# JVBSouza/descriptools

Hardware: AMD Instinct MI355X
Metric: Mcells/s full descriptor chain (higher is better)
Workload: dtype f32; 1 GPU; 16384x16384 synthetic tilted-integer-fBm DEM per GPU, full chain (d8, flowacc, river mask, flowhand/HAND with fused GFI + ln(hl/H), fused slope+TI+MTI, downslope), device-resident; global_dem=16384x16384, river_threshold_cells=524288

## Files before the change

descriptools_amd/_lib.py:

```python
import ctypes as C
import os

import numpy as np

_HERE = os.path.dirname(os.path.abspath(__file__))
_SO = os.path.join(_HERE, "libdescriptools_hip.so")
_lib = None

c_f32p = C.POINTER(C.c_float)
c_f64p = C.POINTER(C.c_double)
c_u8p = C.POINTER(C.c_uint8)
c_i8p = C.POINTER(C.c_int8)
c_i32p = C.POINTER(C.c_int32)
c_i64p = C.POINTER(C.c_int64)
i64, f64, u32, ci = C.c_int64, C.c_double, C.c_uint32, C.c_int
vp = C.c_void_p

_SIGS = {
    "dt_last_error": (C.c_char_p, []),
    "dt_version": (C.c_char_p, []),
    "dt_device_count": (ci, []),
    "dt_set_flow_impl": (ci, [ci]),
    "dt_debug_set": (ci, [ci, ci]),
    "dt_host_trim": (ci, []),
# ... 33 lines not shown
    "dt_dev_condition_d8_f64_async": (ci, [vp, vp, i64, i64, f64, vp, vp, ci]),
    "dt_dev_condition_stage_w": (ci, [vp, vp, ci, ci, vp, vp, vp, vp, vp]),
    "dt_dev_condition_stage_m_w": (ci, [vp, vp, ci, ci, vp, vp, vp, vp, vp, vp]),
    "dt_flowhand": (ci, [c_f32p, c_u8p, c_i8p, i64, i64, f64, c_f32p, c_i64p, c_f32p]),
    "dt_hand_f32": (ci, [c_f32p, c_i64p, i64, c_f32p]),
    "dt_twi": (ci, [c_i64p, c_f32p, i64, f64, f64, c_f32p, c_f32p]),
    "dt_river_accumulation": (ci, [c_i64p, c_i64p, i64, c_i64p]),
    "dt_gfi_area": (ci, [c_f32p, c_i64p, i64, f64, f64, f64, ci, c_f32p]),
    "dt_gfi": (ci, [c_f32p, c_i64p, c_i64p, i64, f64, f64, f64, c_f32p]),
    "dt_lnhlh": (ci, [c_f32p, c_i64p, i64, f64, f64, f64, c_f32p]),
    "dt_downslope": (ci, [c_f32p, c_u8p, i64, i64, f64, f64, ci, c_f32p]),
    "dt_slope_f64": (ci, [c_f64p, i64, i64, f64, c_f32p]),
    "dt_hand_f64": (ci, [c_f64p, c_i64p, i64, c_f64p]),
    "dt_downslope_f64": (ci, [c_f64p, c_u8p, i64, i64, f64, f64, ci, c_f32p]),
    "dt_gfi_f64h": (ci, [c_f64p, c_i64p, c_i64p, i64, f64, f64, f64, ci, c_f32p]),
    "dt_d8_f64": (ci, [c_f64p, i64, i64, f64, c_u8p, c_f32p]),
    "dt_confusion_multi": (ci, [c_f64p, c_i8p, i64, f64, c_f64p, ci, ci, c_i64p]),
    "dt_synth_dem": (ci, [u32, i64, i64, i64, i64, i64, i64, ci, c_f32p]),
    "dt_dev_malloc": (ci, [vp, i64, C.POINTER(vp)]),
    "dt_dev_free": (ci, [vp, vp]),
    "dt_dev_h2d": (ci, [vp, vp, vp, i64]),
    "dt_dev_d2h": (ci, [vp, vp, vp, i64]),
    "dt_dev_d2h_async": (ci, [vp, vp, vp, i64]),
    "dt_dev_synth_dem": (ci, [vp, u32, i64, i64, i64, i64, i64, i64, ci, vp]),
    "dt_dev_slope_d8": (ci, [vp, vp, i64, i64, f64, vp, vp, vp]),
    "dt_dev_slope_twi": (ci, [vp, vp, vp, i64, i64, f64, f64, vp, vp, vp, vp]),
    "dt_dev_flowacc": (ci, [vp, vp, vp, i64, i64, vp]),
    "dt_dev_flowacc_weighted": (ci, [vp, vp, vp, vp, i64, i64, ci, vp]),
    "dt_dev_stream_order": (ci, [vp, vp, vp, i64, i64, vp, vp, vp]),
    "dt_dev_drainage": (ci, [vp, vp, vp, vp, i64, i64, f64, vp, vp, vp]),
    "dt_dev_upslope_length": (ci, [vp, vp, vp, i64, i64, f64, vp]),
    "dt_dev_dinf_direction": (ci, [vp, vp, vp, i64, i64, f64, vp, vp]),
    "dt_dev_dinf_accumulate": (ci, [vp, vp, vp, i64, i64, ci, ci, vp]),
    "dt_dev_dinf_accumulate_info": (ci, [vp, c_i64p]),
    "dt_dev_reach_catchments": (ci, [vp, vp, vp, ci, i64, i64, vp, vp, vp, i64, vp]),
    "dt_dev_reach_channels": (ci, [vp, vp, vp, i64, i64, i64, vp, vp, vp, vp, vp]),
    "dt_dev_reach_tables": (ci, [vp, vp, vp, ci, vp, i64, i64, c_f64p, ci, i64, ci, vp, vp, vp]),
    "dt_dev_inundate": (ci, [vp, vp, vp, ci, vp, i64, i64, i64, vp]),
    "dt_dev_river_mask": (ci, [vp, vp, i64, i64, vp]),
    "dt_dev_flowacc_river": (ci, [vp, vp, vp, i64, i64, i64, vp, vp]),
    "dt_dev_gfi_lnhlh": (ci, [vp, vp, vp, vp, i64, f64, f64, f64, vp, vp]),
    "dt_dev_flowhand": (ci, [vp, vp, vp, vp, vp, i64, i64, f64, vp, vp, vp, vp]),
    "dt_dev_twi": (ci, [vp, vp, vp, i64, f64, f64, vp, vp]),
    "dt_dev_gfi": (ci, [vp, vp, vp, i64, f64, f64, f64, vp]),
    "dt_dev_lnhlh": (ci, [vp, vp, vp, i64, f64, f64, f64, vp]),
    "dt_dev_downslope": (ci, [vp, vp, vp, i64, i64, f64, f64, ci, vp]),
    "dt_downslope_lift_workspace": (i64, [i64, i64]),
    "dt_dev_downslope_lift": (ci, [vp, vp, vp, i64, i64, f64, f64, ci, vp, vp, i64]),
    "dt_downslope_queue_workspace": (i64, [i64, i64]),
    "dt_downslope_tables_workspace": (i64, [i64, i64]),
    "dt_downslope_tables_threshold": (i64, [i64, i64]),
    "dt_dev_downslope_queue": (ci, [vp, vp, vp, i64, i64, f64, f64, ci, vp, vp, i64]),
    "dt_dev_downslope_queued": (ci, [vp, vp, C.POINTER(i64)]),
    "dt_dev_downslope_finish": (ci, [vp, vp, vp, i64, i64, f64, f64, ci, vp, vp, i64, vp, i64]),
    "dt_dev_confusion_multi": (ci, [vp, vp, vp, i64, f64, c_f64p, ci, ci, vp]),
    "dt_perim_cells": (i64, [i64, i64]),
    "dt_dev_slope_d8_w": (ci, [vp, vp, vp, f64, vp, vp, vp]),
    "dt_dev_slope_twi_w": (ci, [vp, vp, vp, vp, f64, f64, vp, vp, vp, vp]),
    "dt_dev_downslope_w": (ci, [vp, vp, vp, vp, f64, f64, ci, vp, vp]),
    "dt_downslope_lift_workspace_w": (i64, [vp]),
    "dt_dev_downslope_lift_w": (ci, [vp, vp, vp, vp, f64, f64, ci, vp, vp, vp, i64]),
    "dt_dev_downslope_emit_w": (ci, [vp, vp, vp, vp, f64, f64, ci, vp, vp, vp, i64, vp, i64]),
    "dt_dev_downslope_walk_w": (ci, [vp, vp, vp, vp, f64, f64, i64, vp, vp, i64]),
    "dt_dev_downslope_walk_route_w": (ci, [vp, vp, vp, vp, f64, f64, i64, vp, vp, i64, vp, vp, C.c_int32, vp, C.c_int32, vp, vp, vp]),
    "dt_dev_downslope_walk_seed_w": (ci, [vp, vp, vp, i64, vp, vp, vp]),
    "dt_dev_flowacc_local_w": (ci, [vp, vp, vp, vp, vp, vp, vp]),
    "dt_dev_flowacc_finish_w": (ci, [vp, vp, vp, vp, vp, i64, vp, vp]),
    "dt_dev_flowhand_local_w": (ci, [vp, vp, vp, vp, vp, vp, vp, vp, vp, vp, vp, vp]),
    "dt_dev_flowhand_finish_w": (ci, [vp, vp, vp, vp, vp, vp, f64, vp, vp, vp, vp, vp, vp, vp, vp, vp, vp, vp]),
    "dt_dev_unique_extremes_f32": (ci, [vp, vp, i64, vp]),
    "dt_dev_minmax_scale_f32": (ci, [vp, vp, i64, C.c_float, C.c_float, C.c_float, vp]),
    "dt_dev_membench_copy": (ci, [vp, vp, vp, i64, ci]),
    "dt_dev_membench_mix": (ci, [vp, vp, vp, vp, vp, vp, i64, ci, ci, ci]),
    "dt_dev_membench_mix_timed": (ci, [vp, vp, vp, vp, vp, vp, i64, ci, ci, ci, ci, c_f64p]),
    "dt_dev_mem_info": (ci, [vp, c_i64p, c_i64p]),
    "dt_dev_minmax_scale_f32_f64": (ci, [vp, vp, i64, f64, f64, f64, vp]),
    "dt_dev_classify": (ci, [vp, vp, vp, i64, f64, f64, ci, ci, vp, vp, vp]),
    "dt_minmax_scale": (ci, [vp, ci, i64, f64, f64, f64, vp]),
    "dt_binary_map": (ci, [vp, ci, i64, f64, f64, ci, c_u8p]),
    "dt_avaliacao": (ci, [c_i32p, c_i8p, i64, c_i32p, c_i64p]),
    "dt_dev_flowhand_gfi": (ci, [vp, vp, vp, vp, vp, i64, i64, f64, f64, f64, vp, vp, vp, vp, vp, vp]),
    "dt_dev_flowhand_gfi_finish_w": (ci, [vp, vp, vp, vp, vp, vp, f64, f64, f64, vp, vp, vp, vp, vp,
                                          vp, vp, vp, vp, vp, vp, vp, vp]),
    "dt_ctx_set_priority": (ci, [vp, ci]),
    "dt_ctx_fork": (ci, [vp, vp]),
    "dt_ctx_join": (ci, [vp, vp]),
    "dt_dev_rank_solve_flowacc": (ci, [vp, ci, ci, c_i64p, c_i64p, i64, vp, i64, c_i64p, ci, i64, vp]),
    "dt_dev_rank_solve_flowhand": (ci, [vp, ci, ci, c_i64p, c_i64p, i64, vp, i64, c_i64p, ci, i64, vp, vp, vp, vp,
                                        vp, vp]),
    "dt_dev_flowacc_finish_w_a64": (ci, [vp, vp, vp, vp, vp, i64, vp, vp]),
    "dt_dev_slope_twi_w_a64": (ci, [vp, vp, vp, vp, f64, f64, vp, vp, vp, vp]),
    "dt_dev_flowhand_local_w_a64": (ci, [vp, vp, vp, vp, vp, vp, vp, vp, vp, vp, vp, vp]),
    "dt_dev_flowhand_finish_w_a64": (ci, [vp, vp, vp, vp, vp, vp, f64, vp, vp, vp, vp, vp, vp, vp, vp, vp, vp, vp]),
    "dt_dev_flowhand_gfi_finish_w_a64": (ci, [vp, vp, vp, vp, vp, vp, f64, f64, f64, vp, vp, vp, vp, vp,
                                              vp, vp, vp, vp, vp, vp, vp, vp]),
    "dt_dev_gfi_lnhlh_a64": (ci, [vp, vp, vp, vp, i64, f64, f64, f64, vp, vp]),
    "dt_dev_flowacc_river_flowhand_local": (ci, [vp, vp, vp, i64, i64, i64, vp, vp]),
    "dt_dev_flowacc_river_flowhand_local_m": (ci, [vp, vp, vp, vp, i64, i64, i64, vp, vp]),
    "dt_dev_slope_d8_m": (ci, [vp, vp, i64, i64, f64, vp, vp]),
    "dt_nodata_mask_bytes": (i64, [i64, i64]),
    "dt_slope_from_d8_ok": (ci, [i64, i64]),
    "dt_slope_marks_bytes": (i64, [i64, i64]),
    "dt_dev_slope_d8_ms": (ci, [vp, vp, i64, i64, f64, vp, vp, vp, vp]),
    "dt_dev_flowacc_river_flowhand_local_ms": (ci, [vp, vp, vp, vp, i64, i64, i64, vp, vp, f64, f64, vp, vp, vp, vp]),
    "dt_dev_slope_twi_fix": (ci, [vp, vp, vp, i64, i64, f64, f64, vp, vp, vp, vp]),
    "dt_dev_flowacc_finish_flowhand_local_w": (ci, [vp, vp, vp, vp, vp, i64, vp, vp, vp, vp, vp, vp, vp, vp]),
    "dt_dev_flowacc_finish_flowhand_local_w_a64": (ci, [vp, vp, vp, vp, vp, i64, vp, vp, vp, vp, vp, vp, vp, vp]),
    "dt_dev_i32_to_i64": (ci, [vp, vp, i64, vp]),
    "dt_dev_i64_to_i32": (ci, [vp, vp, i64, vp]),
    "dt_dev_slope_d8_f64": (ci, [vp, vp, i64, i64, f64, vp, vp]),
    "dt_dev_slope_twi_f64": (ci, [vp, vp, vp, i64, i64, f64, f64, vp, vp, vp, vp]),
    "dt_dev_downslope_f64": (ci, [vp, vp, vp, i64, i64, f64, f64, ci, vp]),
    "dt_dev_hand_gfi_f64": (ci, [vp, vp, vp, vp, i64, i64, f64, f64, f64, vp, vp, vp]),
    "dt_dev_slope_d8_f64_w": (ci, [vp, vp, vp, f64, vp, vp]),
    "dt_dev_slope_twi_f64_w": (ci, [vp, vp, vp, vp, f64, f64, vp, vp, vp, vp]),
    "dt_dev_slope_twi_f64_w_a64": (ci, [vp, vp, vp, vp, f64, f64, vp, vp, vp, vp]),
    "dt_dev_downslope_f64_w": (ci, [vp, vp, vp, vp, f64, f64, ci, vp, vp]),
    "dt_dev_downslope_walk_seed_f64_w": (ci, [vp, vp, vp, i64, vp, vp, vp]),
    "dt_dev_downslope_walk_route_f64_w": (ci, [vp, vp, vp, vp, f64, f64, i64, vp, vp, vp, C.c_int32, vp, C.c_int32,
                                               vp, vp, vp]),
    "dt_dev_flowhand_zr64_w": (ci, [vp, vp, vp, i64, vp, vp, vp]),
    "dt_dev_rank_solve_flowhand_f64": (ci, [vp, ci, ci, c_i64p, c_i64p, i64, vp, i64, c_i64p, ci, i64, vp, vp, vp, vp,
                                            vp, vp, vp]),
    "dt_hand_f64_table_bytes": (i64, [i64]),
    "dt_dev_hand_gfi_f64_w": (ci, [vp, vp, vp, vp, vp, vp, vp, i64, vp, vp, vp, vp, i64, f64, f64, f64, vp, vp, vp]),
    "dt_dev_hand_gfi_f64_w_a64": (ci, [vp, vp, vp, vp, vp, vp, vp, i64, vp, vp, vp, vp, i64, f64, f64, f64, vp, vp,
                                       vp]),
}


class Window(C.Structure):
    _fields_ = [(n, C.c_int64) for n in ("H", "W", "ld", "gy0", "gx0", "Hg", "Wg", "halo")]


def exported_symbols():
    return sorted(_SIGS)


def _preload_torch_hip_runtime():
    import sys
    if "torch" in sys.modules:
        return
    try:
        import importlib.util
        spec = importlib.util.find_spec("torch")
        if spec is None or not spec.submodule_search_locations:
            return
        cand = os.path.join(list(spec.submodule_search_locations)[0], "lib", "libamdhip64.so")
        if os.path.exists(cand):
            C.CDLL(cand, mode=C.RTLD_GLOBAL)
    except Exception:
        pass


def lib():
    global _lib
    if _lib is not None:
        return _lib
    _preload_torch_hip_runtime()
    if not os.path.exists(_SO):
        from . import build as _build
        _build.build()
    try:
        L = C.CDLL(_SO)
    except OSError as e:
        raise RuntimeError("descriptools_amd: cannot load %s (%s); the HIP library is required, "
# ... 108 lines not shown
```

descriptools_amd/build.py:

```python
import os
import subprocess
import sys

HERE = os.path.dirname(os.path.abspath(__file__))
CSRC = os.path.join(HERE, "csrc")
SO = os.path.join(HERE, "libdescriptools_hip.so")
SOURCES = ["dt_kernels.hip", "dt_stencil.hip", "dt_tiles.hip", "dt_hydro.hip", "dt_wide.hip", "dt_streams.hip",
           "dt_watershed.hip", "dt_reaches.hip", "dt_dinf.hip", "dt_proximity.hip", "dt_capi.hip"]
HEADERS = ["dt_common.h", "dt_kernels.h", "dt_math.h", "dt_math_coeffs.h", "dt_d8_kernel.inc", "dt_fa3fh1_kernel.inc",
           os.path.join("..", "..", "include", "descriptools_hip.h")]
FLAGS = ["-O3", "--offload-arch=gfx950", "-fPIC", "-std=c++17", "-ffp-contract=off", "-fno-fast-math",
         "-Wall", "-Wno-unused-function"]


def _stale():
    if not os.path.exists(SO):
        return True
    t = os.path.getmtime(SO)
    deps = [os.path.join(CSRC, f) for f in SOURCES + HEADERS] + [os.path.abspath(__file__)]
    return any(os.path.getmtime(d) > t for d in deps)


def build(force=False, verbose=False):
    if not force and not _stale():
        return SO
    hipcc = os.environ.get("HIPCC", "/opt/rocm/bin/hipcc")
    objs = []
    for src in SOURCES:
        obj = os.path.join(CSRC, src.replace(".hip", ".o"))
        cmd = [hipcc] + FLAGS + ["-c", os.path.join(CSRC, src), "-o", obj]
        if verbose:
            print(" ".join(cmd), flush=True)
        subprocess.check_call(cmd)
        objs.append(obj)
    cmd = [hipcc, "--offload-arch=gfx950", "-shared", "-fPIC", "-o", SO] + objs
    if verbose:
        print(" ".join(cmd), flush=True)
    subprocess.check_call(cmd)
    return SO


if __name__ == "__main__":
    print(build(force="--force" in sys.argv, verbose=True))
```

descriptools_amd/chain.py:

```python
import ctypes as C

import numpy as np

from . import _lib, placement
from ._lib import check
from .device import Context

F32, F64, U8, I8, I32 = np.float32, np.float64, np.uint8, np.int8, np.int32

OUTPUTS = (("slope", F32), ("fdr", U8), ("fac", I32), ("river", I8), ("fdist", F32), ("idx", I32),
           ("hand", F32), ("a_river", I32), ("slope_rad", F32), ("ti", F32), ("mti", F32), ("gfi", F32),
           ("lnhlh", F32), ("down", F32))

ALGO_BYTES_PER_CELL = 90

WRITE_GROUPS = (("slope", "ti", "mti"), ("fdist", "idx", "hand", "gfi", "lnhlh"), ("fac",), ("a_river",),
                ("slope_rad",), ("down",))

OPS = (
    ("d8", 5, ["k_d8<false>", "k_d8_fix"]),
    ("downslope", 9, ["k_downslope_win<24>"]),
    ("flowacc_flowhand_local", 5 + 1 + 2, ["k_fa_tile1", "k_fa_reduce", "k_fa_poison", "k_fa3fh1<2>", "k_fh_tile1",
                                           "k_fh_ghost_init", "k_fh_node_jump"]),
    ("slope_twi", 20, ["k_slope_twi<true, false, 1, int, 1>", "k_slope_twi_fix<int, 1>"]),
    ("flowhand_gfi_finish", 28, ["k_fh_tile3<false, 1, 5, int>"]),
)

OPS_F64 = (
    ("d8", 13, ["k_d8_f64"]),
    ("downslope", 13, ["k_downslope_win_f64"]),
    ("flowacc_flowhand_local", 4 + 1 + 4 + 1 + 2, ["k_fa_tile1", "k_fa_reduce", "k_fa_poison", "k_fa3fh1<2>",
                                                 "k_fh_tile1", "k_fh_ghost_init", "k_fh_node_jump"]),
    ("slope_twi", 24, ["k_slope_twi_f64<false>"]),
    ("flowhand_finish", 10, ["k_fh_tile3<false, 1, 5, int>"]),
    ("hand_gfi", 32, ["k_hand_gfi_f64"]),
)

HEIGHTS = ("float32", "float64")


class Chain:

    def __init__(self, H, W, ctx=None, px=10.0, n_top=0.1, n_gfi=0.4, b=0.1, dz=5.0,
                 river_threshold=None, alloc=None, want_slope_rad=True, side_ctx=None, overlap=True,
                 condition=False, condition_rounds=64, tune_placement=True, release=None, long_walks=False,
                 external_fdr=False, heights="float32"):
        if heights not in HEIGHTS:
            raise ValueError("heights must be one of %s, not %r" % (HEIGHTS, heights))
        self.wide = heights == "float64"
        if self.wide and condition:
            raise ValueError("condition=True is float32-only in Chain: on float64 heights condition the codes with "
                             "dt_dev_condition_d8_f64_async into Chain(heights=\"float64\", external_fdr=True)'s "
                             "p(\"fdr\") (INTEGRATION.md), or use run_host(..., heights=\"float64\", condition=True)")
        if self.wide and long_walks is not False:
            raise ValueError("long_walks is float32-only: the float64 chain walks on its window kernel (long_walks=False)")
        assert long_walks in (False, True, "auto")
        assert not (external_fdr and condition), "conditioning computes the codes itself"
        self.outputs = tuple((k, F64 if (self.wide and k == "hand") else dt) for k, dt in OUTPUTS)
        self.external_fdr = bool(external_fdr)
        self.long_walks = long_walks
        self._lift = self._lift_q = self._lift_dem = self._lift_tables = None
        self.condition, self.condition_rounds = bool(condition), int(condition_rounds)
        self._alloc, self._release = alloc, release
        self.want_slope_rad = want_slope_rad
        self.H, self.W, self.N = int(H), int(W), int(H) * int(W)
        self.ctx = ctx or Context()
        self.side = None
        if overlap:
            self.side = side_ctx if side_ctx is not None else Context(device=self.ctx.device)
        self._own_side = overlap and side_ctx is None
        self.px, self.n_top, self.n_gfi, self.b, self.dz = px, n_top, n_gfi, b, dz
        self.river_threshold = self.N // 512 if river_threshold is None else int(river_threshold)
        self.buf = {}
        self._graphs = []
        for name, dt in self.outputs + ((("filled", F32),) if self.condition else ()):
            self.buf[name] = alloc((H, W), dt) if alloc else self.ctx.empty((H, W), dt)
        self._nodata4 = self._proxy = self._marks = None
        if self.wide:
            self._proxy = self.ctx.empty((H, W), F32)
        elif not (self.external_fdr or self.condition):
            self._nodata4 = self.ctx.empty((int(_lib.lib().dt_nodata_mask_bytes(H, W)),), U8)
            if not want_slope_rad and _lib.lib().dt_slope_from_d8_ok(H, W):
                self._marks = self.ctx.empty((int(_lib.lib().dt_slope_marks_bytes(H, W)),), U8)
        assert tune_placement in (False, True, "search")
        self.placement = {"tuned": False, "why": "tune_placement=False"}
        if tune_placement:
            self._tune_placement(search=tune_placement == "search")

    def _tune_placement(self, search=False):
        four = [name for name, dt in self.outputs if np.dtype(dt).itemsize == 4]
        objs = {}
        for name in four:
            b = self.buf[name]
            objs[int(b.ptr.value if hasattr(b, "ptr") else b)] = b

        def extra_alloc():
            b = self._alloc((self.H, self.W), F32) if self._alloc else self.ctx.empty((self.H, self.W), F32)
            q = int(b.ptr.value if hasattr(b, "ptr") else b)
            objs[q] = b
            return q

        def extra_release(q):
            b = objs.pop(q)
            if hasattr(b, "free"):
                b.free()
            elif self._release is not None:
                self._release(q)
        can_grow = search and (self._alloc is None or self._release is not None)

        def spacer_alloc(nbytes):
            rows = max(int(nbytes) // (self.W * 4), 1)
            if self._alloc:
                return ("user", self._alloc((rows, self.W), F32))
            return ("own", self.ctx.empty((rows, self.W), F32))

        def spacer_release(h):
            kind, b = h
            if kind == "own":
                b.free()
            else:
                self._release(int(b.ptr.value if hasattr(b, "ptr") else b))
        groups = [[k for k in g if k in four] for g in WRITE_GROUPS]
        roles, info = placement.assign(self.ctx, self.N * 4, list(objs), [g for g in groups if g],
                                       extra_alloc if can_grow else None, extra_release if can_grow else None,
                                       spacer_alloc=spacer_alloc if can_grow else None,
                                       spacer_release=spacer_release if can_grow else None, search=search)
        self.placement = info
        if info.get("spacer_GiB"):
            for gib in (2, 16):
                try:
                    self.ctx.empty((gib << 30,), np.uint8).free()
                except MemoryError:
                    break
        if roles is None:
            return
        dts = dict(self.outputs)
        for name, q in roles.items():
            b = objs[q]
            if hasattr(b, "dtype"):
                b.dtype = np.dtype(dts[name])
            self.buf[name] = b

    def _lift_ptr(self):
        if self._lift is None:
            self._lift_bytes = int(_lib.lib().dt_downslope_lift_workspace(self.H, self.W))
            self._lift = self.ctx.empty((self._lift_bytes,), np.uint8)
        return self._lift.ptr

    def _queue_downslope(self, side, dem_ptr):
        L = _lib.lib()
        if self._lift_q is None:
            self._lift_q_bytes = int(L.dt_downslope_queue_workspace(self.H, self.W))
            self._lift_q = self.ctx.empty((self._lift_q_bytes,), np.uint8)
        self._lift_dem = dem_ptr
        return L.dt_dev_downslope_queue(side.h, dem_ptr, self.p("fdr"), self.H, self.W, self.px, self.dz, 0,
                                        self.p("down"), self._lift_q.ptr, self._lift_q_bytes)

    def finish_long_walks(self):
        if self.long_walks != "auto" or self._lift_q is None:
            return 0
        L, c = _lib.lib(), self.ctx
        n = C.c_int64(0)
        check(L.dt_dev_downslope_queued(c.h, self._lift_q.ptr, C.byref(n)))
        if n.value == 0:
            return 0
        tables, tb = None, 0
        if n.value >= int(L.dt_downslope_tables_threshold(self.H, self.W)):
            tb = int(L.dt_downslope_tables_workspace(self.H, self.W))
            if self._lift_tables is None:
                try:
                    self._lift_tables = c.empty((tb,), np.uint8)
                except MemoryError:
                    tb = 0
            tables = self._lift_tables
        check(L.dt_dev_downslope_finish(c.h, self._lift_dem, self.p("fdr"), self.H, self.W, self.px, self.dz, 0,
                                        self.p("down"), self._lift_q.ptr, self._lift_q_bytes,
                                        tables.ptr if tables is not None else None, tb if tables is not None else 0))
        c.sync()
        return int(n.value)

    def p(self, name):
        b = self.buf[name]
        return b.ptr if hasattr(b, "ptr") else b

    def ops(self, dem_ptr, want_a_river=False, serial=False):
        L, c, H, W = _lib.lib(), self.ctx, self.H, self.W
        p = self.p
        side = self.side if (self.side is not None and not serial) else c
        if getattr(self, "_full", None) is None:
            self._full = _lib.Window(H, W, W, 0, 0, H, W, 0)
        full = self._full
        if self.wide:
            return self._ops_f64(dem_ptr, want_a_river, side)
        rad = p("slope_rad") if self.want_slope_rad else None
        m4 = self._nodata4.ptr if self._nodata4 is not None else None
        first = ("d8", c, lambda: L.dt_dev_slope_d8_m(c.h, dem_ptr, H, W, self.px, p("fdr"), m4))
        flow = ((lambda: L.dt_dev_flowacc_river_flowhand_local_m(c.h, p("fdr"), dem_ptr, m4, H, W, self.river_threshold,
                                                                 p("fac"), p("river"))) if m4 is not None else
                (lambda: L.dt_dev_flowacc_river_flowhand_local(c.h, p("fdr"), dem_ptr, H, W, self.river_threshold,
                                                               p("fac"), p("river"))))
        twi = lambda: L.dt_dev_slope_twi(side.h, dem_ptr, p("fac"), H, W, self.px, self.n_top, p("slope"), rad, p("ti"),
                                         p("mti"))
        if self._from_d8(dem_ptr):
            marks = self._marks.ptr
            first = ("d8", c, lambda: L.dt_dev_slope_d8_ms(c.h, dem_ptr, H, W, self.px, p("fdr"), m4, p("slope"), marks))
            flow = lambda: L.dt_dev_flowacc_river_flowhand_local_ms(
                c.h, p("fdr"), dem_ptr, m4, H, W, self.river_threshold, p("fac"), p("river"), self.px, self.n_top,
                p("slope"), p("ti"), p("mti"), marks)
            twi = lambda: L.dt_dev_slope_twi_fix(side.h, dem_ptr, p("fac"), H, W, self.px, self.n_top, p("slope"),
                                                 p("ti"), p("mti"), marks)
        if self.condition:
            first = ("condition_d8", c, lambda: L.dt_dev_condition_d8_async(c.h, dem_ptr, H, W, self.px, p("filled"),
                                                                             p("fdr"), self.condition_rounds))
        return ([] if self.external_fdr else [first]) + [
            ("downslope", side, (lambda: L.dt_dev_downslope_lift(side.h, dem_ptr, p("fdr"), H, W, self.px, self.dz, 0,
                                                                  p("down"), self._lift_ptr(), self._lift_bytes))
             if self.long_walks is True else
             (lambda: self._queue_downslope(side, dem_ptr)) if self.long_walks == "auto" else
             (lambda: L.dt_dev_downslope(side.h, dem_ptr, p("fdr"), H, W, self.px, self.dz, 0, p("down")))),
            ("flowacc_flowhand_local", c, flow),
            ("slope_twi", side, twi),
            ("flowhand_gfi_finish", c, lambda: L.dt_dev_flowhand_gfi_finish_w(
                c.h, C.byref(full), dem_ptr, p("fdr"), p("river"), p("fac"), self.px, self.n_gfi, self.b, None, None,
                None, None, None, None, p("fdist"), p("idx"), None, p("hand"),
                p("a_river") if want_a_river else None, p("gfi"), p("lnhlh"))),
        ]

    def _from_d8(self, dem_ptr=None):
        if self._marks is None:
            return False
        ptrs = [self.p(k) for k in ("slope", "fac", "ti", "mti", "river", "fdr")] + ([dem_ptr] if dem_ptr else [])
        return all((int(q.value if hasattr(q, "value") else q) & 15) == 0 for q in ptrs)

    def _ops_f64(self, dem_ptr, want_a_river, side):
        L, c, H, W, p = _lib.lib(), self.ctx, self.H, self.W, self.p
        prox = self._proxy.ptr
        rad = p("slope_rad") if self.want_slope_rad else None
        first = ("d8", c, lambda: L.dt_dev_slope_d8_f64(c.h, dem_ptr, H, W, self.px, p("fdr"), prox))
        if self.external_fdr:
            first = ("nodata_proxy", c, lambda: L.dt_dev_slope_d8_f64(c.h, dem_ptr, H, W, self.px, None, prox))
        return [
            first,
            ("downslope", side, lambda: L.dt_dev_downslope_f64(side.h, dem_ptr, p("fdr"), H, W, self.px, self.dz, 0,
                                                               p("down"))),
            ("flowacc_flowhand_local", c, lambda: L.dt_dev_flowacc_river_flowhand_local(
                c.h, p("fdr"), prox, H, W, self.river_threshold, p("fac"), p("river"))),
            ("slope_twi", side, lambda: L.dt_dev_slope_twi_f64(side.h, dem_ptr, p("fac"), H, W, self.px, self.n_top,
                                                               p("slope"), rad, p("ti"), p("mti"))),
            ("flowhand_finish", c, lambda: L.dt_dev_flowhand_finish_w(
                c.h, C.byref(self._full), None, p("fdr"), p("river"), p("fac"), self.px, None, None, None, None, None,
                None, p("fdist"), p("idx"), None, None, p("a_river") if want_a_river else None)),
            ("hand_gfi", c, lambda: L.dt_dev_hand_gfi_f64(c.h, dem_ptr, p("idx"), p("fac"), H, W, self.px, self.n_gfi,
                                                          self.b, p("hand"), p("gfi"), p("lnhlh"))),
        ]

    def run(self, dem_ptr, want_a_river=True):
        for name, ctx, call in self.ops(dem_ptr, want_a_river):
            if ctx is not self.ctx:
                self.ctx.fork(ctx)
            check(call())
        if self.side is not None:
            self.ctx.join(self.side)

    def check_status(self):
        self.ctx.raise_on_status()

    def capture(self, dem_ptr, want_a_river=True):
        self.run(dem_ptr, want_a_river)
        self.ctx.sync()
        L = _lib.lib()
        check(L.dt_ctx_capture_begin(self.ctx.h))
        g = C.c_void_p()
        try:
            self.run(dem_ptr, want_a_river)
        except BaseException:
            if L.dt_ctx_capture_end(self.ctx.h, C.byref(g)) == 0 and g:
                L.dt_graph_destroy(g)
            raise
        check(L.dt_ctx_capture_end(self.ctx.h, C.byref(g)))
        gr = Graph(g, self.ctx, self)
        self._graphs.append(gr)
        return gr

    def free(self):
        for gr in self._graphs:
            gr.invalidate("the chain it was captured from has been freed")
        self._graphs = []
        if self._own_side:
            self.side.close()
            self.side, self._own_side = None, False
        for b in list(self.buf.values()):
            if hasattr(b, "free"):
                b.free()
        self.buf = {}
        for name in ("_lift", "_lift_q", "_lift_tables", "_nodata4", "_proxy", "_marks"):
            if getattr(self, name) is not None:
                getattr(self, name).free()
                setattr(self, name, None)


class Graph:

    def __init__(self, handle, ctx, chain=None):
        self.h, self.ctx, self.chain, self._dead = handle, ctx, chain, None

    def invalidate(self, why):
        self._dead = why

    def launch(self):
        if self._dead:
            raise RuntimeError("captured step cannot be replayed: " + self._dead)
        check(_lib.lib().dt_graph_launch(self.h, self.ctx.h))

    def free(self):
        if self.h:
            check(_lib.lib().dt_graph_destroy(self.h))
            self.h = None
        if self.chain is not None and self in self.chain._graphs:
            self.chain._graphs.remove(self)
        self.chain = None


def run_host(dem, px, timings=None, heights="float32", **kw):
    import time
    t0 = time.perf_counter()
    d, wide = _lib.dem_tier(dem, heights)
    H, W = d.shape
    cond64 = None
    if wide:
        if kw.get("long_walks", False) is not False:
            raise ValueError("long_walks is float32-only: the float64 chain walks on its window kernel (long_walks=False)")
        if kw.pop("condition", False):
            if kw.get("external_fdr"):
                raise ValueError("condition=True computes the codes itself: external_fdr must be False")
            cond64 = int(kw.pop("condition_rounds", 64))
            kw["external_fdr"] = True
    ctx = Context()
    kw.setdefault("tune_placement", False)
    kw.setdefault("long_walks", False if wide else "auto")
    ch = Chain(H, W, ctx=ctx, px=px, heights="float64" if wide else "float32", **kw)
    t1 = time.perf_counter()
    d_dem = ctx.to_device(d)
    widened = {k: ctx.empty((H, W), np.int64) for k in ("fac", "idx")}
    filled = ctx.empty((H, W), np.float64) if cond64 is not None else None
# ... 34 lines not shown
```

descriptools_amd/csrc/dt_capi.hip:

```cpp
#include <cmath>
#include <stdarg.h>
#include <stdlib.h>

#include <sys/mman.h>
#include <atomic>
#include <chrono>
#include <mutex>
#include <system_error>
#include <thread>
#include <utility>
#include <vector>

#include "dt_common.h"
#include "dt_kernels.h"

static thread_local char g_err[512] = "";
void dt_set_error(const char *fmt, ...) {
  va_list ap;
  va_start(ap, fmt);
  vsnprintf(g_err, sizeof(g_err), fmt, ap);
  va_end(ap);
}
extern "C" const char *dt_last_error(void) { return g_err; }
extern "C" const char *dt_version(void) { return "descriptools_hip 0.1 (gfx950)"; }
// ... 1191 lines not shown
}

static int dev_flowhand_local_w(dt_ctx *c, const dt_window *win, const float *dem, const uint8_t *fdr,
                                const int8_t *river, const void *acc, int acc64, uint8_t *kind, int32_t *ref,
                                int32_t *nc, int32_t *nd, float *zr, int64_t *ar) {
  DT_DEV(d, c, win);
  DT_REQUIRE(fdr && river && kind && ref && nc && nd && zr && ar, "NULL pointer");
  const size_t need = dt_flowhand_tiled_scratch(d.w.H, d.w.W);
  void *scr = d.scratch(need);
  DT_TRY(d.rc);
  DT_TRY(dt_launch_fh_local(c->stream, d.w, fdr, river, scr, need));
  DT_TRY(d.done(dt_launch_fh_summary(c->stream, d.w, scr, dem, acc, acc64, kind, ref, nc, nd, zr, (long long *)ar)));
  dt_scratch_claim(c, DT_OWNER_HAND, d.w.H, d.w.W, scr);
  return DT_OK;
}
extern "C" int dt_dev_flowhand_local_w(dt_ctx *c, const dt_window *win, const float *dem, const uint8_t *fdr,
                                       const int8_t *river, const int32_t *acc32, uint8_t *kind, int32_t *ref,
                                       int32_t *nc, int32_t *nd, float *zr, int64_t *ar) {
  return dev_flowhand_local_w(c, win, dem, fdr, river, acc32, 0, kind, ref, nc, nd, zr, ar);
}
extern "C" int dt_dev_flowhand_local_w_a64(dt_ctx *c, const dt_window *win, const float *dem, const uint8_t *fdr,
                                           const int8_t *river, const int64_t *acc64, uint8_t *kind, int32_t *ref,
                                           int32_t *nc, int32_t *nd, float *zr, int64_t *ar) {
  return dev_flowhand_local_w(c, win, dem, fdr, river, acc64, 1, kind, ref, nc, nd, zr, ar);
}

static int dev_flowhand_finish_w(dt_ctx *c, const dt_window *win, const float *dem, const uint8_t *fdr,
                                 const int8_t *river, const void *acc, int acc64, double px, double n_gfi, double b,
                                 const uint8_t *res_ok, const int32_t *res_nc, const int32_t *res_nd,
                                 const int64_t *rem_gidx, const float *rem_zr, const int64_t *rem_ar, float *fdist,
                                 int32_t *idx32, int64_t *idx64, float *hand, void *a_river, float *gfi,
                                 float *lnhlh, bool fused) {
  DT_DEV(d, c, win);
  DT_REQUIRE(fdr && river, "NULL raster");
  DT_REQUIRE(!hand || dem, "hand needs dem");
  DT_REQUIRE(!a_river || acc, "a_river needs the accumulation raster");
  DT_REQUIRE(!fused || (dem && acc && gfi && lnhlh), "NULL raster");
  DT_REQUIRE(!res_ok || (res_nc && res_nd && rem_gidx && rem_zr && rem_ar), "incomplete rank-exit results");
  const DtScratchClaim *k;
  DT_TRY(dt_scratch_claimed(c, DT_OWNER_HAND, &d.w, false,
                            "flowhand finish without a matching dt_dev_flowhand_local_w on this context (another call "
                            "has used the context's scratch in between)", &k));
  return d.done(dt_launch_fh_finish(c->stream, d.w, dem, fdr, river, acc, acc64, px, k->ptr, res_ok, res_nc, res_nd,
                                    (const long long *)rem_gidx, rem_zr, (const long long *)rem_ar, fdist, idx32,
                                    (long long *)idx64, hand, a_river, fused ? gfi : nullptr, fused ? lnhlh : nullptr,
                                    n_gfi, b, px));
}
extern "C" int dt_dev_flowhand_finish_w(dt_ctx *c, const dt_window *win, const float *dem, const uint8_t *fdr,
                                        const int8_t *river, const int32_t *acc32, double px,
                                        const uint8_t *res_ok, const int32_t *res_nc, const int32_t *res_nd,
                                        const int64_t *rem_gidx, const float *rem_zr, const int64_t *rem_ar,
                                        float *fdist, int32_t *idx32, int64_t *idx64, float *hand,
                                        int32_t *a_river) {
  return dev_flowhand_finish_w(c, win, dem, fdr, river, acc32, 0, px, 0.0, 1.0, res_ok, res_nc, res_nd, rem_gidx, rem_zr,
                               rem_ar, fdist, idx32, idx64, hand, a_river, nullptr, nullptr, false);
}
extern "C" int dt_dev_flowhand_finish_w_a64(dt_ctx *c, const dt_window *win, const float *dem, const uint8_t *fdr,
                                            const int8_t *river, const int64_t *acc64, double px,
                                            const uint8_t *res_ok, const int32_t *res_nc, const int32_t *res_nd,
                                            const int64_t *rem_gidx, const float *rem_zr, const int64_t *rem_ar,
                                            float *fdist, int32_t *idx32, int64_t *idx64, float *hand,
                                            int64_t *a_river64) {
  return dev_flowhand_finish_w(c, win, dem, fdr, river, acc64, 1, px, 0.0, 1.0, res_ok, res_nc, res_nd, rem_gidx, rem_zr,
                               rem_ar, fdist, idx32, idx64, hand, a_river64, nullptr, nullptr, false);
}
extern "C" int dt_dev_flowhand_gfi_finish_w(dt_ctx *c, const dt_window *win, const float *dem, const uint8_t *fdr,
                                            const int8_t *river, const int32_t *acc32, double px, double n_gfi,
                                            double b, const uint8_t *res_ok, const int32_t *res_nc,
                                            const int32_t *res_nd, const int64_t *rem_gidx, const float *rem_zr,
                                            const int64_t *rem_ar, float *fdist, int32_t *idx32, int64_t *idx64,
                                            float *hand, int32_t *a_river, float *gfi, float *lnhlh) {
  return dev_flowhand_finish_w(c, win, dem, fdr, river, acc32, 0, px, n_gfi, b, res_ok, res_nc, res_nd, rem_gidx, rem_zr,
                               rem_ar, fdist, idx32, idx64, hand, a_river, gfi, lnhlh, true);
}
extern "C" int dt_dev_flowhand_gfi_finish_w_a64(dt_ctx *c, const dt_window *win, const float *dem,
                                                const uint8_t *fdr, const int8_t *river, const int64_t *acc64,
                                                double px, double n_gfi, double b, const uint8_t *res_ok,
                                                const int32_t *res_nc, const int32_t *res_nd,
                                                const int64_t *rem_gidx, const float *rem_zr, const int64_t *rem_ar,
                                                float *fdist, int32_t *idx32, int64_t *idx64, float *hand,
                                                int64_t *a_river64, float *gfi, float *lnhlh) {
  return dev_flowhand_finish_w(c, win, dem, fdr, river, acc64, 1, px, n_gfi, b, res_ok, res_nc, res_nd, rem_gidx, rem_zr,
                               rem_ar, fdist, idx32, idx64, hand, a_river64, gfi, lnhlh, true);
}

static int dt_scratch2_reserve(dt_ctx *c, size_t bytes) {
  return dt_side_reserve(c, &c->scratch2, &c->scratch2_bytes, bytes);
}

extern "C" int dt_dev_rank_solve_flowacc(dt_ctx *c, int ty, int tx, const int64_t *heights, const int64_t *widths,
                                         int64_t Pmax, const void *rows_dev, int64_t rowbytes,
                                         const int64_t *field_offsets3, int rank, int64_t P_rank,
                                         uint64_t *ext_out_dev) {
  DT_DEV(d, c);
  DT_REQUIRE(heights && widths && rows_dev && field_offsets3 && ext_out_dev, "NULL pointer");
  DT_REQUIRE(rank >= 0 && rank < ty * tx && P_rank >= 0 && P_rank <= Pmax, "bad rank / ring size");
  DT_TRY(dt_scratch2_reserve(c, dt_rank_solve_scratch(ty * tx, Pmax)));
  return d.done(dt_launch_rank_solve_flowacc(c->stream, ty, tx, heights, widths, Pmax, rows_dev, rowbytes,
                                             field_offsets3, rank, P_rank, c->scratch2,
                                             (unsigned long long *)ext_out_dev));
}

extern "C" int dt_dev_rank_solve_flowhand(dt_ctx *c, int ty, int tx, const int64_t *heights, const int64_t *widths,
                                          int64_t Pmax, const void *rows_dev, int64_t rowbytes,
                                          const int64_t *field_offsets7, int rank, int64_t P_rank,
                                          uint8_t *res_ok, int32_t *res_nc, int32_t *res_nd, int64_t *rem_gidx,
                                          float *rem_zr, int64_t *rem_ar) {
  DT_DEV(d, c);
  DT_REQUIRE(heights && widths && rows_dev && field_offsets7 && res_ok && res_nc && res_nd && rem_gidx && rem_zr &&
                 rem_ar, "NULL pointer");
  DT_REQUIRE(rank >= 0 && rank < ty * tx && P_rank >= 0 && P_rank <= Pmax, "bad rank / ring size");
  DT_TRY(dt_scratch2_reserve(c, dt_rank_solve_scratch(ty * tx, Pmax)));
  return d.done(dt_launch_rank_solve_flowhand(c->stream, ty, tx, heights, widths, Pmax, rows_dev, rowbytes,
                                              field_offsets7, rank, P_rank, c->scratch2, res_ok, res_nc, res_nd,
                                              (long long *)rem_gidx, rem_zr, (long long *)rem_ar));
}

extern "C" int dt_dev_slope_d8_f64_w(dt_ctx *c, const dt_window *win, const double *dem, double px, uint8_t *fdr,
                                     float *proxy) {
  DT_DEV(d, c, win);
  DT_REQUIRE(dem && (fdr || proxy), "NULL raster");
  return d.done(dt_launch_d8_f64_w(c->stream, d.w, dem, px, fdr, proxy));
}
static int dev_slope_twi_f64_w(dt_ctx *c, const dt_window *win, const double *dem, const void *acc, int acc64,
                               double px, double n_top, float *slope, float *slope_rad, float *ti, float *mti) {
  DT_DEV(d, c, win);
  DT_REQUIRE(dem && acc && ti && mti, "NULL raster");
  return d.done(dt_launch_slope_twi_f64_w(c->stream, d.w, dem, acc, acc64, px, n_top, slope, slope_rad, ti, mti));
}
extern "C" int dt_dev_slope_twi_f64_w(dt_ctx *c, const dt_window *win, const double *dem, const int32_t *acc32,
                                      double px, double n_top, float *slope, float *slope_rad, float *ti, float *mti) {
  return dev_slope_twi_f64_w(c, win, dem, acc32, 0, px, n_top, slope, slope_rad, ti, mti);
}
extern "C" int dt_dev_slope_twi_f64_w_a64(dt_ctx *c, const dt_window *win, const double *dem, const int64_t *acc64,
                                          double px, double n_top, float *slope, float *slope_rad, float *ti,
                                          float *mti) {
  return dev_slope_twi_f64_w(c, win, dem, acc64, 1, px, n_top, slope, slope_rad, ti, mti);
}
extern "C" int dt_dev_downslope_f64_w(dt_ctx *c, const dt_window *win, const double *dem, const uint8_t *fdr,
                                      double px, double dz, int raw, float *out, int32_t *n_unresolved_dev) {
  DT_DEV(d, c, win);
  DT_REQUIRE(dem && fdr && out, "NULL raster");
  if (n_unresolved_dev) DT_HIP(hipMemsetAsync(n_unresolved_dev, 0, sizeof(int32_t), c->stream));
  return d.done(dt_launch_downslope_win_f64_w(c->stream, d.w, dem, fdr, px, dz, raw, out, (int *)n_unresolved_dev));
}
extern "C" int dt_dev_downslope_walk_seed_f64_w(dt_ctx *c, const dt_window *win, const double *dem, int64_t n,
                                                const int32_t *ys, const int32_t *xs, void *rec) {
  return dev_downslope_walk_seed_w(c, win, dem, n, ys, xs, rec, dt_launch_ds_walk_seed_f64);
}
extern "C" int dt_dev_downslope_walk_route_f64_w(dt_ctx *c, const dt_window *win, const double *dem,
                                                 const uint8_t *fdr, double px, double dz, int64_t n, void *rec,
                                                 float *out, const int32_t *row_starts, int32_t ty,
                                                 const int32_t *col_starts, int32_t tx, void *send, int32_t *counts,
                                                 int32_t *scratch) {
  DT_DEV(d, c, win);
  DT_REQUIRE(n >= 0, "negative count");
  DT_REQUIRE(ty >= 1 && tx >= 1 && row_starts && col_starts && counts, "layout / counts missing");
  DT_REQUIRE(n == 0 || (dem && fdr && rec && out && send && scratch), "NULL pointer");
  DT_TRY(dt_launch_ds_walk_f64(c->stream, d.w, dem, fdr, px, dz, n, rec, out));
  return d.done(dt_launch_ds_route(c->stream, n, rec, row_starts, ty, col_starts, tx, send, counts, scratch));
}
extern "C" int dt_dev_flowhand_zr64_w(dt_ctx *c, const dt_window *win, const double *dem, int64_t n,
                                      const uint8_t *kind, const int32_t *ref, double *zr64) {
  DT_DEV(d, c, win);
  DT_REQUIRE(n >= 0 && n <= dt_perim_count(d.w.H, d.w.W), "bad ring size");
  DT_REQUIRE(n == 0 || (dem && kind && ref && zr64), "NULL pointer");
// ... 877 lines not shown
```

descriptools_amd/csrc/dt_kernels.h:

```cpp
#pragma once
#include "dt_common.h"

int dt_launch_synth_dem(hipStream_t s, uint32_t seed, int O, int64_t Hg, int64_t y0, int64_t x0,
                        int64_t h, int64_t w, int nodata_pct, float *out);
int dt_launch_stencil(hipStream_t s, const DtWin &w, const float *dem, double px, float *slope,
                      uint8_t *fdr, float *slope_rad, const void *acc, int acc64, double n_top, float *ti,
                      float *mti, void *aux = nullptr, uint8_t *nod4 = nullptr, int ldm = 0);
static inline int dt_nodata4_ld(int64_t W) { return (int)((((W + 3) / 4) + 7) & ~(int64_t)7); }
static inline size_t dt_nodata4_bytes(int64_t H, int64_t W) { return (size_t)((H + 3) / 4) * (size_t)dt_nodata4_ld(W) * 2; }
struct DtStencilAux {
  uint8_t *mark;
  uint16_t *lmask;
  size_t bytes;
};
static inline DtStencilAux dt_stencil_aux_layout(int64_t ntiles, void *aux) {
  DtStencilAux a;
  DtCarver c(aux);
  a.mark = c.take<uint8_t>((size_t)ntiles);
  a.lmask = c.take<uint16_t>((size_t)ntiles * 256);
  a.bytes = c.bytes();
  return a;
}
size_t dt_stencil_aux_bytes(int64_t H, int64_t W);
int dt_launch_d8_slope(hipStream_t s, const DtWin &w, const float *dem, double px, uint8_t *fdr, float *slope,
                       void *aux, uint8_t *nod4, int ldm, void *smarks);
int dt_launch_slope_twi_fix(hipStream_t s, const DtWin &w, const float *dem, double px, float *slope,
                            const int32_t *acc, double n_top, float *ti, float *mti, void *smarks);
int dt_launch_flowacc(hipStream_t s, const uint8_t *fdr, const float *dem, int64_t H, int64_t W,
                      unsigned long long *state, int32_t *acc32);
int dt_launch_river_mask(hipStream_t s, const int32_t *acc32, int64_t n, int64_t thr, int8_t *river);
int dt_launch_flowhand(hipStream_t s, const float *dem, const uint8_t *fdr, const int8_t *river,
                       const int32_t *acc32, int64_t H, int64_t W, double px,
                       unsigned long long *state, float *fdist, int32_t *idx32, float *hand,
                       int32_t *a_river);
int dt_launch_twi(hipStream_t s, const int32_t *acc32, const float *srad, int64_t n, double px,
                  double n_top, float *ti, float *mti);
int dt_launch_twi_i64(hipStream_t s, const int64_t *fac, const float *srad, int64_t n, double px,
                      double n_top, float *ti, float *mti);
int dt_launch_gfi(hipStream_t s, const float *hand, const int32_t *area, int64_t n, double expo,
                  double b, double size, float *out, int own_cell);
int dt_launch_gfi_i64(hipStream_t s, const float *hand, const int64_t *area, int64_t n, double expo,
                      double b, double size, float *out, int own_cell);
int dt_launch_river_acc_i64(hipStream_t s, const int64_t *fac, const int64_t *idx, int64_t n,
                            int64_t *out);
struct DtDsLift {
  uint32_t *qcount;
  uint4 *qentries;
  uint32_t qcapacity;
  uint2 *tab[3];
  uint8_t *dom;
  size_t queue_bytes, tables_bytes, bytes;
};
DtDsLift dt_downslope_lift_layout(const DtWin &w, void *work);
size_t dt_downslope_lift_bytes(int64_t H, int64_t W);
size_t dt_downslope_queue_bytes(int64_t H, int64_t W);
size_t dt_downslope_tables_bytes(int64_t H, int64_t W);
uint32_t dt_downslope_lift_min(int64_t H, int64_t W);
size_t dt_downslope_tables_bytes_w(const DtWin &w);
size_t dt_downslope_lift_bytes_w(const DtWin &w);
int dt_launch_downslope(hipStream_t s, const DtWin &w, const float *dem, const uint8_t *fdr, double px,
                        double dz, int raw, float *out, int *n_unresolved, void *qwork = nullptr,
                        void *twork = nullptr, int phase = 0, void *walkers = nullptr, size_t walkers_bytes = 0);
int dt_launch_ds_walk(hipStream_t s, const DtWin &w, const float *dem, const uint8_t *fdr, double px, double dz,
                      int64_t n, void *rec, void *work, float *out = nullptr);
int dt_launch_ds_route(hipStream_t s, int64_t n, const void *rec, const int32_t *row_starts, int ty,
                       const int32_t *col_starts, int tx, void *send, int32_t *counts, int32_t *scratch);
int dt_launch_ds_walk_seed(hipStream_t s, const DtWin &w, const float *dem, int64_t n, const int32_t *ys,
                           const int32_t *xs, void *rec);
int dt_launch_downslope_v1(hipStream_t s, const float *dem, const uint8_t *fdr, int64_t H, int64_t W,
                           double px, double dz, int raw, float *out);
int dt_launch_hand_i64(hipStream_t s, const float *dem, const int64_t *idx, int64_t n, float *hand);
int dt_launch_slope_f64(hipStream_t s, const double *dem, int64_t H, int64_t W, double px, float *slope);
int dt_launch_hand_f64(hipStream_t s, const double *dem, const int64_t *idx, int64_t n, double *hand);
int dt_launch_downslope_f64(hipStream_t s, const double *dem, const uint8_t *fdr, int64_t H, int64_t W, double px,
                            double dz, int raw, float *out);
int dt_launch_gfi_f64h(hipStream_t s, const double *hand, const int64_t *fac, const int64_t *idx, int64_t n,
                       double expo, double b, double size, int own_area, float *out);
int dt_launch_d8_f64(hipStream_t s, const double *dem, int64_t H, int64_t W, double px, uint8_t *fdr, float *slope,
                     float *proxy);
int dt_launch_slope_twi_f64(hipStream_t s, const double *dem, const int32_t *acc32, int64_t H, int64_t W, double px,
                            double n_top, float *slope, float *slope_rad, float *ti, float *mti);
int dt_launch_downslope_win_f64(hipStream_t s, const double *dem, const uint8_t *fdr, int64_t H, int64_t W, double px,
                                double dz, int raw, float *out);
int dt_launch_hand_gfi_f64(hipStream_t s, const double *dem, const int32_t *idx32, const int32_t *acc32, int64_t n,
                           double expo, double b, double size, double *hand, float *gfi, float *lnhlh);
int dt_launch_d8_f64_w(hipStream_t s, const DtWin &w, const double *dem, double px, uint8_t *fdr, float *proxy);
int dt_launch_slope_twi_f64_w(hipStream_t s, const DtWin &w, const double *dem, const void *acc, int acc64, double px,
                              double n_top, float *slope, float *slope_rad, float *ti, float *mti);
int dt_launch_downslope_win_f64_w(hipStream_t s, const DtWin &w, const double *dem, const uint8_t *fdr, double px,
                                  double dz, int raw, float *out, int *n_unresolved);
int dt_launch_fh_zr64_w(hipStream_t s, const DtWin &w, const double *dem, int64_t n, const uint8_t *kind,
                        const int32_t *ref, double *zr64);
int64_t dt_hand_f64_table_slots(int64_t n_remote);
int dt_launch_hand_gfi_f64_w(hipStream_t s, const DtWin &w, const double *dem, const int32_t *idx32,
                             const int64_t *idx64, const void *fac, const void *a_river, int acc64, int64_t n_remote,
                             const uint8_t *res_ok, const int64_t *rem_gidx, const double *rem_zr64, void *table,
                             double expo, double b, double size, double *hand, float *gfi, float *lnhlh);
int dt_launch_ds_walk_f64(hipStream_t s, const DtWin &w, const double *dem, const uint8_t *fdr, double px, double dz,
                          int64_t n, void *rec, float *out);
int dt_launch_ds_walk_seed_f64(hipStream_t s, const DtWin &w, const double *dem, int64_t n, const int32_t *ys,
                               const int32_t *xs, void *rec);
int dt_launch_confusion(hipStream_t s, const double *desc, const int8_t *flood, int64_t n,
                        double nodata, const double *th_host, int nth, int under,
                        unsigned long long *counts4);
int dt_launch_i32_to_i64(hipStream_t s, const int32_t *a, int64_t n, int64_t *b);
int dt_launch_i64_to_i32(hipStream_t s, const int64_t *a, int64_t n, int32_t *b);

size_t dt_flowacc_tiled_scratch(int64_t H, int64_t W);
int dt_launch_fa_local(hipStream_t s, const DtWin &w, const uint8_t *fdr, void *scratch, size_t scratch_bytes,
                       int32_t *acc32, int rank_level);
int dt_launch_fa_summary(hipStream_t s, const DtWin &w, void *scratch, int64_t *A, int32_t *xr, uint8_t *code);
int dt_launch_fa_finish(hipStream_t s, const DtWin &w, const uint8_t *fdr, const float *dem, void *scratch,
                        const unsigned long long *ext_perim, int64_t river_thr, void *acc, int acc64,
                        int8_t *river, int *status = nullptr);
size_t dt_flowacc_weighted_scratch(int64_t H, int64_t W);
int dt_launch_flowacc_weighted(hipStream_t s, const DtWin &w, const uint8_t *fdr, const float *dem, const double *wt,
                               int frac_bits, void *scratch, size_t scratch_bytes, double *acc, int *status);
size_t dt_flowhand_tiled_scratch(int64_t H, int64_t W);
struct DtTwiEpilogue {
  const float *slope;
  float *ti, *mti;
  double px, n_top;
  void *marks;
};
int dt_launch_fa_finish_fh_local(hipStream_t s, const DtWin &w, const uint8_t *fdr, const float *dem, void *fa_scratch,
                                 void *fh_scratch, size_t fh_bytes, const unsigned long long *ext_perim,
                                 int64_t river_thr, void *acc, int acc64, int8_t *river, int *status,
                                 const uint8_t *nod4 = nullptr, int ldm = 0, const DtTwiEpilogue *twi = nullptr);
bool dt_twi_epilogue_ok(const DtWin &w, const void *acc, const int8_t *river, const DtTwiEpilogue *twi);
int dt_launch_fh_local(hipStream_t s, const DtWin &w, const uint8_t *fdr, const int8_t *river, void *scratch,
                       size_t scratch_bytes);
int dt_launch_fh_summary(hipStream_t s, const DtWin &w, void *scratch, const float *dem, const void *acc, int acc64,
                         uint8_t *kind, int32_t *ref, int32_t *nc, int32_t *nd, float *zr, long long *ar);
int dt_launch_fh_finish(hipStream_t s, const DtWin &w, const float *dem, const uint8_t *fdr,
                        const int8_t *river, const void *acc, int acc64, double px, void *scratch,
                        const uint8_t *res_ok, const int32_t *res_nc, const int32_t *res_nd,
                        const long long *rem_gidx, const float *rem_zr, const long long *rem_ar, float *fdist,
                        int32_t *idx32, long long *idx64, float *hand, void *a_river, float *gfi = nullptr,
                        float *lnhlh = nullptr, double n_gfi = 0.0, double b_gfi = 1.0, double size = 1.0);
int dt_launch_gfi_both(hipStream_t s, const float *hand, const void *a_river, const void *fac, int acc64,
                       int64_t n, double expo, double b, double size, float *gfi, float *lnhlh);
int dt_launch_unique_extremes(hipStream_t s, const float *x, int64_t n, uint32_t *work4, float *out3);
int dt_launch_minmax_scale(hipStream_t s, const float *x, int64_t n, float mn, float mx, float nodata,
                           double *out);
int dt_launch_minmax_scale_f32f32(hipStream_t s, const float *x, int64_t n, float mn, float mx, float nodata,
                                  float *out);
int dt_launch_minmax_scale_f64(hipStream_t s, const double *x, int64_t n, double mn, double mx, double nodata,
                               double *out);
int dt_launch_minmax_scale_f32f64(hipStream_t s, const float *x, int64_t n, double mn, double mx, double nodata,
                                  double *out);
int dt_launch_classify_f64(hipStream_t s, const double *desc, const int32_t *bin_in, int8_t *flood, int64_t n,
// ... 84 lines not shown
```

descriptools_amd/csrc/dt_kernels.hip:

```cpp
#include <math.h>

#include "dt_common.h"
#include "dt_kernels.h"
#include "dt_math.h"

void dt_math_host_table(DtLogEntry *tab) {
  for (int i = 0; i < DT_LOGTAB_N; i++) {
    double c = 1.0 + (i + 0.5) / DT_LOGTAB_N;
    double rc = 1.0 / c;
    tab[i].rc = rc;
    tab[i].lnc = (double)(-logl((long double)rc));
  }
}
__device__ DtLogEntry g_logtab[DT_LOGTAB_N];
const DtLogEntry *dt_math_device_table(hipStream_t s) {
  static thread_local int uploaded_dev = -1;
  int dev = 0;
  (void)hipGetDevice(&dev);
  DtLogEntry *p = nullptr;
  (void)hipGetSymbolAddress((void **)&p, HIP_SYMBOL(g_logtab));
  if (uploaded_dev != dev) {
    static DtLogEntry host[DT_LOGTAB_N];
    dt_math_host_table(host);
    (void)hipMemcpyAsync(p, host, sizeof(host), hipMemcpyHostToDevice, s);
    (void)hipStreamSynchronize(s);
    uploaded_dev = dev;
  }
  return p;
}

#define DT_SYNTH_TILT 64
#define DT_SYNTH_KMIN 5
#define DT_SYNTH_SX 4
__constant__ int32_t c_synth_amp[15] = {0,    0,    0,    0,    0,     256,   445,  776,
                                        1351, 2352, 4096, 7131, 12416, 21618, 37640};

__device__ __forceinline__ uint32_t dt_hash32(uint32_t seed, uint32_t o, uint32_t ix, uint32_t iy) {
  uint32_t h = seed * 0x9E3779B1u ^ (o + 1u) * 0x85EBCA77u;
  h ^= ix * 0xC2B2AE3Du;
  h = ((h << 13) | (h >> 19)) * 0x27D4EB2Fu;
  h ^= iy * 0x165667B1u;
  h = ((h << 13) | (h >> 19)) * 0x9E3779B1u;
  h ^= h >> 15;
  h *= 0x85EBCA6Bu;
  h ^= h >> 13;
  h *= 0xC2B2AE35u;
  h ^= h >> 16;
  return h;
}

__global__ __launch_bounds__(256) void k_synth_dem(uint32_t seed, int O, int64_t Hg, int64_t y0,
                                                  int64_t x0, int64_t h, int64_t w, int nodata_pct,
                                                  float *__restrict__ out) {
  int64_t i = (int64_t)blockIdx.x * 256 + threadIdx.x;
  if (i >= h * w) return;
  int64_t r = i / w, c = i - r * w;
  int64_t y = y0 + r, x = x0 + c;
  int64_t z = (int64_t)DT_SYNTH_TILT * (Hg - 1 - y);
  for (int o = 0; o < O; o++) {
    int sh = O - o;
    if (sh < DT_SYNTH_KMIN) break;
    int shx = sh - DT_SYNTH_SX;
    uint32_t lx = (uint32_t)(x >> shx), ly = (uint32_t)(y >> sh);
    uint64_t fx = (uint64_t)(x & ((1 << shx) - 1)) << (16 - shx);
    uint64_t fy = (uint64_t)(y & ((1 << sh) - 1)) << (16 - sh);
    uint64_t v00 = dt_hash32(seed, (uint32_t)o, lx, ly) >> 16;
    uint64_t v10 = dt_hash32(seed, (uint32_t)o, lx + 1, ly) >> 16;
    uint64_t v01 = dt_hash32(seed, (uint32_t)o, lx, ly + 1) >> 16;
    uint64_t v11 = dt_hash32(seed, (uint32_t)o, lx + 1, ly + 1) >> 16;
    uint64_t top = v00 * (65536 - fx) + v10 * fx;
    uint64_t bot = v01 * (65536 - fx) + v11 * fx;
    uint64_t val = (top * (65536 - fy) + bot * fy) >> 32;
    z += (int64_t)((val * (uint64_t)c_synth_amp[sh]) >> 16);
  }
  float zf = (float)z * (1.0f / 256.0f);
  if (nodata_pct > 0) {
    uint32_t hb = dt_hash32(seed ^ 0xA5A5A5A5u, 77u, (uint32_t)(x >> 5), (uint32_t)(y >> 5));
    if ((hb % 100u) < (uint32_t)nodata_pct) zf = DT_NODATA;
  }
  out[i] = zf;
}

int dt_launch_synth_dem(hipStream_t s, uint32_t seed, int O, int64_t Hg, int64_t y0, int64_t x0,
                        int64_t h, int64_t w, int nodata_pct, float *out) {
  int64_t n = h * w;
  if (n == 0) return DT_OK;
  hipLaunchKernelGGL(k_synth_dem, dim3((unsigned)((n + 255) / 256)), dim3(256), 0, s, seed, O, Hg,
// ... 454 lines not shown
      dt_d8_delta(code, dy, dx);
      int ny = y + dy, nx = x + dx;
      if (!dt_in_global(w, ny, nx)) { failed = true; break; }
      if (!dt_readable(w, ny, nx)) { unresolved = true; break; }
      const long long on = (long long)ny * w.ld + nx;
      float zt = dem[on];
      code = fdr[on];
      if (zt == DT_NODATA) { failed = true; break; }
      y = ny;
      x = nx;
      nd += (dy != 0 && dx != 0) ? 1u : 0u;
      drop = z0 - zt;
      if (++loop == 5000u) { failed = true; break; }
    }
  }
  float res = 0.0f;
  if (!slow && !unresolved && loop != 0u) {
    bool safe;
    res = ds_quotient(drop, loop, nd, dcard, ddiag, safe);
    if (!safe) slow = true;
  }
  if (slow) {
    y = y0;
    x = x0;
    double dist = 0.0;
    drop = 0.0f;
    failed = false;
    unresolved = false;
    uint32_t moves = 0;
    nd = 0u;
    while ((double)drop < dz) {
      if (!(RANKED ? dt_has_code(w, y, x) : dt_readable(w, y, x))) { unresolved = true; break; }
      uint32_t code = fdr[(long long)y * w.ld + x];
      if (!dt_d8_valid(code)) { failed = true; break; }
      int dy, dx;
      dt_d8_delta(code, dy, dx);
      int ny = y + dy, nx = x + dx;
      if (!dt_in_global(w, ny, nx)) { failed = true; break; }
      if (!dt_readable(w, ny, nx)) { unresolved = true; break; }
      float zt = dem[(long long)ny * w.ld + nx];
      if (zt == DT_NODATA) { failed = true; break; }
      y = ny;
      x = nx;
      dist += (dy != 0 && dx != 0) ? ddiag : dcard;
      drop = z0 - zt;
      if (++moves == 5000u) { failed = true; break; }
    }
    res = dist == 0.0 ? 0.0f : (float)((double)drop / dist);
    loop = moves;
    wflags = DSW_SEQ;
    wdist = dist;
  }
  if (unresolved) {
    *outp = -50.0f;
    n_unres++;
    if (RANKED && wo.rec) ds_emit_walker(wo, w, y0, x0, y, x, loop, nd, z0, wflags, wdist);
  } else if (raw && failed) *outp = -50.0f;
  else *outp = res;
}

template <bool RANKED>
__device__ __attribute__((noinline)) void ds_finish_overflow(const DtWin &w, const float *__restrict__ dem,
                                                             const uint8_t *__restrict__ fdr, int y0, int x0, float z0,
                                                             uint32_t loop, uint32_t nd, uint32_t pos, double px,
                                                             double dz, float dzf, int raw, float *__restrict__ out,
                                                             int *__restrict__ n_unresolved, DsWalkOut wo) {
  int y, x;
  ds_mem_cell(w, pos, y, x);
  uint32_t unres = 0u;
  ds_finish_cell<RANKED>(w, dem, fdr, y0, x0, z0, z0 - dem[(long long)y * w.ld + x], loop, nd, false, y, x, px,
                        px * sqrt(2.0), dz, dzf, raw, out + (long long)y0 * w.ld + x0, unres, wo);
  if (unres && n_unresolved) atomicAdd(n_unresolved, (int)unres);
}

#define DW_CORE 64
#define MW_OFF 0x3FFu
#define MW_BIAS 512
#define MW_DIAG 0x400u
#define MW_BADCODE 0x800u
#define MW_EDGE 0x1000u
#define MW_RING 0x2000u
#define MW_STOP 0x8000u

template <int DW_M, bool QUEUE, bool RANKED>
__device__ __forceinline__ void ds_win_body(const float *__restrict__ dem,
                                                       const uint8_t *__restrict__ fdr, DtWin w,
                                                       double px, double dz, float dzf, int raw,
                                                       float *__restrict__ out, int tiles_x, int ntiles,
                                                       int *__restrict__ n_unresolved, DsQueue queue, DsWalkOut wo) {
  constexpr int DW_WIN = DW_CORE + 2 * DW_M, DW_LD = DW_WIN + 4;
  __shared__ __attribute__((aligned(16))) unsigned char smem[DW_LD * DW_WIN * 6];
  __shared__ uint16_t s_lut[256];
  __shared__ uint32_t s_queued[3];
  float *s_z = reinterpret_cast<float *>(smem);
  uint16_t *s_w = reinterpret_cast<uint16_t *>(smem + DW_LD * DW_WIN * 4);
  const uint32_t lds0 = (uint32_t)(uintptr_t)(__attribute__((address_space(3))) unsigned char *)smem;
  int b = blockIdx.x, tile;
  {
    int xcd = b & 7, j = b >> 3;
    int q = ntiles >> 3, rem = ntiles & 7;
    if (rem == 0 && q % tiles_x == 0 && (tiles_x & 7) == 0) {
      const int rows = q / tiles_x, per_strip = rows * 8;
      const int strip = j / per_strip, r = (j - strip * per_strip) >> 3, c = (j & 7) + strip * 8;
      tile = xcd * q + r * tiles_x + c;
    } else {
      tile = (xcd < rem ? xcd * (q + 1) : rem * (q + 1) + (xcd - rem) * q) + j;
    }
  }
  const int tyi = tile / tiles_x, txi = tile - tyi * tiles_x;
  const int wy0 = tyi * DW_CORE - DW_M, wx0 = txi * DW_CORE - DW_M;
  const bool vec = (w.ld % 4 == 0) && (((uintptr_t)dem & 15) == 0) && (((uintptr_t)fdr & 3) == 0);
  const int ya = max(-w.halo, -w.gy0), yb = min(w.H + w.halo, w.Hg - w.gy0);
  const int xa = max(-w.halo, -w.gx0), xb = min(w.W + w.halo, w.Wg - w.gx0);
  const int yca = (RANKED && -w.halo > -w.gy0) ? ya + 1 : ya, ycb = (RANKED && w.H + w.halo < w.Hg - w.gy0) ? yb - 1 : yb;
  const int xca = (RANKED && -w.halo > -w.gx0) ? xa + 1 : xa, xcb = (RANKED && w.W + w.halo < w.Wg - w.gx0) ? xb - 1 : xb;
  const bool interior = vec && wy0 >= yca && wy0 + DW_WIN <= ycb && wx0 >= xca && wx0 + DW_WIN <= xcb &&
                        w.gy0 + wy0 >= 1 && w.gy0 + wy0 + DW_WIN <= w.Hg - 1 && w.gx0 + wx0 >= 1 &&
                        w.gx0 + wx0 + DW_WIN <= w.Wg - 1;
  const float ninf = -__builtin_inff();
  constexpr int NG = DW_WIN * (DW_WIN / 4);
  float4 vv[4];
  uint32_t cc[4];
  int nod_here = 0;
  if (interior) {
#pragma unroll
    for (int u = 0; u < 4; u++) {
      int i = threadIdx.x + 1024 * u;
      if (i < NG) {
        int r = i / (DW_WIN / 4), c4 = (i - r * (DW_WIN / 4)) * 4;
        long long g = (long long)(wy0 + r) * w.ld + wx0 + c4;
        vv[u] = *reinterpret_cast<const float4 *>(dem + g);
        cc[u] = *reinterpret_cast<const uint32_t *>(fdr + g);
      }
    }
  }
  if (threadIdx.x < 256) {
    uint32_t code = threadIdx.x, mw = MW_BADCODE | MW_STOP | MW_BIAS;
    if (dt_d8_valid(code)) {
      int dy, dx;
      dt_d8_delta(code, dy, dx);
      mw = (uint32_t)(2 * (dy * DW_LD + dx) + MW_BIAS);
      if (dy != 0 && dx != 0) mw |= MW_DIAG;
    }
    s_lut[code] = (uint16_t)mw;
  }
  if ((QUEUE || RANKED) && threadIdx.x == 0) s_queued[0] = s_queued[2] = 0u;
  __syncthreads();
  if (interior) {
#pragma unroll
    for (int u = 0; u < 4; u++) {
      int i = threadIdx.x + 1024 * u;
      if (i < NG) {
        int r = i / (DW_WIN / 4), c4 = (i - r * (DW_WIN / 4)) * 4;
        const uint32_t rowring = (r == 0 || r == DW_WIN - 1) ? (MW_RING | MW_STOP) : 0u;
        uint32_t m0 = (uint32_t)s_lut[cc[u] & 0xFFu] | rowring | (c4 == 0 ? (MW_RING | MW_STOP) : 0u);
        uint32_t m1 = (uint32_t)s_lut[(cc[u] >> 8) & 0xFFu] | rowring;
        uint32_t m2 = (uint32_t)s_lut[(cc[u] >> 16) & 0xFFu] | rowring;
        uint32_t m3 = (uint32_t)s_lut[cc[u] >> 24] | rowring | (c4 == DW_WIN - 4 ? (MW_RING | MW_STOP) : 0u);
        float4 v = vv[u];
        nod_here |= (v.x == DT_NODATA || v.y == DT_NODATA || v.z == DT_NODATA || v.w == DT_NODATA) ? 1 : 0;
        v.x = v.x == DT_NODATA ? ninf : v.x;
        v.y = v.y == DT_NODATA ? ninf : v.y;
        v.z = v.z == DT_NODATA ? ninf : v.z;
        v.w = v.w == DT_NODATA ? ninf : v.w;
        *reinterpret_cast<float4 *>(&s_z[r * DW_LD + c4]) = v;
        *reinterpret_cast<uint2 *>(&s_w[r * DW_LD + c4]) = make_uint2(m0 | (m1 << 16), m2 | (m3 << 16));
      }
    }
  } else {
    for (int i = threadIdx.x; i < NG; i += 1024) {
      int r = i / (DW_WIN / 4), c4 = (i - r * (DW_WIN / 4)) * 4;
      int gy = wy0 + r, gx = wx0 + c4;
      float4 v = make_float4(0.f, 0.f, 0.f, 0.f);
      uint32_t mwv[4];
      uint32_t codes = 0;
      const bool row_ok = gy >= ya && gy < yb;
      bool rd[4];
#pragma unroll
      for (int k = 0; k < 4; k++) rd[k] = row_ok && gx + k >= xa && gx + k < xb;
      if (vec && rd[0] && rd[3]) {
        v = *reinterpret_cast<const float4 *>(dem + (long long)gy * w.ld + gx);
        codes = *reinterpret_cast<const uint32_t *>(fdr + (long long)gy * w.ld + gx);
      } else {
        const float *p = dem + (long long)gy * w.ld;
        const uint8_t *f = fdr + (long long)gy * w.ld;
        if (rd[0]) { v.x = p[gx]; codes |= (uint32_t)f[gx]; }
        if (rd[1]) { v.y = p[gx + 1]; codes |= (uint32_t)f[gx + 1] << 8; }
        if (rd[2]) { v.z = p[gx + 2]; codes |= (uint32_t)f[gx + 2] << 16; }
        if (rd[3]) { v.w = p[gx + 3]; codes |= (uint32_t)f[gx + 3] << 24; }
      }
#pragma unroll
      for (int k = 0; k < 4; k++) {
// ... 56 lines not shown
    uint32_t q2 = q2_0, mw = s_w[pos0], acc = 0;
    {
      uint32_t t, cnt;
      float zt;
      uint64_t sv;
      asm volatile(
          "s_mov_b64 %[sv], exec\n\t"
          "s_movk_i32 %[cnt], %[cap]\n\t"
          "v_cmpx_gt_f32 vcc, %[dzf], %[drop]\n\t"
          "v_cmpx_gt_u32 vcc, 0x8000, %[mw]\n\t"
          "s_cbranch_execz 2f\n"
          "1:\n\t"
          "v_and_b32 %[t], 0x3ff, %[mw]\n\t"
          "v_add3_u32 %[acc], %[acc], %[mw], %[k19]\n\t"
          "v_add3_u32 %[q2], %[q2], %[t], %[nbias]\n\t"
          "v_lshl_add_u32 %[t], %[q2], 1, %[n2l]\n\t"
          "ds_read_b32 %[zt], %[t]\n\t"
          "ds_read_u16 %[mw], %[q2] offset:%[woff]\n\t"
          "s_sub_u32 %[cnt], %[cnt], 1\n\t"
          "s_waitcnt lgkmcnt(0)\n\t"
          "v_sub_f32 %[drop], %[z0], %[zt]\n\t"
          "s_cbranch_scc1 2f\n\t"
          "v_cmpx_gt_f32 vcc, %[dzf], %[drop]\n\t"
          "v_cmpx_gt_u32 vcc, 0x8000, %[mw]\n\t"
          "s_cbranch_execnz 1b\n"
          "2:\n\t"
          "s_mov_b64 exec, %[sv]"
          : [q2] "+v"(q2), [mw] "+v"(mw), [acc] "+v"(acc), [drop] "+v"(drop), [t] "=&v"(t), [zt] "=&v"(zt),
            [sv] "=&s"(sv), [cnt] "=&s"(cnt)
          : [z0] "v"(z0), [dzf] "s"(dzf), [nbias] "s"(0u - (uint32_t)MW_BIAS), [n2l] "s"(neg2lds0),
            [k19] "s"(1u << 19), [woff] "n"(DW_LD * DW_WIN * 4),
            [cap] "n"(QUEUE ? DS_Q_CAP : 255)
          : "vcc", "scc", "memory");
    }
    uint32_t loop = acc >> 19;
    uint32_t nd = ((acc & 0x7FFFFu) - (q2 - q2_0) - (uint32_t)MW_BIAS * loop) / MW_DIAG;
    const uint32_t pos = (q2 - lds0) >> 1;
    const int ys = wy0 + (int)(pos / DW_LD), xs = wx0 + (int)(pos % DW_LD);
    const bool stop_fail = (mw & (MW_BADCODE | MW_EDGE)) != 0u;
    if (QUEUE && drop < dzf && !stop_fail && (RANKED ? dt_has_code(w, ys, xs) : dt_readable(w, ys, xs))) {
      const uint32_t pq = ds_mem_index(w, ys, xs), pl = loop | (nd << 16);
      if (j == 0) { pq0 = pq; pl0 = pl; }
      else if (j == 1) { pq1 = pq; pl1 = pl; }
      else if (j == 2) { pq2 = pq; pl2 = pl; }
      else { pq3 = pq; pl3 = pl; }
      pend |= 1u << j;
      continue;
    }
    ds_finish_cell<RANKED>(w, dem, fdr, y0, x0, z0, drop, loop, nd, stop_fail, ys, xs, dcard, ddiag, dz, dzf, raw,
                           out + o, unres, wo);
  }
  if (RANKED) {
    if (unres) atomicAdd(&s_queued[2], unres);
    __syncthreads();
    if (threadIdx.x == 0 && s_queued[2] && n_unresolved) atomicAdd(n_unresolved, (int)s_queued[2]);
  } else if (unres && n_unresolved) {
    atomicAdd(n_unresolved, (int)unres);
  }
  if (QUEUE) {
    const uint32_t mine = (uint32_t)__popc(pend);
    uint32_t slot = 0u;
    if (mine) slot = atomicAdd(&s_queued[0], mine);
    __syncthreads();
    if (threadIdx.x == 0 && s_queued[0]) s_queued[1] = atomicAdd(queue.count, s_queued[0]);
    __syncthreads();
    slot += s_queued[1];
    for (int j = 0; pend >> j; j++) {
      if (!((pend >> j) & 1u)) continue;
      const uint32_t pq = j == 0 ? pq0 : j == 1 ? pq1 : j == 2 ? pq2 : pq3;
      const uint32_t pl = j == 0 ? pl0 : j == 1 ? pl1 : j == 2 ? pl2 : pl3;
      const int c = threadIdx.x + 1024 * j;
      const int cy = c / DW_CORE, cx = c - cy * DW_CORE;
      const int y0 = tyi * DW_CORE + cy, x0 = txi * DW_CORE + cx;
      if (slot < queue.capacity) {
        queue.entries[slot] = make_uint4(ds_mem_index(w, y0, x0), pq, pl & 0xFFFFu, pl >> 16);
      } else {
        const float z0 = s_z[(cy + DW_M) * DW_LD + cx + DW_M];
        ds_finish_overflow<RANKED>(w, dem, fdr, y0, x0, z0, pl & 0xFFFFu, pl >> 16, pq, px, dz, dzf, raw, out,
                                   n_unresolved, wo);
      }
      slot++;
    }
  }
}

template <int DW_M>
__global__ __launch_bounds__(1024, 8) void k_downslope_win(const float *__restrict__ dem,
                                                       const uint8_t *__restrict__ fdr, DtWin w, double px, double dz,
                                                       float dzf, int raw, float *__restrict__ out, int tiles_x,
                                                       int ntiles, int *__restrict__ n_unresolved) {
  ds_win_body<DW_M, false, false>(dem, fdr, w, px, dz, dzf, raw, out, tiles_x, ntiles, n_unresolved, DsQueue(),
                                  DsWalkOut());
}
__global__ __launch_bounds__(1024, 8) void k_downslope_win_r(const float *__restrict__ dem,
                                                         const uint8_t *__restrict__ fdr, DtWin w, double px,
                                                         double dz, float dzf, int raw, float *__restrict__ out,
                                                         int tiles_x, int ntiles, int *__restrict__ n_unresolved,
                                                         DsWalkOut wo) {
  ds_win_body<24, false, true>(dem, fdr, w, px, dz, dzf, raw, out, tiles_x, ntiles, n_unresolved, DsQueue(), wo);
}
__global__ __launch_bounds__(1024, 8) void k_downslope_win_q(const float *__restrict__ dem,
                                                         const uint8_t *__restrict__ fdr, DtWin w, double px,
                                                         double dz, float dzf, int raw, float *__restrict__ out,
                                                         int tiles_x, int ntiles, int *__restrict__ n_unresolved,
                                                         DsQueue queue) {
  ds_win_body<24, true, false>(dem, fdr, w, px, dz, dzf, raw, out, tiles_x, ntiles, n_unresolved, queue, DsWalkOut());
}

__global__ __launch_bounds__(1024, 8) void k_downslope_win_rq(const float *__restrict__ dem,
                                                          const uint8_t *__restrict__ fdr, DtWin w, double px,
                                                          double dz, float dzf, int raw, float *__restrict__ out,
                                                          int tiles_x, int ntiles, int *__restrict__ n_unresolved,
                                                          DsQueue queue, DsWalkOut wo) {
  ds_win_body<24, true, true>(dem, fdr, w, px, dz, dzf, raw, out, tiles_x, ntiles, n_unresolved, queue, wo);
}

__device__ __forceinline__ float ds_lift_z(float z) { return z != z ? -__builtin_inff() : z; }
#define LT_M 8
#define LT_WIN (64 + 2 * LT_M)
#define LT_LD (LT_WIN + 1)
template <bool RANKED>
__global__ __launch_bounds__(256) void k_ds_lift_init(const float *__restrict__ dem, const uint8_t *__restrict__ fdr,
                                                     DtWin w, uint2 *__restrict__ T, const uint32_t *__restrict__ qcount,
                                                     uint32_t lift_min, int tiles_x) {
  if (*qcount < lift_min) return;
  __shared__ uint2 s_c[LT_WIN * LT_LD];
  __shared__ uint32_t s_tab[256];
  {
    const uint32_t code = threadIdx.x;
    uint32_t m = 0u;
    if (dt_d8_valid(code)) {
      int dy, dx;
      dt_d8_delta(code, dy, dx);
      m = ((uint32_t)((dy * LT_LD + dx) * 8) & 0xFFFFu) | (1u << 16) | ((dy != 0 && dx != 0) ? (1u << 24) : 0u);
    }
    s_tab[code] = m;
  }
  const int ty = (int)blockIdx.x / tiles_x, tx = (int)blockIdx.x - ty * tiles_x;
  const int y0 = ty * 64 - w.halo, x0 = tx * 64 - w.halo;
  const int wy0 = y0 - LT_M, wx0 = x0 - LT_M;
  static_assert(LT_WIN * LT_WIN % 256 == 0, "the staging loops are unrolled");
  constexpr int LT_CPT = LT_WIN * LT_WIN / 256;
  float zs[LT_CPT];
  uint8_t cs[LT_CPT];
  const int ring = RANKED ? 1 : 0;
  const bool inside = wy0 >= -w.halo + ring && wy0 + LT_WIN <= w.H + w.halo - ring && wx0 >= -w.halo + ring &&
                      wx0 + LT_WIN <= w.W + w.halo - ring && w.gy0 + wy0 >= 0 && w.gy0 + wy0 + LT_WIN <= w.Hg &&
                      w.gx0 + wx0 >= 0 && w.gx0 + wx0 + LT_WIN <= w.Wg;
  if (inside) {
    const float *__restrict__ d0 = dem + ((long long)wy0 * w.ld + wx0);
    const uint8_t *__restrict__ f0 = fdr + ((long long)wy0 * w.ld + wx0);
    const int ld = (int)w.ld;
#pragma unroll
    for (int j = 0; j < LT_CPT; j++) {
      const int i = (int)threadIdx.x + 256 * j;
      const int r = i / LT_WIN, c = i - r * LT_WIN;
      zs[j] = d0[r * ld + c];
      cs[j] = f0[r * ld + c];
    }
  } else {
#pragma unroll
    for (int j = 0; j < LT_CPT; j++) {
      const int i = (int)threadIdx.x + 256 * j;
      const int r = i / LT_WIN, c = i - r * LT_WIN;
      const int y = wy0 + r, x = wx0 + c;
      zs[j] = dt_readable(w, y, x) ? dem[(long long)y * w.ld + x] : DT_NODATA;
      cs[j] = (RANKED ? dt_has_code(w, y, x) : dt_readable(w, y, x)) ? fdr[(long long)y * w.ld + x] : (uint8_t)0;
    }
  }
  int valid = 0;
#pragma unroll
  for (int j = 0; j < LT_CPT; j++) {
    const int i = (int)threadIdx.x + 256 * j;
    const int r = i / LT_WIN, c = i - r * LT_WIN;
    valid |= (r >= LT_M && r < LT_M + 64 && c >= LT_M && c < LT_M + 64 && zs[j] != DT_NODATA) ? 1 : 0;
// ... 453 lines not shown
  L.bytes = c.bytes();
  L.tables_bytes = L.bytes - L.queue_bytes;
  return L;
}
static DtDsLift ds_sizes(int64_t H, int64_t W) { return dt_downslope_lift_layout(dt_full_window(H, W), nullptr); }
size_t dt_downslope_queue_bytes(int64_t H, int64_t W) { return ds_sizes(H, W).queue_bytes; }
size_t dt_downslope_tables_bytes(int64_t H, int64_t W) { return ds_sizes(H, W).tables_bytes; }
size_t dt_downslope_lift_bytes(int64_t H, int64_t W) { return ds_sizes(H, W).bytes; }
uint32_t dt_downslope_lift_min(int64_t H, int64_t W) { return (uint32_t)std::max<int64_t>(DS_LIFT_MIN, H * W / 256); }
size_t dt_downslope_tables_bytes_w(const DtWin &w) { return dt_downslope_lift_layout(w, nullptr).tables_bytes; }
size_t dt_downslope_lift_bytes_w(const DtWin &w) { return dt_downslope_lift_layout(w, nullptr).bytes; }
int dt_launch_downslope(hipStream_t s, const DtWin &w, const float *dem, const uint8_t *fdr, double px,
                        double dz, int raw, float *out, int *n_unresolved, void *qwork, void *twork, int phase,
                        void *walkers, size_t walkers_bytes) {
  const int64_t H = w.H, W = w.W;
  int64_t n = H * W;
  if (n == 0) return DT_OK;
  int tiles_x = (int)((W + DW_CORE - 1) / DW_CORE), tiles_y = (int)((H + DW_CORE - 1) / DW_CORE);
  int64_t ntiles = (int64_t)tiles_x * tiles_y;
  float dzf = (float)dz;
  if ((double)dzf < dz) dzf = nextafterf(dzf, INFINITY);
  DsQueue q;
  DsWalkOut wo;
  if (walkers && walkers_bytes >= 256 + DSW_WORDS * 4) {
    DtCarver cw(walkers);
    wo.count = (uint32_t *)cw.raw(256);
    wo.rec = (uint4 *)((char *)walkers + cw.bytes());
    wo.capacity = (uint32_t)std::min<size_t>((walkers_bytes - cw.bytes()) / (DSW_WORDS * 4), 0x7FFFFFFFu);
    if (phase != 2) DT_HIP(hipMemsetAsync(wo.count, 0, sizeof(uint32_t), s));
  }
  DtDsLift L = {};
  const bool ranked = !(w.halo == 0 && w.gy0 == 0 && w.gx0 == 0 && w.Hg == w.H && w.Wg == w.W);
  if (qwork && ds_mem_cells(w) < 0x7FFFFFFFull) {
    DtCarver cq(qwork), ct(twork);
    ds_carve_queue(cq, w, L);
    ds_carve_tables(ct, w, L);
    q.count = L.qcount;
    q.entries = L.qentries;
    q.capacity = L.qcapacity;
  }
  DT_REQUIRE(phase == 0 || q.entries, "the phases of the long-walk form need the queue workspace (and a window of < 2^31 cells)");
  if (phase != 2) {
    if (q.entries) DT_HIP(hipMemsetAsync(q.count, 0, sizeof(uint32_t), s));
    if (ranked && q.entries)
      hipLaunchKernelGGL(k_downslope_win_rq, dim3((unsigned)ntiles), dim3(1024), 0, s, dem, fdr, w, px, dz, dzf, raw,
                         out, tiles_x, (int)ntiles, n_unresolved, q, wo);
    else if (ranked)
      hipLaunchKernelGGL(k_downslope_win_r, dim3((unsigned)ntiles), dim3(1024), 0, s, dem, fdr, w, px, dz, dzf, raw,
                         out, tiles_x, (int)ntiles, n_unresolved, wo);
    else if (q.entries)
      hipLaunchKernelGGL(k_downslope_win_q, dim3((unsigned)ntiles), dim3(1024), 0, s, dem, fdr, w, px, dz, dzf, raw,
                         out, tiles_x, (int)ntiles, n_unresolved, q);
    else
      hipLaunchKernelGGL(k_downslope_win<24>, dim3((unsigned)ntiles), dim3(1024), 0, s, dem, fdr, w, px, dz, dzf, raw,
                         out, tiles_x, (int)ntiles, n_unresolved);
  }
  if (q.entries && phase != 1) {
    const dim3 b(256);
    const uint32_t lift_min = dt_downslope_lift_min(H, W);
    uint2 *src = nullptr;
    const unsigned fin_blocks = dt_capped_grid(q.capacity, 8192);
    if (L.tab[0]) {
      DT_HIP(hipMemsetAsync(L.dom, 0, ds_mem_cells(w), s));
      const int rows = (int)(H + 2 * w.halo), cols = (int)(W + 2 * w.halo);
      const int ltx = (cols + 63) / 64, lty = (rows + 63) / 64;
      const dim3 gt((unsigned)(ltx * lty));
      const uint32_t *qc = (const uint32_t *)q.count;
      if (ranked) hipLaunchKernelGGL(k_ds_lift_init<true>, gt, b, 0, s, dem, fdr, w, L.tab[2], qc, lift_min, ltx);
      else hipLaunchKernelGGL(k_ds_lift_init<false>, gt, b, 0, s, dem, fdr, w, L.tab[2], qc, lift_min, ltx);
      hipLaunchKernelGGL(k_ds_tab_double<true>, dim3(fin_blocks), b, 0, s, q, (const uint2 *)L.tab[2], L.tab[0], L.dom, (int)w.ld, lift_min);
      hipLaunchKernelGGL(k_ds_tab_double<false>, dim3(fin_blocks), b, 0, s, q, (const uint2 *)L.tab[0], L.tab[1], L.dom, (int)w.ld, lift_min);
      hipLaunchKernelGGL(k_ds_tab_double<false>, dim3(fin_blocks), b, 0, s, q, (const uint2 *)L.tab[1], L.tab[0], L.dom, (int)w.ld, lift_min);
      src = L.tab[0];
    }
    if (ranked)
      hipLaunchKernelGGL(k_ds_finish<true>, dim3(fin_blocks), b, 0, s, dem, fdr, w, px, dz, dzf, raw, out, q,
                         (const uint2 *)src, (const uint2 *)L.tab[2], (const uint8_t *)L.dom, n_unresolved, lift_min, wo);
    else
      hipLaunchKernelGGL(k_ds_finish<false>, dim3(fin_blocks), b, 0, s, dem, fdr, w, px, dz, dzf, raw, out, q,
                         (const uint2 *)src, (const uint2 *)L.tab[2], (const uint8_t *)L.dom, n_unresolved, lift_min, DsWalkOut());
  }
  return DT_OK;
}
int dt_launch_downslope_v1(hipStream_t s, const float *dem, const uint8_t *fdr, int64_t H, int64_t W,
                           double px, double dz, int raw, float *out) {
  int64_t n = H * W;
  if (n == 0) return DT_OK;
  hipLaunchKernelGGL(k_downslope, dim3((unsigned)((n + 255) / 256)), dim3(256), 0, s, dem, fdr, (int)H,
                     (int)W, px, dz, raw, out);
  return DT_OK;
}

__global__ __launch_bounds__(256) void k_hand_i64(const float *__restrict__ dem,
                                                 const int64_t *__restrict__ idx, int64_t n,
                                                 float *__restrict__ hand) {
  int64_t i = (int64_t)blockIdx.x * 256 + threadIdx.x;
  if (i >= n) return;
  float z = dem[i], h = DT_NODATA;
  int64_t k = idx[i];
  if (z != DT_NODATA && k != -100) {
    if (k < 0) k += n;
    if (k >= 0 && k < n) {
      h = z - dem[k];
      if (h < 0.0f && h != DT_NODATA) h = 0.0f;
    }
  }
  hand[i] = h;
}
int dt_launch_hand_i64(hipStream_t s, const float *dem, const int64_t *idx, int64_t n, float *hand) {
  if (n) hipLaunchKernelGGL(k_hand_i64, dim3((unsigned)((n + 255) / 256)), dim3(256), 0, s, dem, idx, n, hand);
  return DT_OK;
}

#define CF_MAXT 24
struct CfThresholds {
  double v[CF_MAXT];
};

__global__ __launch_bounds__(256) void k_confusion(const double *__restrict__ desc,
                                                  const int8_t *__restrict__ flood, int64_t n,
                                                  double nodata, int nth, int under,
                                                  CfThresholds th,
                                                  unsigned long long *__restrict__ counts4) {
  unsigned int b0[CF_MAXT], b2[CF_MAXT];
#pragma unroll
  for (int t = 0; t < CF_MAXT; t++) b0[t] = b2[t] = 0u;
  unsigned int t0 = 0u, t2 = 0u, t3 = 0u;
  int64_t stride = (int64_t)gridDim.x * 256;
  for (int64_t i = (int64_t)blockIdx.x * 256 + threadIdx.x; i < n; i += stride) {
    double v = desc[i];
    int g = flood[i];
    if (g == 1) g = 2;
    else if (g == -100) g = 0;
    bool isn = (v == nodata) || (v != v);
    if (g == 0 || g == 2) {
      if (g == 0) t0++; else t2++;
#pragma unroll
      for (int t = 0; t < CF_MAXT; t++) {
        bool bin = !isn && (t < nth) && (under ? (v <= th.v[t]) : (v >= th.v[t]));
        b0[t] += (bin && g == 0) ? 1u : 0u;
        b2[t] += (bin && g == 2) ? 1u : 0u;
      }
    } else {
      for (int t = 0; t < nth; t++) {
        int bin = (!isn && (under ? (v <= th.v[t]) : (v >= th.v[t]))) ? 1 : 0;
        int r = bin + g;
        if (r >= 0 && r <= 3) atomicAdd(&counts4[t * 4 + r], 1ull);
      }
    }
  }
  (void)t3;
  for (int off = 32; off > 0; off >>= 1) {
    t0 += __shfl_down(t0, off);
    t2 += __shfl_down(t2, off);
#pragma unroll
    for (int t = 0; t < CF_MAXT; t++) {
      b0[t] += __shfl_down(b0[t], off);
      b2[t] += __shfl_down(b2[t], off);
    }
  }
  if ((threadIdx.x & 63) == 0) {
#pragma unroll
    for (int t = 0; t < CF_MAXT; t++) {
      if (t < nth) {
        atomicAdd(&counts4[t * 4 + 0], (unsigned long long)(t0 - b0[t]));
        atomicAdd(&counts4[t * 4 + 1], (unsigned long long)b0[t]);
// ... 274 lines not shown
```

descriptools_amd/csrc/dt_tiles.hip:

```cpp
#include "dt_common.h"
#include "dt_kernels.h"
#include "dt_math.h"

#define TW 64
#define TH 64
#define NT (TW * TH)
#define PS (2 * TW + 2 * (TH - 2))
#define CPT (NT / 256)

#define NX_SINK 0xFFFFu
#define NX_EXIT 0xFFFEu
#define NX_REXIT 0xFFFDu
#define X_NONE 0xFFFFu

__device__ __forceinline__ int dt_slot_of(int ly, int lx) {
  if (ly == 0) return lx;
  if (ly == TH - 1) return TW + lx;
  if (lx == 0) return 2 * TW + (ly - 1);
  if (lx == TW - 1) return 2 * TW + (TH - 2) + (ly - 1);
  return -1;
}
__device__ __forceinline__ void dt_cell_of_slot(int s, int &ly, int &lx) {
  if (s < TW) { ly = 0; lx = s; }
  else if (s < 2 * TW) { ly = TH - 1; lx = s - TW; }
  else if (s < 2 * TW + (TH - 2)) { ly = s - 2 * TW + 1; lx = 0; }
  else { ly = s - 2 * TW - (TH - 2) + 1; lx = TW - 1; }
}
__device__ __forceinline__ uint32_t dt_node_of(int y, int x, int tiles_x) {
  int ty = y / TH, tx = x / TW;
  return (uint32_t)((ty * tiles_x + tx) * PS + dt_slot_of(y - ty * TH, x - tx * TW));
}

__device__ __forceinline__ int dt_tile_of_block(int b, int ntiles) {
  const int full = ntiles & ~15;
  if (b >= full) return b;
  const int xcd = b & 7, j = b >> 3;
  return ((j >> 1) * 8 + xcd) * 2 + (j & 1);
}

__device__ __forceinline__ uint4 dt_tile_fetch16(const uint8_t *__restrict__ fdr, const DtWin &w, int y0, int x0) {
  int t = threadIdx.x;
  int r = t >> 2, c = (t & 3) * 16;
  int gy = y0 + r, gx = x0 + c;
  uint4 v = make_uint4(0, 0, 0, 0);
  if (gy < w.H) {
    const uint8_t *p = fdr + (long long)gy * w.ld + gx;
    if (gx + 15 < w.W && (((uintptr_t)p) & 15) == 0) {
      v = *reinterpret_cast<const uint4 *>(p);
    } else {
      uint32_t w4[4] = {0, 0, 0, 0};
#pragma unroll
      for (int k = 0; k < 16; k++)
        if (gx + k < w.W) w4[k >> 2] |= (uint32_t)p[k] << (8 * (k & 3));
      v = make_uint4(w4[0], w4[1], w4[2], w4[3]);
    }
  }
  return v;
}
__device__ __forceinline__ void dt_tile_put16(uint8_t *s_fdr, uint4 v) {
  int t = threadIdx.x;
  *reinterpret_cast<uint4 *>(&s_fdr[(t >> 2) * TW + (t & 3) * 16]) = v;
}
__device__ __forceinline__ void dt_tile_load_fdr(const uint8_t *__restrict__ fdr, const DtWin &w, int y0,
                                                 int x0, uint8_t *s_fdr) {
  dt_tile_put16(s_fdr, dt_tile_fetch16(fdr, w, y0, x0));
}

__device__ __forceinline__ uint32_t dt_tile_next(uint32_t code, int ly, int lx, int y0, int x0,
                                                const DtWin &w) {
  int y = y0 + ly, x = x0 + lx;
  if (y >= w.H || x >= w.W || !dt_d8_valid(code)) return NX_SINK;
  int dy, dx;
  dt_d8_delta(code, dy, dx);
  int ty = y + dy, tx = x + dx;
  if (!dt_in_core(w, ty, tx)) return dt_in_global(w, ty, tx) ? NX_REXIT : NX_SINK;
  int ny = ly + dy, nx = lx + dx;
  if (ny < 0 || ny >= TH || nx < 0 || nx >= TW) return NX_EXIT;
  return (uint32_t)(ny * TW + nx);
}

__device__ __forceinline__ bool dt_tile_interior(const DtWin &w, int y0, int x0) {
  return y0 >= 1 && x0 >= 1 && y0 + TH + 1 <= w.H && x0 + TW + 1 <= w.W;
}
__device__ __forceinline__ uint32_t dt_tile_next_interior(uint32_t code, int ly, int lx) {
  if (!dt_d8_valid(code)) return NX_SINK;
  int dy, dx;
  dt_d8_delta(code, dy, dx);
  uint32_t ny = (uint32_t)(ly + dy), nx = (uint32_t)(lx + dx);
  return (ny < (uint32_t)TH && nx < (uint32_t)TW) ? ny * TW + nx : NX_EXIT;
}

#define PT_ALIVE 0x8000u
#define PT_EXIT 0x4000u
#define PT_IDX 0x0FFFu

__device__ __forceinline__ void dt_tile_sums_packed(uint32_t *s_word, uint8_t *s_cyc, uint32_t (&va)[CPT / 2],
                                                    uint32_t (&vb)[CPT / 2]) {
  uint32_t P[CPT / 2];
  unsigned long long *s_word2 = reinterpret_cast<unsigned long long *>(s_word);
#pragma unroll
  for (int j = 0; j < CPT / 2; j++) {
    unsigned long long r = s_word2[threadIdx.x + 256 * j];
    P[j] = ((uint32_t)r >> 16) | ((uint32_t)(r >> 32) & 0xFFFF0000u);
    va[j] = vb[j] = 1u;
  }
  for (int round = 0; round < 12; round++) {
    uint32_t jumped = 0;
#pragma unroll
    for (int j = 0; j < CPT / 2; j++) {
      const uint32_t p = P[j];
      if (p & PT_ALIVE) {
        P[j] = (P[j] & 0xFFFF0000u) | (atomicAdd(&s_word[p & PT_IDX], min(va[j], (uint32_t)NT)) >> 16);
        jumped |= 1u << j;
      }
// ... 878 lines not shown
  __syncthreads();
  uint32_t nx[CPT];
#pragma unroll
  for (int j = 0; j < CPT; j++) {
    const int c = threadIdx.x + 256 * j;
    nx[j] = dt_tile_next(s_fdr[c], c / TW, c % TW, y0, x0, w);
  }
  __syncthreads();
#pragma unroll
  for (int j = 0; j < CPT; j++) {
    const int c = threadIdx.x + 256 * j;
    s_nxt[P3(c)] = (uint16_t)(nx[j] < NT ? P3(nx[j]) : nx[j]);
    s_delta[P3(c)] = 0ull;
  }
  __syncthreads();
  if (e != 0ull) {
    int ly, lx;
    dt_cell_of_slot(threadIdx.x, ly, lx);
    uint32_t c = P3(ly * TW + lx);
    if (e & FAW_CYC) {
      for (int it = 0; it < NT && c < NT3; it++) {
        atomicOr(&s_delta[c], FAW_CYC);
        c = s_nxt[c];
      }
    } else {
      for (int it = 0; it < NT && c < NT3; it++) {
        atomicAdd(&s_delta[c], e);
        c = s_nxt[c];
      }
    }
  }
  __syncthreads();
#pragma unroll
  for (int j = 0; j < CPT; j++) {
    const int c = threadIdx.x + 256 * j;
    const int y = y0 + c / TW, x = x0 + c % TW;
    if (y >= w.H || x >= w.W) continue;
    const unsigned long long d = s_delta[P3(c)];
    const bool dead = lv[j] == FAW_LOC_CYC || (d & FAW_CYC) || (HAS_DEM && zv[j] <= DT_NODATA);
    acc[(long long)y * w.ld + x] = dead ? -100.0 : ldexp((double)(lv[j] + d), -sbits);
  }
}
#undef P3
#undef NT3

struct FawScratch {
  unsigned long long *rec, *state, *loc;
  uint32_t *parent;
  int64_t nnodes, ntiles;
  int tiles_x;
  size_t bytes;
};
static FawScratch faw_layout(const DtWin &w, void *scratch) {
  FawScratch f;
  f.tiles_x = (w.W + TW - 1) / TW;
  f.ntiles = (int64_t)f.tiles_x * ((w.H + TH - 1) / TH);
  f.nnodes = f.ntiles * PS;
  DtCarver c(scratch);
  f.rec = c.take<unsigned long long>((size_t)f.nnodes);
  f.state = c.take<unsigned long long>((size_t)f.nnodes);
  f.parent = c.take<uint32_t>((size_t)f.nnodes);
  f.loc = c.take<unsigned long long>((size_t)f.ntiles * NT);
  f.bytes = c.bytes();
  return f;
}
size_t dt_flowacc_weighted_scratch(int64_t H, int64_t W) { return faw_layout(dt_full_window(H, W), nullptr).bytes; }

int dt_launch_flowacc_weighted(hipStream_t s, const DtWin &w, const uint8_t *fdr, const float *dem, const double *wt,
                               int frac_bits, void *scratch, size_t scratch_bytes, double *acc, int *status) {
  if (w.H == 0 || w.W == 0) return DT_OK;
  FawScratch f = faw_layout(w, scratch);
  DT_REQUIRE(scratch_bytes >= f.bytes, "scratch too small");
  DT_REQUIRE(f.nnodes < 0x7FFFFFF0ll, "raster too large for one device tile");
  const unsigned long long qmax = (1ull << 52) / (unsigned long long)((int64_t)w.H * w.W);
  dim3 gt((unsigned)f.ntiles), b(256), gn((unsigned)((f.nnodes + 255) / 256));
  hipLaunchKernelGGL(k_faw_tile1, gt, b, 0, s, fdr, wt, w, f.tiles_x, frac_bits, qmax, f.rec, f.state, f.parent,
                     f.loc, status);
  hipLaunchKernelGGL(k_faw_reduce, gn, b, 0, s, f.rec, f.nnodes, f.parent, f.state);
  if (dem) hipLaunchKernelGGL(k_faw_tile3<true>, gt, b, 0, s, fdr, dem, w, f.tiles_x, f.rec, f.state, f.loc, frac_bits, acc);
  else hipLaunchKernelGGL(k_faw_tile3<false>, gt, b, 0, s, fdr, dem, w, f.tiles_x, f.rec, f.state, f.loc, frac_bits, acc);
  return DT_OK;
}

#define FHT_DEAD 0xFFFFFFFFu
#define FHT_REMOTE 0x80000000u
#define FHT_DONE 0x8000u
#define FHT_CAP 20000u
#define K_RIVER 1u
#define K_DEAD 2u
#define K_EXIT 3u
#define K_REXIT 4u

__device__ __forceinline__ unsigned long long fht_pack(uint32_t ptr, uint32_t nd, uint32_t ncf) {
  return ((unsigned long long)ptr << 32) | ((unsigned long long)nd << 16) | (unsigned long long)ncf;
}

struct FhTile {
  uint8_t *s_fdr;
  uint8_t *s_halo;
  unsigned long long *s_st;
};

__device__ __forceinline__ uint32_t fht_fdr_at(const FhTile &T, int ly, int lx) {
  if (ly >= 0 && ly < TH && lx >= 0 && lx < TW) return T.s_fdr[ly * TW + lx];
  if (ly < 0) return T.s_halo[lx + 1];
  if (ly >= TH) return T.s_halo[(TW + 2) + lx + 1];
  if (lx < 0) return T.s_halo[2 * (TW + 2) + ly];
  return T.s_halo[2 * (TW + 2) + TH + ly];
}

__device__ __forceinline__ void fht_solve_tile(const FhTile &T, const uint8_t *__restrict__ fdr,
                                               const int8_t *__restrict__ river, const DtWin &w, int y0,
                                               int x0) {
  dt_tile_load_fdr(fdr, w, y0, x0, T.s_fdr);
  for (int i = threadIdx.x; i < 2 * (TW + 2) + 2 * TH; i += 256) {
    int y, x;
    if (i < TW + 2) { y = y0 - 1; x = x0 - 1 + i; }
    else if (i < 2 * (TW + 2)) { y = y0 + TH; x = x0 - 1 + (i - (TW + 2)); }
    else if (i < 2 * (TW + 2) + TH) { y = y0 + (i - 2 * (TW + 2)); x = x0 - 1; }
    else { y = y0 + (i - 2 * (TW + 2) - TH); x = x0 + TW; }
    uint8_t v = 0;
    if (dt_readable(w, y, x)) v = fdr[(long long)y * w.ld + x];
    T.s_halo[i] = v;
  }
  uint8_t *s_riv = reinterpret_cast<uint8_t *>(T.s_st);
  dt_tile_load_fdr(reinterpret_cast<const uint8_t *>(river), w, y0, x0, s_riv);
  __syncthreads();
  uint32_t riv = 0;
  for (int j = 0; j < CPT; j++) {
    int c = threadIdx.x + 256 * j;
    if (s_riv[c] == 1) riv |= 1u << j;
  }
  __syncthreads();
  if (dt_tile_interior(w, y0, x0)) {
#pragma unroll
    for (int j = 0; j < CPT; j++) {
      int c = threadIdx.x + 256 * j;
      int ly = c / TW, lx = c % TW;
      uint32_t code = T.s_fdr[c];
      uint32_t ptr = (uint32_t)c | (K_DEAD << 12), lo = FHT_DONE;
      if (code != 0u && ((riv >> j) & 1u)) {
        ptr = (uint32_t)c | (K_RIVER << 12);
      } else if (dt_d8_valid(code)) {
        int dy, dx;
        dt_d8_delta(code, dy, dx);
        uint32_t ny = (uint32_t)(ly + dy), nx = (uint32_t)(lx + dx);
        bool in_tile = ny < (uint32_t)TH && nx < (uint32_t)TW;
        uint32_t tcode = in_tile ? (uint32_t)T.s_fdr[ny * TW + nx] : fht_fdr_at(T, ly + dy, lx + dx);
        if (tcode != 0u) {
          if (in_tile) {
            bool diag = dy != 0 && dx != 0;
            ptr = ny * TW + nx;
            lo = diag ? (1u << 16) : 1u;
          } else {
            ptr = (uint32_t)c | (K_EXIT << 12);
          }
        }
      }
      T.s_st[c] = ((unsigned long long)ptr << 32) | (unsigned long long)lo;
    }
  } else {
    for (int j = 0; j < CPT; j++) {
      int c = threadIdx.x + 256 * j;
      int ly = c / TW, lx = c % TW;
      int y = y0 + ly, x = x0 + lx;
      uint32_t code = T.s_fdr[c];
      unsigned long long s;
      if (y >= w.H || x >= w.W || code == 0u) {
        s = fht_pack((uint32_t)c | (K_DEAD << 12), 0, FHT_DONE);
      } else if ((riv >> j) & 1u) {
        s = fht_pack((uint32_t)c | (K_RIVER << 12), 0, FHT_DONE);
      } else if (!dt_d8_valid(code)) {
        s = fht_pack((uint32_t)c | (K_DEAD << 12), 0, FHT_DONE);
      } else {
        int dy, dx;
        dt_d8_delta(code, dy, dx);
        int ty = y + dy, tx = x + dx;
        if (!dt_in_global(w, ty, tx) || fht_fdr_at(T, ly + dy, lx + dx) == 0u) {
          s = fht_pack((uint32_t)c | (K_DEAD << 12), 0, FHT_DONE);
        } else if (!dt_in_core(w, ty, tx)) {
          s = fht_pack((uint32_t)c | (K_REXIT << 12), 0, FHT_DONE);
        } else if (ly + dy < 0 || ly + dy >= TH || lx + dx < 0 || lx + dx >= TW) {
          s = fht_pack((uint32_t)c | (K_EXIT << 12), 0, FHT_DONE);
        } else {
          bool diag = dy != 0 && dx != 0;
          s = fht_pack((uint32_t)((ly + dy) * TW + lx + dx), diag ? 1u : 0u, diag ? 0u : 1u);
        }
      }
      T.s_st[c] = s;
    }
  }
  __syncthreads();
  ulonglong2 *s_st2 = reinterpret_cast<ulonglong2 *>(T.s_st);
  for (int round = 0; round < 13; round++) {
    int changed = 0;
#pragma unroll
    for (int j = 0; j < CPT / 2; j++) {
      int c2 = threadIdx.x + 256 * j;
      ulonglong2 s = s_st2[c2];
      bool dx = ((uint32_t)s.x & FHT_DONE) != 0u, dy = ((uint32_t)s.y & FHT_DONE) != 0u;
      if (dx && dy) continue;
      if (!dx) {
        unsigned long long t = T.s_st[(uint32_t)(s.x >> 32) & 0xFFFu];
        s.x = (t & 0xFFFFFFFF00000000ull) | (unsigned long long)((uint32_t)s.x + (uint32_t)t);
      }
      if (!dy) {
        unsigned long long t = T.s_st[(uint32_t)(s.y >> 32) & 0xFFFu];
        s.y = (t & 0xFFFFFFFF00000000ull) | (unsigned long long)((uint32_t)s.y + (uint32_t)t);
      }
      s_st2[c2] = s;
      changed |= (((uint32_t)s.x & (uint32_t)s.y & FHT_DONE) == 0u) ? 1 : 0;
    }
    if (!__syncthreads_or(changed)) break;
  }
#pragma unroll
  for (int j = 0; j < CPT; j++) {
    int c = threadIdx.x + 256 * j;
    if (!((uint32_t)T.s_st[c] & FHT_DONE)) T.s_st[c] = fht_pack((uint32_t)c | (K_DEAD << 12), 0, FHT_DONE);
  }
  __syncthreads();
}

__device__ __forceinline__ uint32_t fh_cache_pack(unsigned long long s) {
  uint32_t ptr = (uint32_t)(s >> 32);
  return (ptr & 0x7FFFu) | ((uint32_t)((s >> 16) & 0xFFu) << 15) | ((uint32_t)(s & 0xFFu) << 23);
}
__device__ __forceinline__ unsigned long long fh_cache_unpack(uint32_t v) {
  return fht_pack(v & 0x7FFFu, (v >> 15) & 0xFFu, ((v >> 23) & 0xFFu) | FHT_DONE);
}
__device__ __forceinline__ unsigned long long fh_cache_get(const unsigned long long *__restrict__ cache, bool wide,
                                                            int tile, int c) {
  if (wide) return cache[(size_t)tile * NT + c];
  return fh_cache_unpack(reinterpret_cast<const uint32_t *>(cache + (size_t)tile * NT)[c]);
}

__global__ __launch_bounds__(256) void k_fh_tile1(const uint8_t *__restrict__ fdr,
                                                 const int8_t *__restrict__ river, DtWin w, int tiles_x,
                                                 uint32_t nnodes, unsigned long long *__restrict__ nodes,
                                                 unsigned long long *__restrict__ cache,
                                                 uint8_t *__restrict__ cache_wide, int only_marked, int ntiles) {
  __shared__ __attribute__((aligned(16))) uint8_t s_fdr[NT];
  __shared__ uint8_t s_halo[2 * (TW + 2) + 2 * TH];
  __shared__ __attribute__((aligned(16))) unsigned long long s_st[NT];
  for (int tile = (int)blockIdx.x; tile < ntiles; tile += (int)gridDim.x) {
  if (only_marked && cache_wide[tile] != 2) continue;
  const int ty = tile / tiles_x, tx = tile - ty * tiles_x;
  const int y0 = ty * TH, x0 = tx * TW;
  FhTile T{s_fdr, s_halo, s_st};
  fht_solve_tile(T, fdr, river, w, y0, x0);
  if (threadIdx.x < PS) {
    int ly, lx;
    dt_cell_of_slot(threadIdx.x, ly, lx);
    unsigned long long s = s_st[ly * TW + lx];
    uint32_t ptr = (uint32_t)(s >> 32), nd = (uint32_t)((s >> 16) & 0xFFFFu);
    uint32_t ncf = (uint32_t)(s & 0xFFFFu), nc = ncf & 0x7FFFu;
    uint32_t kind = (ptr >> 12) & 7u, f = ptr & 0xFFFu;
    int fy = (int)f / TW, fx = (int)f % TW;
    unsigned long long o = fht_pack(FHT_DEAD, 0, FHT_DONE);
    if (!(ncf & FHT_DONE)) {
    } else if (kind == K_RIVER) {
      o = fht_pack((uint32_t)((y0 + fy) * w.W + x0 + fx), nd, nc | FHT_DONE);
    } else if (kind == K_EXIT || kind == K_REXIT) {
      int dy, dx;
      dt_d8_delta(s_fdr[f], dy, dx);
      bool diag = dy != 0 && dx != 0;
      uint32_t node = kind == K_EXIT ? dt_node_of(y0 + fy + dy, x0 + fx + dx, tiles_x)
                                     : nnodes + (uint32_t)dt_perim_index(w.H, w.W, y0 + fy, x0 + fx);
      o = fht_pack(node, nd + (diag ? 1u : 0u), nc + (diag ? 0u : 1u));
    }
    nodes[(size_t)tile * PS + threadIdx.x] = o;
  }
  unsigned long long wv[CPT];
  int wide = 0;
#pragma unroll
  for (int j = 0; j < CPT; j++) {
    wv[j] = s_st[threadIdx.x + 256 * j];
    wide |= (((uint32_t)wv[j] & 0x7FFFu) > 255u || ((uint32_t)(wv[j] >> 16) & 0xFFFFu) > 255u) ? 1 : 0;
  }
  wide = __syncthreads_or(wide);
  if (threadIdx.x == 0) cache_wide[tile] = (uint8_t)wide;
  if (wide) {
#pragma unroll
    for (int j = 0; j < CPT; j++) cache[(size_t)tile * NT + threadIdx.x + 256 * j] = wv[j];
  } else {
    uint32_t *c32 = reinterpret_cast<uint32_t *>(cache + (size_t)tile * NT);
#pragma unroll
    for (int j = 0; j < CPT; j++) c32[threadIdx.x + 256 * j] = fh_cache_pack(wv[j]);
  }
  __syncthreads();
  }
}

#define FN_CNT 0x3FFFFu
#define FN_DONE 0x40000u
#define FN_LOW 0x7FFFFu
#define FN_OVF 0x20100u
#define FN_PTR_SH 19
__device__ __forceinline__ uint32_t fh_lut_entry(uint32_t code) {
  if (!dt_d8_valid(code)) return 0u;
  int dy, dx;
  dt_d8_delta(code, dy, dx);
  return ((uint32_t)(dy * TW + dx) << FN_PTR_SH) + ((dy != 0 && dx != 0) ? (1u << 9) : 1u);
}
__device__ __forceinline__ void fh_tile1n_body(uint8_t *s_fdr, uint32_t *s_w, uint8_t *s_kind, int *s_ovf_p,
                                               const uint32_t *s_lut, const uint32_t (&riv4)[NT / 4 / 256],
                                               const DtWin &w, int tile, int tiles_x, int y0, int x0, uint32_t nnodes,
                                               unsigned long long *__restrict__ nodes,
                                               unsigned long long *__restrict__ cache,
                                               uint8_t *__restrict__ cache_wide) {
#define s_ovf (*s_ovf_p)
  const bool interior = dt_tile_interior(w, y0, x0);
  const uint32_t lx0 = (4u * threadIdx.x) & 63u;
#pragma unroll
  for (int u = 0; u < NT / 4 / 256; u++) {
    const int c0 = 4 * (threadIdx.x + 256 * u);
    const uint32_t codes = *reinterpret_cast<const uint32_t *>(&s_fdr[c0]);
// ... 166 lines not shown
  if (i < P) nodes[nnodes + i] = fht_pack(nnodes + (uint32_t)i, 0, 0);
}

__global__ __launch_bounds__(256) void k_fh_node_jump(unsigned long long *__restrict__ state, int64_t n,
                                                      int *__restrict__ flags, int round, int hops) {
  if (flags && round > 0 && flags[round - 1] == 0) {
    if (blockIdx.x == 0 && threadIdx.x == 0) flags[round] = 0;
    return;
  }
  bool pending = false;
  for (int64_t i = (int64_t)blockIdx.x * 256 + threadIdx.x; i < n; i += (int64_t)gridDim.x * 256) {
    unsigned long long s = __hip_atomic_load(&state[i], __ATOMIC_RELAXED, __HIP_MEMORY_SCOPE_AGENT);
    bool open = false, changed = false;
    for (int h = 0; h < hops; h++) {
      const uint32_t ncf = (uint32_t)(s & 0xFFFFu);
      const uint32_t ptr = (uint32_t)(s >> 32), nd = (uint32_t)((s >> 16) & 0xFFFFu);
      if ((ncf & FHT_DONE) || ptr == (uint32_t)i) break;
      const unsigned long long t = __hip_atomic_load(&state[ptr], __ATOMIC_RELAXED, __HIP_MEMORY_SCOPE_AGENT);
      const uint32_t tptr = (uint32_t)(t >> 32), tnd = (uint32_t)((t >> 16) & 0xFFFFu);
      const uint32_t tncf = (uint32_t)(t & 0xFFFFu);
      const uint32_t nnc = ncf + (tncf & 0x7FFFu), nnd = nd + tnd;
      if (((tncf & FHT_DONE) && tptr == FHT_DEAD) || nnc + nnd > FHT_CAP) s = fht_pack(FHT_DEAD, 0, FHT_DONE);
      else s = fht_pack(tptr, nnd, nnc | (tncf & FHT_DONE));
      changed = true;
      open = !(s & (unsigned long long)FHT_DONE) && tptr != ptr;
      if (!open) break;
    }
    if (changed) __hip_atomic_store(&state[i], s, __ATOMIC_RELAXED, __HIP_MEMORY_SCOPE_AGENT);
    pending = pending || open;
  }
  if (flags && __any(pending) && (threadIdx.x & 63) == 0) flags[round] = 1;
}

template <typename AccT>
__global__ __launch_bounds__(256) void k_fh_rank_summary(DtWin w, int tiles_x, uint32_t nnodes,
                                                        const unsigned long long *__restrict__ nodes,
                                                        const float *__restrict__ dem,
                                                        const AccT *__restrict__ acc32, int64_t P,
                                                        uint8_t *__restrict__ kind, int32_t *__restrict__ ref,
                                                        int32_t *__restrict__ nc, int32_t *__restrict__ nd,
                                                        float *__restrict__ zr, long long *__restrict__ ar) {
  int64_t i = (int64_t)blockIdx.x * 256 + threadIdx.x;
  if (i >= P) return;
  int y, x;
  dt_perim_cell(w.H, w.W, i, y, x);
  const bool has_node = dt_slot_of(y % TH, x % TW) >= 0;
  unsigned long long s = has_node ? nodes[dt_node_of(y, x, tiles_x)] : fht_pack(FHT_DEAD, 0, FHT_DONE);
  uint32_t ptr = (uint32_t)(s >> 32), ncf = (uint32_t)(s & 0xFFFFu);
  uint8_t k = (uint8_t)K_DEAD;
  int32_t r = -1;
  float z = DT_NODATA;
  long long a = 0;
  if (ncf & FHT_DONE) {
    if (ptr != FHT_DEAD) {
      k = (uint8_t)K_RIVER;
      r = (int32_t)ptr;
      long long o = (long long)(ptr / (uint32_t)w.W) * w.ld + (ptr % (uint32_t)w.W);
      if (dem) z = dem[o];
      if (acc32) a = (long long)acc32[o];
    }
  } else if (ptr >= nnodes) {
    k = (uint8_t)K_REXIT;
    r = (int32_t)(ptr - nnodes);
  }
  kind[i] = k;
  ref[i] = r;
  nc[i] = (int32_t)(ncf & 0x7FFFu);
  nd[i] = (int32_t)((s >> 16) & 0xFFFFu);
  zr[i] = z;
  ar[i] = a;
}

__global__ __launch_bounds__(256) void k_fh_ghost_set(unsigned long long *__restrict__ nodes, uint32_t nnodes,
                                                     int64_t P, const uint8_t *__restrict__ res_ok,
                                                     const int32_t *__restrict__ res_nc,
                                                     const int32_t *__restrict__ res_nd) {
  int64_t i = (int64_t)blockIdx.x * 256 + threadIdx.x;
  if (i >= P) return;
  unsigned long long o = fht_pack(FHT_DEAD, 0, FHT_DONE);
  if (res_ok[i]) o = fht_pack(FHT_REMOTE | (uint32_t)i, (uint32_t)res_nd[i], (uint32_t)res_nc[i] | FHT_DONE);
  nodes[nnodes + i] = o;
}

struct FhGfi {
  float *gfi, *lnhlh;
  double expo, c0;
  const DtLogEntry *tab;
};
struct FhRemote {
  const long long *gidx;
  const float *zr;
  const long long *ar;
};
template <typename AccT>
struct FhPay;
template <>
struct FhPay<int32_t> {
  unsigned long long v[PS];
  __device__ __forceinline__ void set(int i, float z, int32_t a) {
    v[i] = ((unsigned long long)(uint32_t)a << 32) | (unsigned long long)__float_as_uint(z);
  }
  __device__ __forceinline__ void get(int i, float &z, int32_t &a) const {
    const unsigned long long p = v[i];
    z = __uint_as_float((uint32_t)p);
    a = (int32_t)(uint32_t)(p >> 32);
  }
};
template <>
struct FhPay<long long> {
  long long av[PS];
  float zv[PS];
  __device__ __forceinline__ void set(int i, float z, long long a) {
    av[i] = a;
    zv[i] = z;
  }
  __device__ __forceinline__ void get(int i, float &z, long long &a) const {
    z = zv[i];
    a = av[i];
  }
};

typedef float fh_v4f __attribute__((ext_vector_type(4)));
typedef int fh_v4i __attribute__((ext_vector_type(4)));
__device__ __forceinline__ void fh_store4(float *p, float a, float b, float c, float d) {
  fh_v4f v = {a, b, c, d};
  __builtin_nontemporal_store(v, reinterpret_cast<fh_v4f *>(p));
}
__device__ __forceinline__ void fh_store4(int32_t *p, int32_t a, int32_t b, int32_t c, int32_t d) {
  fh_v4i v = {a, b, c, d};
  __builtin_nontemporal_store(v, reinterpret_cast<fh_v4i *>(p));
}
typedef long long fh_v2l __attribute__((ext_vector_type(2)));
__device__ __forceinline__ void fh_store4(long long *p, long long a, long long b, long long c, long long d) {
  fh_v2l v0 = {a, b}, v1 = {c, d};
  __builtin_nontemporal_store(v0, reinterpret_cast<fh_v2l *>(p));
  __builtin_nontemporal_store(v1, reinterpret_cast<fh_v2l *>(p + 2));
}

template <bool RANKED, int VH, int MINW, typename AccT>
__global__ __launch_bounds__(256, MINW) void k_fh_tile3(const uint8_t *__restrict__ fdr,
                                                 const float *__restrict__ dem,
                                                 const AccT *__restrict__ acc32, DtWin w, int tiles_x,
                                                 uint32_t nnodes, const unsigned long long *__restrict__ nodes,
                                                 const unsigned long long *__restrict__ cache,
                                                 const uint8_t *__restrict__ cache_wide,
                                                 FhRemote rem, double px, float *__restrict__ fdist,
                                                 int32_t *__restrict__ idx32, long long *__restrict__ idx64,
                                                 float *__restrict__ hand, AccT *__restrict__ a_river,
                                                 FhGfi G) {
  __shared__ unsigned long long s_x[PS];
  __shared__ FhPay<AccT> s_pay;
  __shared__ DtLogEntry s_tab[DT_LOGTAB_N];
  if (G.gfi) dt_math_stage(G.tab, s_tab);
  const int tile = dt_tile_of_block((int)blockIdx.x, (int)gridDim.x);
  const int ty = tile / tiles_x, tx = tile - ty * tiles_x;
  const int y0 = ty * TH, x0 = tx * TW;
  const bool wide = cache_wide[tile] != 0;
  if (threadIdx.x < PS) {
    int ly, lx;
    dt_cell_of_slot(threadIdx.x, ly, lx);
    int f = ly * TW + lx;
    unsigned long long s = fh_cache_get(cache, wide, tile, f);
    uint32_t sp = (uint32_t)(s >> 32);
    unsigned long long o = fht_pack(FHT_DEAD, 0, FHT_DONE);
    float zr = DT_NODATA;
    AccT ar = -100;
    bool ex = sp == ((uint32_t)f | (K_EXIT << 12)), rex = sp == ((uint32_t)f | (K_REXIT << 12));
    if (ex || rex) {
      int dy, dx;
      dt_d8_delta(fdr[(long long)(y0 + ly) * w.ld + x0 + lx], dy, dx);
      size_t node = ex ? (size_t)dt_node_of(y0 + ly + dy, x0 + lx + dx, tiles_x)
                       : (size_t)nnodes + (size_t)dt_perim_index(w.H, w.W, y0 + ly, x0 + lx);
      unsigned long long ns = nodes[node];
      uint32_t nptr = (uint32_t)(ns >> 32), nnd = (uint32_t)((ns >> 16) & 0xFFFFu);
      uint32_t nncf = (uint32_t)(ns & 0xFFFFu);
      if (RANKED && !(nncf & FHT_DONE) && nptr >= nnodes && (size_t)nptr != node) {
        unsigned long long gs = nodes[nptr];
        uint32_t gncf = (uint32_t)(gs & 0xFFFFu);
        nnd += (uint32_t)((gs >> 16) & 0xFFFFu);
        const uint32_t cnt = (nncf & 0x7FFFu) + (gncf & 0x7FFFu);
        nptr = (uint32_t)(gs >> 32);
        if ((gncf & FHT_DONE) && nptr != FHT_DEAD && cnt + nnd <= FHT_CAP) nncf = cnt | FHT_DONE;
        else nptr = FHT_DEAD;
      }
      bool diag = dy != 0 && dx != 0;
      if ((nncf & FHT_DONE) && nptr != FHT_DEAD) {
        o = fht_pack(nptr, nnd + (diag ? 1u : 0u), ((nncf & 0x7FFFu) + (diag ? 0u : 1u)) | FHT_DONE);
        if (RANKED && (nptr & FHT_REMOTE)) {
          zr = rem.zr[nptr & ~FHT_REMOTE];
          ar = (AccT)rem.ar[nptr & ~FHT_REMOTE];
        } else {
          long long ro = (long long)(nptr / (uint32_t)w.W) * w.ld + (nptr % (uint32_t)w.W);
          if (dem) zr = dem[ro];
          if (acc32) ar = acc32[ro];
        }
      }
    }
    s_x[threadIdx.x] = o;
    s_pay.set((int)threadIdx.x, zr, ar);
  }
  const bool vec = x0 + TW <= w.W && (w.ld & 3) == 0 && (!dem || ((uintptr_t)dem & 15) == 0) &&
                   (!fdist || ((uintptr_t)fdist & 15) == 0) && (!idx32 || ((uintptr_t)idx32 & 15) == 0) &&
                   (!idx64 || ((uintptr_t)idx64 & 15) == 0) && (!hand || ((uintptr_t)hand & 15) == 0) &&
                   (!a_river || ((uintptr_t)a_river & 15) == 0) &&
                   (!G.gfi || ((((uintptr_t)G.gfi | (uintptr_t)G.lnhlh | (uintptr_t)acc32) & 15) == 0));
  const double dcard = px, ddiag = px * sqrt(2.0);
  struct CellOut {
    float fd, h;
    int32_t i32;
    AccT ar;
    long long i64;
  };
  auto solve = [&](unsigned long long s, float z) -> CellOut {
    uint32_t ptr = (uint32_t)(s >> 32), nd = (uint32_t)((s >> 16) & 0xFFFFu);
    uint32_t ncf = (uint32_t)(s & 0xFFFFu), nc = ncf & 0x7FFFu;
    uint32_t kind = (ptr >> 12) & 7u, f = ptr & 0xFFFu;
    bool ok = false;
    uint32_t ridx = 0;
    float pz = 0.0f;
    AccT pa = 0;
    if (ncf & FHT_DONE) {
      if (kind == K_RIVER) {
        ok = true;
        ridx = (uint32_t)((y0 + (int)f / TW) * w.W + x0 + (int)f % TW);
        long long ro = (long long)(y0 + (int)f / TW) * w.ld + x0 + (int)f % TW;
        pz = dem ? dem[ro] : DT_NODATA;
        pa = acc32 ? acc32[ro] : (AccT)-100;
      } else if (kind == K_EXIT || kind == K_REXIT) {
        int slot = dt_slot_of((int)f / TW, (int)f % TW);
        unsigned long long xs = s_x[slot];
        uint32_t xptr = (uint32_t)(xs >> 32);
        if (xptr != FHT_DEAD) {
          nc += (uint32_t)(xs & 0x7FFFu);
          nd += (uint32_t)((xs >> 16) & 0xFFFFu);
          ok = nc + nd <= FHT_CAP;
          ridx = xptr;
          s_pay.get(slot, pz, pa);
        }
      }
    }
    const bool remote = RANKED && ok && (ridx & FHT_REMOTE) != 0u;
    CellOut o;
    o.fd = ok ? (float)(dcard * (double)nc + ddiag * (double)nd) : DT_NODATA;
    o.i32 = (ok && !remote) ? (int32_t)ridx : -100;
    o.i64 = -100;
    if (RANKED && ok) {
      o.i64 = remote ? rem.gidx[ridx & ~FHT_REMOTE]
                     : (long long)(w.gy0 + (int)(ridx / (uint32_t)w.W)) * w.Wg + w.gx0 + (int)(ridx % (uint32_t)w.W);
      o.i32 = (int32_t)o.i64;
    }
    o.h = DT_NODATA;
    if (z != DT_NODATA && ok) {
      o.h = z - pz;
      if (o.h < 0.0f && o.h != DT_NODATA) o.h = 0.0f;
    }
    o.ar = ok ? pa : (AccT)-100;
    return o;
  };
  if (vec) {
    constexpr int VPT = NT / 4 / 256;
#pragma unroll 1
    for (int h = 0; h < VPT / VH; h++) {
      uint4 wa[VH], wb[VH];
      float4 z4[VH];
#pragma unroll
      for (int u = 0; u < VH; u++) {
        int c = 4 * (threadIdx.x + 256 * (h * VH + u));
        if (wide) {
          const uint4 *cp = reinterpret_cast<const uint4 *>(cache + (size_t)tile * NT + c);
          wa[u] = cp[0];
          wb[u] = cp[1];
        } else {
          uint4 v = *reinterpret_cast<const uint4 *>(reinterpret_cast<const uint32_t *>(cache + (size_t)tile * NT) + c);
          unsigned long long a = fh_cache_unpack(v.x), b2 = fh_cache_unpack(v.y), c2 = fh_cache_unpack(v.z),
                             d2 = fh_cache_unpack(v.w);
          wa[u] = make_uint4((uint32_t)a, (uint32_t)(a >> 32), (uint32_t)b2, (uint32_t)(b2 >> 32));
          wb[u] = make_uint4((uint32_t)c2, (uint32_t)(c2 >> 32), (uint32_t)d2, (uint32_t)(d2 >> 32));
        }
        int y = y0 + c / TW;
        z4[u] = make_float4(DT_NODATA, DT_NODATA, DT_NODATA, DT_NODATA);
        if (dem && y < w.H) z4[u] = *reinterpret_cast<const float4 *>(dem + (long long)y * w.ld + x0 + c % TW);
      }
      if (h == 0) __syncthreads();
#pragma unroll
      for (int u = 0; u < VH; u++) {
        int c = 4 * (threadIdx.x + 256 * (h * VH + u));
        int y = y0 + c / TW;
        if (y >= w.H) continue;
        long long o = (long long)y * w.ld + x0 + c % TW;
        CellOut r0 = solve(((unsigned long long)wa[u].y << 32) | wa[u].x, z4[u].x);
        CellOut r1 = solve(((unsigned long long)wa[u].w << 32) | wa[u].z, z4[u].y);
        CellOut r2 = solve(((unsigned long long)wb[u].y << 32) | wb[u].x, z4[u].z);
        CellOut r3 = solve(((unsigned long long)wb[u].w << 32) | wb[u].z, z4[u].w);
        if (fdist) fh_store4(fdist + o, r0.fd, r1.fd, r2.fd, r3.fd);
        if (idx32) fh_store4(idx32 + o, r0.i32, r1.i32, r2.i32, r3.i32);
        if (RANKED && idx64) {
          *reinterpret_cast<longlong2 *>(idx64 + o) = make_longlong2(r0.i64, r1.i64);
          *reinterpret_cast<longlong2 *>(idx64 + o + 2) = make_longlong2(r2.i64, r3.i64);
        }
        if (hand) fh_store4(hand + o, r0.h, r1.h, r2.h, r3.h);
        if (a_river) fh_store4(a_river + o, r0.ar, r1.ar, r2.ar, r3.ar);
        if (G.gfi) {
          AccT fx, fy, fz, fw;
          if (sizeof(AccT) == 8) {
            const longlong2 fa = *reinterpret_cast<const longlong2 *>(acc32 + o);
            const longlong2 fb = *reinterpret_cast<const longlong2 *>(acc32 + o + 2);
            fx = (AccT)fa.x; fy = (AccT)fa.y; fz = (AccT)fb.x; fw = (AccT)fb.y;
          } else {
            const int4 f = *reinterpret_cast<const int4 *>(acc32 + o);
            fx = (AccT)f.x; fy = (AccT)f.y; fz = (AccT)f.z; fw = (AccT)f.w;
          }
          float4 g, l;
          dt_gfi_both_cell(r0.h, r0.ar, fx, G.expo, G.c0, s_tab, g.x, l.x);
          __builtin_amdgcn_sched_barrier(0);
          dt_gfi_both_cell(r1.h, r1.ar, fy, G.expo, G.c0, s_tab, g.y, l.y);
          __builtin_amdgcn_sched_barrier(0);
          dt_gfi_both_cell(r2.h, r2.ar, fz, G.expo, G.c0, s_tab, g.z, l.z);
          __builtin_amdgcn_sched_barrier(0);
          dt_gfi_both_cell(r3.h, r3.ar, fw, G.expo, G.c0, s_tab, g.w, l.w);
          fh_store4(G.gfi + o, g.x, g.y, g.z, g.w);
          fh_store4(G.lnhlh + o, l.x, l.y, l.z, l.w);
        }
        __builtin_amdgcn_sched_barrier(0);
      }
    }
    return;
  }
  __syncthreads();
#pragma unroll 1
  for (int j = 0; j < CPT; j++) {
    int c = threadIdx.x + 256 * j;
    int y = y0 + c / TW, x = x0 + c % TW;
    if (y >= w.H || x >= w.W) continue;
    long long o = (long long)y * w.ld + x;
    CellOut r = solve(fh_cache_get(cache, wide, tile, c), dem ? dem[o] : DT_NODATA);
    if (fdist) fdist[o] = r.fd;
    if (idx32) idx32[o] = r.i32;
    if (RANKED && idx64) idx64[o] = r.i64;
    if (hand) hand[o] = r.h;
    if (a_river) a_river[o] = r.ar;
    if (G.gfi) {
// ... 82 lines not shown
    const FaIn in = fa_inputs(f, ext_perim);
    int32_t thr = river_thr > 2147483647ll ? 2147483647 : (river_thr < -2147483647ll ? -2147483647 : (int32_t)river_thr);
    const bool use_mask = nod4 != nullptr && w.halo == 0 && w.gx0 == 0 && w.gy0 == 0;
    if (twi) {
      DT_REQUIRE(dt_twi_epilogue_ok(w, acc, river, twi) && use_mask && !ext_perim,
                 "the TI / MTI epilogue takes a single raster with its nodata mask (dt_twi_epilogue_ok)");
      const int64_t stx = (w.W + 255) / 256, sntiles = stx * ((w.H + 15) / 16);
      const DtStencilAux S = dt_stencil_aux_layout(sntiles, twi->marks);
      TwiOut tw{twi->slope, twi->ti, twi->mti, twi->n_top, log(twi->px * twi->px), S.mark, (uint32_t *)S.lmask, (int)stx};
      hipLaunchKernelGGL(k_fa3fh1_twi, gt, b, 0, s, fdr, dem, nod4, ldm, w, f.tiles_x, in.rec, in.state, in.ext, f.loc16,
                         (int32_t *)acc, thr, river, status, (uint32_t)h.nnodes, h.nodes, h.cache, h.cache_wide, tw);
    } else if (use_mask)
      hipLaunchKernelGGL(k_fa3fh1<2>, gt, b, 0, s, fdr, dem, nod4, ldm, w, f.tiles_x, in.rec, in.state, in.ext, f.loc16, (int32_t *)acc, thr,
                         river, status, (uint32_t)h.nnodes, h.nodes, h.cache, h.cache_wide);
    else if (dem)
      hipLaunchKernelGGL(k_fa3fh1<1>, gt, b, 0, s, fdr, dem, nod4, ldm, w, f.tiles_x, in.rec, in.state, in.ext, f.loc16, (int32_t *)acc, thr,
                         river, status, (uint32_t)h.nnodes, h.nodes, h.cache, h.cache_wide);
    else
      hipLaunchKernelGGL(k_fa3fh1<0>, gt, b, 0, s, fdr, dem, nod4, ldm, w, f.tiles_x, in.rec, in.state, in.ext, f.loc16, (int32_t *)acc, thr,
                         river, status, (uint32_t)h.nnodes, h.nodes, h.cache, h.cache_wide);
  } else {
    DT_REQUIRE(!twi, "the TI / MTI epilogue needs the fused form of the tile passes (dt_twi_epilogue_ok)");
    if (acc64) {
      fa_launch_tile3<long long>(s, gt, w, fdr, dem, f, ext_perim, (long long *)acc, (long long)river_thr, river, status);
    } else {
      int32_t thr = river_thr > 2147483647ll ? 2147483647 : (river_thr < -2147483647ll ? -2147483647 : (int32_t)river_thr);
      fa_launch_tile3<int32_t>(s, gt, w, fdr, dem, f, ext_perim, (int32_t *)acc, thr, river, status);
    }
    hipLaunchKernelGGL(k_fh_tile1n, gt, b, 0, s, fdr, river, w, h.tiles_x, (uint32_t)h.nnodes, h.nodes, h.cache,
                       h.cache_wide);
  }
  return fh_local_tail(s, w, fdr, river, h);
}

int dt_launch_fh_summary(hipStream_t s, const DtWin &w, void *scratch, const float *dem, const void *acc, int acc64,
                         uint8_t *kind, int32_t *ref, int32_t *nc, int32_t *nd, float *zr, long long *ar) {
  FhScratch f = fh_layout(w, scratch);
  if (f.P == 0) return DT_OK;
  dim3 g((unsigned)((f.P + 255) / 256)), b(256);
  if (acc64)
    hipLaunchKernelGGL(k_fh_rank_summary<long long>, g, b, 0, s, w, f.tiles_x, (uint32_t)f.nnodes, f.nodes, dem,
                       (const long long *)acc, f.P, kind, ref, nc, nd, zr, ar);
  else
    hipLaunchKernelGGL(k_fh_rank_summary<int32_t>, g, b, 0, s, w, f.tiles_x, (uint32_t)f.nnodes, f.nodes, dem,
                       (const int32_t *)acc, f.P, kind, ref, nc, nd, zr, ar);
  return DT_OK;
}

int dt_launch_fh_finish(hipStream_t s, const DtWin &w, const float *dem, const uint8_t *fdr,
                        const int8_t *river, const void *acc, int acc64, double px, void *scratch,
                        const uint8_t *res_ok, const int32_t *res_nc, const int32_t *res_nd,
                        const long long *rem_gidx, const float *rem_zr, const long long *rem_ar, float *fdist,
                        int32_t *idx32, long long *idx64, float *hand, void *a_river, float *gfi,
                        float *lnhlh, double n_gfi, double b_gfi, double size) {
  if (w.H == 0 || w.W == 0) return DT_OK;
  FhScratch f = fh_layout(w, scratch);
  dim3 gt((unsigned)f.ntiles), b(256), gn((unsigned)((f.nnodes + f.P + 255) / 256));
  if (res_ok) {
    hipLaunchKernelGGL(k_fh_ghost_set, dim3((unsigned)((f.P + 255) / 256)), b, 0, s, f.nodes, (uint32_t)f.nnodes,
                       f.P, res_ok, res_nc, res_nd);
  }
  FhRemote rem{rem_gidx, rem_zr, rem_ar};
  FhGfi G{nullptr, nullptr, 0.0, 0.0, nullptr};
  if (gfi && lnhlh) {
    DT_REQUIRE(dem && acc, "fused GFI needs dem and the accumulation raster");
    G = FhGfi{gfi, lnhlh, n_gfi, log(b_gfi) + n_gfi * log(size * size), dt_math_device_table(s)};
  }
  (void)river;
  const bool ranked = res_ok || idx64;
#define FH_GO(R, MW, T)                                                                                                \
  hipLaunchKernelGGL((k_fh_tile3<R, 1, MW, T>), gt, b, 0, s, fdr, dem, (const T *)acc, w, f.tiles_x, (uint32_t)f.nnodes, \
                     f.nodes, f.cache, f.cache_wide, rem, px, fdist, idx32, idx64, hand, (T *)a_river, G)
  if (acc64) {
    if (ranked) FH_GO(true, 4, long long);
    else FH_GO(false, 4, long long);
  } else {
    if (ranked) FH_GO(true, 5, int32_t);
    else FH_GO(false, 5, int32_t);
  }
#undef FH_GO
  return DT_OK;
}

#define RK_MAX 64
struct RkLayout {
  int ty, tx, nranks;
  long long Pmax;
  int ys[RK_MAX + 1], xs[RK_MAX + 1];
  int Hg, Wg;
};
__device__ __forceinline__ void rk_rank_geom(const RkLayout &L, int r, int &y0, int &x0, int &H, int &W) {
  int ry = r / L.tx, rx = r - ry * L.tx;
  y0 = L.ys[ry];
  x0 = L.xs[rx];
  H = L.ys[ry + 1] - y0;
  W = L.xs[rx + 1] - x0;
}
__device__ __forceinline__ long long rk_step_target(const RkLayout &L, int r, long long i, uint32_t code) {
  if (!dt_d8_valid(code)) return -1;
  int y0, x0, H, W;
  rk_rank_geom(L, r, y0, x0, H, W);
  if (i >= dt_perim_count(H, W)) return -1;
  int y, x, dy, dx;
  dt_perim_cell(H, W, i, y, x);
  dt_d8_delta(code, dy, dx);
  int ty = y + dy, tx = x + dx;
  if (ty >= 0 && ty < H && tx >= 0 && tx < W) return -1;
  int gy = y0 + ty, gx = x0 + tx;
  if (gy < 0 || gy >= L.Hg || gx < 0 || gx >= L.Wg) return -1;
  int ry = 0, rx = 0;
  while (gy >= L.ys[ry + 1]) ry++;
  while (gx >= L.xs[rx + 1]) rx++;
  int r2 = ry * L.tx + rx, y2, x2, H2, W2;
  rk_rank_geom(L, r2, y2, x2, H2, W2);
  return (long long)r2 * L.Pmax + dt_perim_index(H2, W2, gy - y2, gx - x2);
}

struct RkRows {
  const unsigned char *buf;
  long long rowbytes;
  long long off[8];
};
template <typename T>
__device__ __forceinline__ T rk_get(const RkRows &R, int field, int r, long long i) {
  return reinterpret_cast<const T *>(R.buf + (long long)r * R.rowbytes + R.off[field])[i];
}

__global__ __launch_bounds__(256) void k_rk_fa_link(RkLayout L, RkRows R, int32_t *__restrict__ entry_of,
                                                   int32_t *__restrict__ parent, uint32_t *__restrict__ pending) {
  long long n = (long long)blockIdx.x * 256 + threadIdx.x;
  if (n >= (long long)L.nranks * L.Pmax) return;
  int r = (int)(n / L.Pmax);
  long long i = n - (long long)r * L.Pmax;
  long long e = rk_step_target(L, r, i, rk_get<uint8_t>(R, 2, r, i));
  int32_t par = -1;
  if (e >= 0) {
    int r2 = (int)(e / L.Pmax);
    int32_t xr = rk_get<int32_t>(R, 1, r2, e - (long long)r2 * L.Pmax);
    if (xr >= 0) {
      par = (int32_t)((long long)r2 * L.Pmax + xr);
      atomicAdd(&pending[par], 1u);
    }
  }
  entry_of[n] = (int32_t)e;
  parent[n] = par;
}
__global__ __launch_bounds__(256) void k_rk_fa_sources(long long nn, const int32_t *__restrict__ entry_of,
                                                      const uint32_t *__restrict__ pending,
                                                      uint8_t *__restrict__ is_src) {
  long long n = (long long)blockIdx.x * 256 + threadIdx.x;
  if (n >= nn) return;
  is_src[n] = (entry_of[n] >= 0 && pending[n] == 0u) ? 1 : 0;
}
__global__ __launch_bounds__(256) void k_rk_fa_reduce(RkLayout L, RkRows R, const int32_t *__restrict__ entry_of,
                                                     const int32_t *__restrict__ parent,
                                                     const uint8_t *__restrict__ is_src,
                                                     uint32_t *__restrict__ pending,
                                                     unsigned long long *__restrict__ sum,
                                                     unsigned long long *__restrict__ ext) {
  long long n = (long long)blockIdx.x * 256 + threadIdx.x;
  long long nn = (long long)L.nranks * L.Pmax;
  if (n >= nn) return;
  if (!is_src[n]) return;
  long long q = n;
  int rq = (int)(q / L.Pmax);
  unsigned long long A = (unsigned long long)rk_get<long long>(R, 0, rq, q - (long long)rq * L.Pmax);
// ... 194 lines not shown
```

include/descriptools_hip.h:

```cpp
#ifndef DESCRIPTOOLS_HIP_H
#define DESCRIPTOOLS_HIP_H

#include <stdint.h>

#ifdef __cplusplus
extern "C" {
#endif

#define DT_OK 0
#define DT_EINVAL (-1)
#define DT_EHIP (-2)
#define DT_ENOMEM (-3)
#define DT_ENODEV (-4)

typedef struct dt_ctx dt_ctx;

typedef struct dt_window {
  int64_t H, W, ld, gy0, gx0, Hg, Wg, halo;
} dt_window;

const char *dt_last_error(void);
int dt_device_count(void);
const char *dt_version(void);
int dt_set_flow_impl(int impl);
// ... 169 lines not shown
int dt_dev_hand_gfi_f64(dt_ctx *ctx, const double *dem, const int32_t *idx32, const int32_t *acc32, int64_t H,
                        int64_t W, double px, double n_gfi, double scale_factor, double *hand, float *gfi,
                        float *lnhlh);
int dt_dev_river_mask(dt_ctx *ctx, const int32_t *acc32, int64_t N, int64_t threshold,
                      int8_t *river);
int dt_dev_flowhand(dt_ctx *ctx, const float *dem, const uint8_t *fdr, const int8_t *river,
                    const int32_t *acc32, int64_t H, int64_t W, double px, float *fdist,
                    int32_t *idx32, float *hand, int32_t *a_river);
int dt_dev_flowhand_gfi(dt_ctx *ctx, const float *dem, const uint8_t *fdr, const int8_t *river,
                        const int32_t *acc32, int64_t H, int64_t W, double px, double n_gfi, double b,
                        float *fdist, int32_t *idx32, float *hand, int32_t *a_river, float *gfi, float *lnhlh);
int dt_dev_twi(dt_ctx *ctx, const int32_t *acc32, const float *slope_rad, int64_t N, double px,
               double n_top, float *ti, float *mti);
int dt_dev_gfi(dt_ctx *ctx, const float *hand, const int32_t *a_river, int64_t N, double n_gfi,
               double scale_factor, double size, float *gfi);
int dt_dev_lnhlh(dt_ctx *ctx, const float *hand, const int32_t *acc32, int64_t N, double n_gfi,
                 double scale_factor, double size, float *out);
int dt_dev_gfi_lnhlh(dt_ctx *ctx, const float *hand, const int32_t *a_river, const int32_t *acc32,
                     int64_t N, double n_gfi, double scale_factor, double size, float *gfi, float *lnhlh);
int dt_dev_downslope(dt_ctx *ctx, const float *dem, const uint8_t *fdr, int64_t H, int64_t W,
                     double px, double elevation_difference, int raw, float *out);
int64_t dt_downslope_lift_workspace(int64_t H, int64_t W);
int dt_dev_downslope_lift(dt_ctx *ctx, const float *dem, const uint8_t *fdr, int64_t H, int64_t W, double px,
                          double dz, int raw, float *out, void *work, int64_t work_bytes);
int64_t dt_downslope_queue_workspace(int64_t H, int64_t W);
int64_t dt_downslope_tables_workspace(int64_t H, int64_t W);
int64_t dt_downslope_tables_threshold(int64_t H, int64_t W);
int dt_dev_downslope_queue(dt_ctx *ctx, const float *dem, const uint8_t *fdr, int64_t H, int64_t W, double px,
                           double dz, int raw, float *out, void *qwork, int64_t qbytes);
int dt_dev_downslope_queued(dt_ctx *ctx, const void *qwork, int64_t *count);
int dt_dev_downslope_finish(dt_ctx *ctx, const float *dem, const uint8_t *fdr, int64_t H, int64_t W, double px,
                            double dz, int raw, float *out, void *qwork, int64_t qbytes, void *twork, int64_t tbytes);
int dt_dev_confusion_multi(dt_ctx *ctx, const double *desc, const int8_t *flood, int64_t N,
                           double nodata_value, const double *th_host, int nth, int under,
                           int64_t *counts4_dev);
int64_t dt_perim_cells(int64_t H, int64_t W);
int dt_dev_condition_stage_w(dt_ctx *ctx, const dt_window *win, int stage, int rounds, const float *dem, float *filled,
                             uint8_t *fdr, uint32_t *dist, int32_t *flag_dev);
int dt_dev_condition_stage_m_w(dt_ctx *ctx, const dt_window *win, int stage, int rounds, const float *dem, float *filled,
                               uint8_t *fdr, uint32_t *dist, int32_t *flag_dev, uint8_t *nsame);
int dt_dev_slope_d8_w(dt_ctx *ctx, const dt_window *win, const float *dem, double px, float *slope,
                      uint8_t *fdr, float *slope_rad);
int dt_dev_slope_twi_w(dt_ctx *ctx, const dt_window *win, const float *dem, const int32_t *acc32, double px,
                       double n_top, float *slope, float *slope_rad, float *ti, float *mti);
int dt_dev_downslope_w(dt_ctx *ctx, const dt_window *win, const float *dem, const uint8_t *fdr, double px,
                       double elevation_difference, int raw, float *out, int32_t *n_unresolved_dev);
int64_t dt_downslope_lift_workspace_w(const dt_window *win);
int dt_dev_downslope_lift_w(dt_ctx *ctx, const dt_window *win, const float *dem, const uint8_t *fdr, double px,
                            double elevation_difference, int raw, float *out, int32_t *n_unresolved_dev, void *work,
                            int64_t work_bytes);
int dt_dev_downslope_emit_w(dt_ctx *ctx, const dt_window *win, const float *dem, const uint8_t *fdr, double px,
                            double elevation_difference, int raw, float *out, int32_t *n_unresolved_dev, void *work,
                            int64_t work_bytes, void *walkers, int64_t walkers_bytes);
int dt_dev_downslope_walk_w(dt_ctx *ctx, const dt_window *win, const float *dem, const uint8_t *fdr, double px,
                            double elevation_difference, int64_t n, void *records, void *work, int64_t work_bytes);
int dt_dev_downslope_walk_route_w(dt_ctx *ctx, const dt_window *win, const float *dem, const uint8_t *fdr, double px,
                                  double elevation_difference, int64_t n, void *records, void *work, int64_t work_bytes,
                                  float *out, const int32_t *row_starts, int32_t ty, const int32_t *col_starts,
                                  int32_t tx, void *send, int32_t *counts, int32_t *scratch);
int dt_dev_downslope_walk_seed_w(dt_ctx *ctx, const dt_window *win, const float *dem, int64_t n, const int32_t *ys,
                                 const int32_t *xs, void *records);
int dt_dev_flowacc_local_w(dt_ctx *ctx, const dt_window *win, const uint8_t *fdr, int32_t *acc32,
                           int64_t *A_perim, int32_t *xr_perim, uint8_t *code_perim);
int dt_dev_flowacc_finish_w(dt_ctx *ctx, const dt_window *win, const uint8_t *fdr, const float *dem,
                            const uint64_t *ext_perim, int64_t threshold, int32_t *acc32, int8_t *river);
int dt_dev_flowacc_finish_flowhand_local_w(dt_ctx *ctx, const dt_window *win, const uint8_t *fdr, const float *dem,
                                           const uint64_t *ext_perim, int64_t threshold, int32_t *acc32, int8_t *river,
                                           uint8_t *kind, int32_t *ref, int32_t *nc, int32_t *nd, float *zr,
                                           int64_t *ar);
int dt_dev_flowhand_local_w(dt_ctx *ctx, const dt_window *win, const float *dem, const uint8_t *fdr,
                            const int8_t *river, const int32_t *acc32, uint8_t *kind, int32_t *ref,
                            int32_t *nc, int32_t *nd, float *zr, int64_t *ar);
int dt_dev_flowhand_finish_w(dt_ctx *ctx, const dt_window *win, const float *dem, const uint8_t *fdr,
                             const int8_t *river, const int32_t *acc32, double px, const uint8_t *res_ok,
                             const int32_t *res_nc, const int32_t *res_nd, const int64_t *rem_gidx,
                             const float *rem_zr, const int64_t *rem_ar, float *fdist, int32_t *idx32,
                             int64_t *idx64, float *hand, int32_t *a_river);
int dt_dev_flowhand_gfi_finish_w(dt_ctx *ctx, const dt_window *win, const float *dem, const uint8_t *fdr,
                                 const int8_t *river, const int32_t *acc32, double px, double n_gfi, double b,
                                 const uint8_t *res_ok, const int32_t *res_nc, const int32_t *res_nd,
                                 const int64_t *rem_gidx, const float *rem_zr, const int64_t *rem_ar,
                                 float *fdist, int32_t *idx32, int64_t *idx64, float *hand, int32_t *a_river,
                                 float *gfi, float *lnhlh);

int dt_dev_slope_d8_f64_w(dt_ctx *ctx, const dt_window *win, const double *dem, double px, uint8_t *fdr, float *proxy);
int dt_dev_slope_twi_f64_w(dt_ctx *ctx, const dt_window *win, const double *dem, const int32_t *acc32, double px,
                           double n_top, float *slope, float *slope_rad, float *ti, float *mti);
int dt_dev_slope_twi_f64_w_a64(dt_ctx *ctx, const dt_window *win, const double *dem, const int64_t *acc64, double px,
                               double n_top, float *slope, float *slope_rad, float *ti, float *mti);
int dt_dev_downslope_f64_w(dt_ctx *ctx, const dt_window *win, const double *dem, const uint8_t *fdr, double px,
                           double elevation_difference, int raw, float *out, int32_t *n_unresolved_dev);
int dt_dev_downslope_walk_seed_f64_w(dt_ctx *ctx, const dt_window *win, const double *dem, int64_t n, const int32_t *ys,
                                     const int32_t *xs, void *records);
int dt_dev_downslope_walk_route_f64_w(dt_ctx *ctx, const dt_window *win, const double *dem, const uint8_t *fdr,
                                      double px, double elevation_difference, int64_t n, void *records, float *out,
                                      const int32_t *row_starts, int32_t ty, const int32_t *col_starts, int32_t tx,
                                      void *send, int32_t *counts, int32_t *scratch);
int dt_dev_flowhand_zr64_w(dt_ctx *ctx, const dt_window *win, const double *dem, int64_t n, const uint8_t *kind,
                           const int32_t *ref, double *zr64);
int dt_dev_rank_solve_flowhand_f64(dt_ctx *ctx, int ty, int tx, const int64_t *heights, const int64_t *widths,
                                   int64_t Pmax, const void *rows_dev, int64_t rowbytes,
                                   const int64_t *field_offsets8, int rank, int64_t P_rank, uint8_t *res_ok,
                                   int32_t *res_nc, int32_t *res_nd, int64_t *rem_gidx, float *rem_zr,
                                   int64_t *rem_ar, double *rem_zr64);
int64_t dt_hand_f64_table_bytes(int64_t n_remote);
int dt_dev_hand_gfi_f64_w(dt_ctx *ctx, const dt_window *win, const double *dem, const int32_t *idx32,
                          const int64_t *idx64, const int32_t *acc32, const int32_t *a_river32, int64_t n_remote,
                          const uint8_t *res_ok, const int64_t *rem_gidx, const double *rem_zr64, void *table,
                          int64_t table_bytes, double px, double n_gfi, double scale_factor, double *hand, float *gfi,
                          float *lnhlh);
int dt_dev_hand_gfi_f64_w_a64(dt_ctx *ctx, const dt_window *win, const double *dem, const int32_t *idx32,
                              const int64_t *idx64, const int64_t *acc64, const int64_t *a_river64, int64_t n_remote,
                              const uint8_t *res_ok, const int64_t *rem_gidx, const double *rem_zr64, void *table,
                              int64_t table_bytes, double px, double n_gfi, double scale_factor, double *hand,
                              float *gfi, float *lnhlh);

int dt_dev_flowacc_finish_w_a64(dt_ctx *ctx, const dt_window *win, const uint8_t *fdr, const float *dem,
                                const uint64_t *ext_perim, int64_t threshold, int64_t *acc64, int8_t *river);
int dt_dev_flowacc_finish_flowhand_local_w_a64(dt_ctx *ctx, const dt_window *win, const uint8_t *fdr, const float *dem,
                                               const uint64_t *ext_perim, int64_t threshold, int64_t *acc64,
                                               int8_t *river, uint8_t *kind, int32_t *ref, int32_t *nc, int32_t *nd,
                                               float *zr, int64_t *ar);
int dt_dev_slope_twi_w_a64(dt_ctx *ctx, const dt_window *win, const float *dem, const int64_t *acc64, double px,
                           double n_top, float *slope, float *slope_rad, float *ti, float *mti);
int dt_dev_flowhand_local_w_a64(dt_ctx *ctx, const dt_window *win, const float *dem, const uint8_t *fdr,
                                const int8_t *river, const int64_t *acc64, uint8_t *kind, int32_t *ref,
                                int32_t *nc, int32_t *nd, float *zr, int64_t *ar);
int dt_dev_flowhand_finish_w_a64(dt_ctx *ctx, const dt_window *win, const float *dem, const uint8_t *fdr,
                                 const int8_t *river, const int64_t *acc64, double px, const uint8_t *res_ok,
                                 const int32_t *res_nc, const int32_t *res_nd, const int64_t *rem_gidx,
                                 const float *rem_zr, const int64_t *rem_ar, float *fdist, int32_t *idx32,
                                 int64_t *idx64, float *hand, int64_t *a_river64);
int dt_dev_flowhand_gfi_finish_w_a64(dt_ctx *ctx, const dt_window *win, const float *dem, const uint8_t *fdr,
                                     const int8_t *river, const int64_t *acc64, double px, double n_gfi, double b,
                                     const uint8_t *res_ok, const int32_t *res_nc, const int32_t *res_nd,
                                     const int64_t *rem_gidx, const float *rem_zr, const int64_t *rem_ar,
                                     float *fdist, int32_t *idx32, int64_t *idx64, float *hand,
                                     int64_t *a_river64, float *gfi, float *lnhlh);
int dt_dev_gfi_lnhlh_a64(dt_ctx *ctx, const float *hand, const int64_t *a_river64, const int64_t *acc64, int64_t N,
                         double n_gfi, double scale_factor, double size, float *gfi, float *lnhlh);

int dt_dev_unique_extremes_f32(dt_ctx *ctx, const float *x, int64_t N, float *out3_dev);
int dt_dev_minmax_scale_f32(dt_ctx *ctx, const float *x, int64_t N, float mn, float mx, float nodata,
                            double *desc);

int dt_dev_minmax_scale_f32_f64(dt_ctx *ctx, const float *x, int64_t N, double mn, double mx, double nodata,
                                double *desc);
int dt_dev_classify(dt_ctx *ctx, const double *desc, int8_t *flood, int64_t N, double nodata_value, double threshold,
                    int under, int remap_flood, uint8_t *binary, int32_t *klass, int64_t *counts4_dev);

int dt_dev_membench_copy(dt_ctx *ctx, const float *a, float *b, int64_t N, int blocks);
int dt_dev_membench_mix(dt_ctx *ctx, const float *r0, const float *r1, float *w0, float *w1, float *w2, int64_t N,
                        int n_reads, int n_writes, int nontemporal);
int dt_dev_membench_mix_timed(dt_ctx *ctx, const float *r0, const float *r1, float *w0, float *w1, float *w2, int64_t N,
                              int n_reads, int n_writes, int nontemporal, int reps, double *ms);
int dt_dev_mem_info(dt_ctx *ctx, int64_t *free_bytes, int64_t *total_bytes);

int dt_dev_rank_solve_flowacc(dt_ctx *ctx, int ty, int tx, const int64_t *heights, const int64_t *widths,
                              int64_t Pmax, const void *rows_dev, int64_t rowbytes,
                              const int64_t *field_offsets3, int rank, int64_t P_rank, uint64_t *ext_out_dev);
int dt_dev_rank_solve_flowhand(dt_ctx *ctx, int ty, int tx, const int64_t *heights, const int64_t *widths,
                               int64_t Pmax, const void *rows_dev, int64_t rowbytes,
                               const int64_t *field_offsets7, int rank, int64_t P_rank, uint8_t *res_ok,
                               int32_t *res_nc, int32_t *res_nd, int64_t *rem_gidx, float *rem_zr,
                               int64_t *rem_ar);

// ... 8 lines not shown
```

Before: 36000 Mcells/s.

## Fuse flowhand GFI finish with downslope into one tail kernel

Adds a fused tail kernel that computes the flowhand/HAND finish with GFI and ln(hl/H) together with the downslope descriptor in a single pass over tiles. It runs serially on the main stream instead of running downslope on a side stream. The aim is to share DEM/fdr reads and cut a separate launch and pass over memory, and the placement groups put 'down' with the HAND outputs. The trade-off is that downslope no longer overlaps with other work on a side context, and the kernel may carry more register and LDS pressure.

```diff
diff --git a/descriptools_amd/_lib.py b/descriptools_amd/_lib.py
--- a/descriptools_amd/_lib.py
+++ b/descriptools_amd/_lib.py
@@ -139,6 +139,9 @@
     "dt_dev_flowhand_gfi": (ci, [vp, vp, vp, vp, vp, i64, i64, f64, f64, f64, vp, vp, vp, vp, vp, vp]),
     "dt_dev_flowhand_gfi_finish_w": (ci, [vp, vp, vp, vp, vp, vp, f64, f64, f64, vp, vp, vp, vp, vp,
                                           vp, vp, vp, vp, vp, vp, vp, vp]),
+    "dt_tail_fused_ok": (ci, [i64, i64]),
+    "dt_dev_flowhand_gfi_finish_downslope": (ci, [vp, vp, vp, vp, vp, vp, f64, f64, f64, vp, vp, vp, vp, vp, vp, f64,
+                                                  ci, vp]),
     "dt_ctx_set_priority": (ci, [vp, ci]),
     "dt_ctx_fork": (ci, [vp, vp]),
     "dt_ctx_join": (ci, [vp, vp]),
diff --git a/descriptools_amd/build.py b/descriptools_amd/build.py
--- a/descriptools_amd/build.py
+++ b/descriptools_amd/build.py
@@ -8,6 +8,7 @@
 SOURCES = ["dt_kernels.hip", "dt_stencil.hip", "dt_tiles.hip", "dt_hydro.hip", "dt_wide.hip", "dt_streams.hip",
            "dt_watershed.hip", "dt_reaches.hip", "dt_dinf.hip", "dt_proximity.hip", "dt_capi.hip"]
 HEADERS = ["dt_common.h", "dt_kernels.h", "dt_math.h", "dt_math_coeffs.h", "dt_d8_kernel.inc", "dt_fa3fh1_kernel.inc",
+           "dt_fh_tail.h", "dt_fh_solve.inc",
            os.path.join("..", "..", "include", "descriptools_hip.h")]
 FLAGS = ["-O3", "--offload-arch=gfx950", "-fPIC", "-std=c++17", "-ffp-contract=off", "-fno-fast-math",
          "-Wall", "-Wno-unused-function"]
diff --git a/descriptools_amd/chain.py b/descriptools_amd/chain.py
--- a/descriptools_amd/chain.py
+++ b/descriptools_amd/chain.py
@@ -16,6 +16,8 @@
 
 WRITE_GROUPS = (("slope", "ti", "mti"), ("fdist", "idx", "hand", "gfi", "lnhlh"), ("fac",), ("a_river",),
                 ("slope_rad",), ("down",))
+WRITE_GROUPS_FUSED_TAIL = (("slope", "ti", "mti"), ("fdist", "idx", "hand", "gfi", "lnhlh", "down"), ("fac",),
+                           ("a_river",), ("slope_rad",))
 
 OPS = (
     ("d8", 5, ["k_d8<false>", "k_d8_fix"]),
@@ -120,7 +122,8 @@
                 b.free()
             else:
                 self._release(int(b.ptr.value if hasattr(b, "ptr") else b))
-        groups = [[k for k in g if k in four] for g in WRITE_GROUPS]
+        written_together = WRITE_GROUPS_FUSED_TAIL if self._tail_shape() else WRITE_GROUPS
+        groups = [[k for k in g if k in four] for g in written_together]
         roles, info = placement.assign(self.ctx, self.N * 4, list(objs), [g for g in groups if g],
                                        extra_alloc if can_grow else None, extra_release if can_grow else None,
                                        spacer_alloc=spacer_alloc if can_grow else None,
@@ -232,6 +235,24 @@
         ptrs = [self.p(k) for k in ("slope", "fac", "ti", "mti", "river", "fdr")] + ([dem_ptr] if dem_ptr else [])
         return all((int(q.value if hasattr(q, "value") else q) & 15) == 0 for q in ptrs)
 
+    def _tail_shape(self):
+        return (not self.wide and self.long_walks is False
+                and bool(_lib.lib().dt_tail_fused_ok(self.H, self.W)))
+
+    def _fused_tail(self, dem_ptr, want_a_river):
+        if not self._tail_shape():
+            return None
+        L, c, p = _lib.lib(), self.ctx, self.p
+        names = ["fdr", "fac", "fdist", "idx", "hand", "gfi", "lnhlh", "down"] + (["a_river"] if want_a_river else [])
+        ptrs = [p(k) for k in names] + [dem_ptr]
+        if any((int(q.value if hasattr(q, "value") else q) & 15) != 0 for q in ptrs):
+            return None
+        if getattr(self, "_full", None) is None:
+            self._full = _lib.Window(self.H, self.W, self.W, 0, 0, self.H, self.W, 0)
+        return lambda: L.dt_dev_flowhand_gfi_finish_downslope(
+            c.h, C.byref(self._full), dem_ptr, p("fdr"), p("river"), p("fac"), self.px, self.n_gfi, self.b, p("fdist"),
+            p("idx"), p("hand"), p("a_river") if want_a_river else None, p("gfi"), p("lnhlh"), self.dz, 0, p("down"))
+
     def _ops_f64(self, dem_ptr, want_a_river, side):
         L, c, H, W, p = _lib.lib(), self.ctx, self.H, self.W, self.p
         prox = self._proxy.ptr
@@ -255,11 +276,16 @@
         ]
 
     def run(self, dem_ptr, want_a_river=True):
-        for name, ctx, call in self.ops(dem_ptr, want_a_river):
+        tail = self._fused_tail(dem_ptr, want_a_river)
+        for name, ctx, call in self.ops(dem_ptr, want_a_river, serial=tail is not None):
+            if tail is not None and name == "downslope":
+                continue
+            if tail is not None and name == "flowhand_gfi_finish":
+                call = tail
             if ctx is not self.ctx:
                 self.ctx.fork(ctx)
             check(call())
-        if self.side is not None:
+        if self.side is not None and tail is None:
             self.ctx.join(self.side)
 
     def check_status(self):
diff --git a/descriptools_amd/csrc/dt_capi.hip b/descriptools_amd/csrc/dt_capi.hip
--- a/descriptools_amd/csrc/dt_capi.hip
+++ b/descriptools_amd/csrc/dt_capi.hip
@@ -1297,6 +1297,30 @@
                                                 int64_t *a_river64, float *gfi, float *lnhlh) {
   return dev_flowhand_finish_w(c, win, dem, fdr, river, acc64, 1, px, n_gfi, b, res_ok, res_nc, res_nd, rem_gidx, rem_zr,
                                rem_ar, fdist, idx32, idx64, hand, a_river64, gfi, lnhlh, true);
+}
+
+extern "C" int dt_tail_fused_ok(int64_t H, int64_t W) { return dt_tail_fused_shape_ok(H, W) ? 1 : 0; }
+extern "C" int dt_dev_flowhand_gfi_finish_downslope(dt_ctx *c, const dt_window *win, const float *dem,
+                                                    const uint8_t *fdr, const int8_t *river, const int32_t *acc32,
+                                                    double px, double n_gfi, double b, float *fdist, int32_t *idx32,
+                                                    float *hand, int32_t *a_river, float *gfi, float *lnhlh, double dz,
+                                                    int raw, float *down) {
+  DT_DEV(d, c, win);
+  DT_REQUIRE(dem && fdr && river && acc32 && fdist && idx32 && hand && gfi && lnhlh && down, "NULL raster");
+  DT_REQUIRE(d.w.halo == 0 && d.w.gy0 == 0 && d.w.gx0 == 0 && d.w.Hg == d.w.H && d.w.Wg == d.w.W,
+             "the fused tail takes a single raster: the window must be the whole raster, without a halo");
+  DT_REQUIRE(dt_tail_fused_shape_ok(d.w.H, d.w.W) && d.w.ld % 4 == 0,
+             "this raster does not take the fused tail (dt_tail_fused_ok: W % 64 == 0; ld % 4 == 0): use "
+             "dt_dev_flowhand_gfi_finish_w and dt_dev_downslope");
+  DT_REQUIRE((((uintptr_t)dem | (uintptr_t)fdr | (uintptr_t)acc32 | (uintptr_t)fdist | (uintptr_t)idx32 |
+               (uintptr_t)hand | (uintptr_t)a_river | (uintptr_t)gfi | (uintptr_t)lnhlh | (uintptr_t)down) & 15) == 0,
+             "the fused tail takes 16-byte aligned rasters");
+  const DtScratchClaim *k;
+  DT_TRY(dt_scratch_claimed(c, DT_OWNER_HAND, &d.w, false,
+                            "flowhand finish without a matching dt_dev_flowhand_local_w on this context (another call "
+                            "has used the context's scratch in between)", &k));
+  return d.done(dt_launch_tail_ds_fh(c->stream, d.w, dem, fdr, acc32, px, n_gfi, b, k->ptr, fdist, idx32, hand, a_river,
+                                     gfi, lnhlh, dz, raw, down));
 }
 
 static int dt_scratch2_reserve(dt_ctx *c, size_t bytes) {
diff --git a/descriptools_amd/csrc/dt_fh_solve.inc b/descriptools_amd/csrc/dt_fh_solve.inc
--- /dev/null
+++ b/descriptools_amd/csrc/dt_fh_solve.inc
@@ -0,0 +1,52 @@
+  struct CellOut {
+    float fd, h;
+    int32_t i32;
+    AccT ar;
+    long long i64;
+  };
+  auto solve = [&](unsigned long long s, float z) -> CellOut {
+    uint32_t ptr = (uint32_t)(s >> 32), nd = (uint32_t)((s >> 16) & 0xFFFFu);
+    uint32_t ncf = (uint32_t)(s & 0xFFFFu), nc = ncf & 0x7FFFu;
+    uint32_t kind = (ptr >> 12) & 7u, f = ptr & 0xFFFu;
+    bool ok = false;
+    uint32_t ridx = 0;
+    float pz = 0.0f;
+    AccT pa = 0;
+    if (ncf & FHT_DONE) {
+      if (kind == K_RIVER) {
+        ok = true;
+        ridx = (uint32_t)((y0 + (int)f / TW) * w.W + x0 + (int)f % TW);
+        long long ro = (long long)(y0 + (int)f / TW) * w.ld + x0 + (int)f % TW;
+        pz = dem ? dem[ro] : DT_NODATA;
+        pa = acc32 ? acc32[ro] : (AccT)-100;
+      } else if (kind == K_EXIT || kind == K_REXIT) {
+        int slot = dt_slot_of((int)f / TW, (int)f % TW);
+        unsigned long long xs = s_x[slot];
+        uint32_t xptr = (uint32_t)(xs >> 32);
+        if (xptr != FHT_DEAD) {
+          nc += (uint32_t)(xs & 0x7FFFu);
+          nd += (uint32_t)((xs >> 16) & 0xFFFFu);
+          ok = nc + nd <= FHT_CAP;
+          ridx = xptr;
+          s_pay.get(slot, pz, pa);
+        }
+      }
+    }
+    const bool remote = RANKED && ok && (ridx & FHT_REMOTE) != 0u;
+    CellOut o;
+    o.fd = ok ? (float)(dcard * (double)nc + ddiag * (double)nd) : DT_NODATA;
+    o.i32 = (ok && !remote) ? (int32_t)ridx : -100;
+    o.i64 = -100;
+    if (RANKED && ok) {
+      o.i64 = remote ? rem.gidx[ridx & ~FHT_REMOTE]
+                     : (long long)(w.gy0 + (int)(ridx / (uint32_t)w.W)) * w.Wg + w.gx0 + (int)(ridx % (uint32_t)w.W);
+      o.i32 = (int32_t)o.i64;
+    }
+    o.h = DT_NODATA;
+    if (z != DT_NODATA && ok) {
+      o.h = z - pz;
+      if (o.h < 0.0f && o.h != DT_NODATA) o.h = 0.0f;
+    }
+    o.ar = ok ? pa : (AccT)-100;
+    return o;
+  };
diff --git a/descriptools_amd/csrc/dt_fh_tail.h b/descriptools_amd/csrc/dt_fh_tail.h
--- /dev/null
+++ b/descriptools_amd/csrc/dt_fh_tail.h
@@ -0,0 +1,238 @@
+#pragma once
+#include "dt_common.h"
+#include "dt_math.h"
+
+#define TW 64
+#define TH 64
+#define PS (2 * TW + 2 * (TH - 2))
+
+__device__ __forceinline__ int dt_slot_of(int ly, int lx) {
+  if (ly == 0) return lx;
+  if (ly == TH - 1) return TW + lx;
+  if (lx == 0) return 2 * TW + (ly - 1);
+  if (lx == TW - 1) return 2 * TW + (TH - 2) + (ly - 1);
+  return -1;
+}
+__device__ __forceinline__ void dt_cell_of_slot(int s, int &ly, int &lx) {
+  if (s < TW) { ly = 0; lx = s; }
+  else if (s < 2 * TW) { ly = TH - 1; lx = s - TW; }
+  else if (s < 2 * TW + (TH - 2)) { ly = s - 2 * TW + 1; lx = 0; }
+  else { ly = s - 2 * TW - (TH - 2) + 1; lx = TW - 1; }
+}
+__device__ __forceinline__ uint32_t dt_node_of(int y, int x, int tiles_x) {
+  int ty = y / TH, tx = x / TW;
+  return (uint32_t)((ty * tiles_x + tx) * PS + dt_slot_of(y - ty * TH, x - tx * TW));
+}
+
+#define FHT_DEAD 0xFFFFFFFFu
+#define FHT_REMOTE 0x80000000u
+#define FHT_DONE 0x8000u
+#define FHT_CAP 20000u
+#define K_RIVER 1u
+#define K_DEAD 2u
+#define K_EXIT 3u
+#define K_REXIT 4u
+
+__device__ __forceinline__ unsigned long long fht_pack(uint32_t ptr, uint32_t nd, uint32_t ncf) {
+  return ((unsigned long long)ptr << 32) | ((unsigned long long)nd << 16) | (unsigned long long)ncf;
+}
+
+__device__ __forceinline__ uint32_t fh_cache_pack(unsigned long long s) {
+  uint32_t ptr = (uint32_t)(s >> 32);
+  return (ptr & 0x7FFFu) | ((uint32_t)((s >> 16) & 0xFFu) << 15) | ((uint32_t)(s & 0xFFu) << 23);
+}
+__device__ __forceinline__ unsigned long long fh_cache_unpack(uint32_t v) {
+  return fht_pack(v & 0x7FFFu, (v >> 15) & 0xFFu, ((v >> 23) & 0xFFu) | FHT_DONE);
+}
+__device__ __forceinline__ unsigned long long fh_cache_get(const unsigned long long *__restrict__ cache, bool wide,
+                                                            int tile, int c) {
+  if (wide) return cache[(size_t)tile * (TW * TH) + c];
+  return fh_cache_unpack(reinterpret_cast<const uint32_t *>(cache + (size_t)tile * (TW * TH))[c]);
+}
+
+struct FhGfi {
+  float *gfi, *lnhlh;
+  double expo, c0;
+  const DtLogEntry *tab;
+};
+struct FhRemote {
+  const long long *gidx;
+  const float *zr;
+  const long long *ar;
+};
+template <typename AccT>
+struct FhPay;
+template <>
+struct FhPay<int32_t> {
+  unsigned long long v[PS];
+  __device__ __forceinline__ void set(int i, float z, int32_t a) {
+    v[i] = ((unsigned long long)(uint32_t)a << 32) | (unsigned long long)__float_as_uint(z);
+  }
+  __device__ __forceinline__ void get(int i, float &z, int32_t &a) const {
+    const unsigned long long p = v[i];
+    z = __uint_as_float((uint32_t)p);
+    a = (int32_t)(uint32_t)(p >> 32);
+  }
+};
+template <>
+struct FhPay<long long> {
+  long long av[PS];
+  float zv[PS];
+  __device__ __forceinline__ void set(int i, float z, long long a) {
+    av[i] = a;
+    zv[i] = z;
+  }
+  __device__ __forceinline__ void get(int i, float &z, long long &a) const {
+    z = zv[i];
+    a = av[i];
+  }
+};
+
+typedef float fh_v4f __attribute__((ext_vector_type(4)));
+typedef int fh_v4i __attribute__((ext_vector_type(4)));
+__device__ __forceinline__ void fh_store4(float *p, float a, float b, float c, float d) {
+  fh_v4f v = {a, b, c, d};
+  __builtin_nontemporal_store(v, reinterpret_cast<fh_v4f *>(p));
+}
+__device__ __forceinline__ void fh_store4(int32_t *p, int32_t a, int32_t b, int32_t c, int32_t d) {
+  fh_v4i v = {a, b, c, d};
+  __builtin_nontemporal_store(v, reinterpret_cast<fh_v4i *>(p));
+}
+typedef long long fh_v2l __attribute__((ext_vector_type(2)));
+__device__ __forceinline__ void fh_store4(long long *p, long long a, long long b, long long c, long long d) {
+  fh_v2l v0 = {a, b}, v1 = {c, d};
+  __builtin_nontemporal_store(v0, reinterpret_cast<fh_v2l *>(p));
+  __builtin_nontemporal_store(v1, reinterpret_cast<fh_v2l *>(p + 2));
+}
+
+struct FhTailArgs {
+  const int32_t *acc;
+  uint32_t nnodes;
+  const unsigned long long *nodes, *cache;
+  const uint8_t *cache_wide;
+  float *fdist;
+  int32_t *idx;
+  float *hand;
+  int32_t *a_river;
+  FhGfi G;
+};
+int dt_fh_tail_args(hipStream_t s, const DtWin &w, void *scratch, const int32_t *acc, double n_gfi, double b_gfi,
+                    double size, float *fdist, int32_t *idx, float *hand, int32_t *a_river, float *gfi, float *lnhlh,
+                    FhTailArgs *a);
+
+#define FH_TAIL_LDS (2 * PS * 8 + DT_LOGTAB_N * 16)
+
+template <int EARLY>
+struct FhTail {
+  const FhTailArgs &a;
+  const float *__restrict__ dem;
+  const uint8_t *__restrict__ fdr;
+  const DtWin &w;
+  int tiles_x;
+  double px;
+  unsigned long long p_o;
+  float p_zr;
+  int32_t p_ar;
+  uint4 c_w;
+  float4 c_z;
+  int4 c_f;
+  bool wide;
+
+  __device__ __forceinline__ void perimeter(int tile, int y0, int x0) {
+    p_o = fht_pack(FHT_DEAD, 0, FHT_DONE);
+    p_zr = DT_NODATA;
+    p_ar = -100;
+    if (threadIdx.x < PS) {
+      int ly, lx;
+      dt_cell_of_slot(threadIdx.x, ly, lx);
+      const int f = ly * TW + lx;
+      const uint32_t sp = (uint32_t)(fh_cache_get(a.cache, wide, tile, f) >> 32);
+      if (sp == ((uint32_t)f | (K_EXIT << 12))) {
+        int dy, dx;
+        dt_d8_delta(fdr[(long long)(y0 + ly) * w.ld + x0 + lx], dy, dx);
+        const unsigned long long ns = a.nodes[dt_node_of(y0 + ly + dy, x0 + lx + dx, tiles_x)];
+        const uint32_t nptr = (uint32_t)(ns >> 32), nnd = (uint32_t)((ns >> 16) & 0xFFFFu);
+        const uint32_t nncf = (uint32_t)(ns & 0xFFFFu);
+        const bool diag = dy != 0 && dx != 0;
+        if ((nncf & FHT_DONE) && nptr != FHT_DEAD) {
+          p_o = fht_pack(nptr, nnd + (diag ? 1u : 0u), ((nncf & 0x7FFFu) + (diag ? 0u : 1u)) | FHT_DONE);
+          const long long ro = (long long)(nptr / (uint32_t)w.W) * w.ld + (nptr % (uint32_t)w.W);
+          p_zr = dem[ro];
+          p_ar = a.acc[ro];
+        }
+      }
+    }
+  }
+  __device__ __forceinline__ void cells(int tile, long long o, bool row_in) {
+    c_w = make_uint4(0u, 0u, 0u, 0u);
+    c_z = make_float4(DT_NODATA, DT_NODATA, DT_NODATA, DT_NODATA);
+    c_f = make_int4(0, 0, 0, 0);
+    if (!row_in) return;
+    if (!wide) c_w = *reinterpret_cast<const uint4 *>(reinterpret_cast<const uint32_t *>(a.cache + (size_t)tile * (TW * TH)) + 4 * threadIdx.x);
+    c_z = *reinterpret_cast<const float4 *>(dem + o);
+    c_f = *reinterpret_cast<const int4 *>(a.acc + o);
+  }
+  __device__ __forceinline__ void before(int tile, int ty, int tx) {
+    wide = a.cache_wide[tile] != 0;
+    const int y0 = ty * TH, x0 = tx * TW;
+    if (EARLY & 1) perimeter(tile, y0, x0);
+    if (EARLY & 2) {
+      const int y = y0 + (int)(threadIdx.x >> 4);
+      cells(tile, (long long)y * w.ld + x0 + 4 * (int)(threadIdx.x & 15u), y < w.H);
+    }
+  }
+  __device__ __forceinline__ void after(unsigned char *lds, int tile, int ty, int tx) {
+    unsigned long long *s_x = reinterpret_cast<unsigned long long *>(lds);
+    FhPay<int32_t> &s_pay = *reinterpret_cast<FhPay<int32_t> *>(lds + PS * 8);
+    DtLogEntry *s_tab = reinterpret_cast<DtLogEntry *>(lds + 2 * PS * 8);
+    const int y0 = ty * TH, x0 = tx * TW;
+    const int y = y0 + (int)(threadIdx.x >> 4);
+    const bool row_in = y < w.H;
+    const long long o = (long long)y * w.ld + x0 + 4 * (int)(threadIdx.x & 15u);
+    __syncthreads();
+    dt_math_stage(a.G.tab, s_tab);
+    if (!(EARLY & 1)) perimeter(tile, y0, x0);
+    if (threadIdx.x < PS) {
+      s_x[threadIdx.x] = p_o;
+      s_pay.set((int)threadIdx.x, p_zr, p_ar);
+    }
+    if (!(EARLY & 2)) cells(tile, o, row_in);
+    uint4 wa = c_w, wb = make_uint4(0u, 0u, 0u, 0u);
+    if (wide && row_in) {
+      const uint4 *cp = reinterpret_cast<const uint4 *>(a.cache + (size_t)tile * (TW * TH) + 4 * threadIdx.x);
+      wa = cp[0];
+      wb = cp[1];
+    }
+    __syncthreads();
+    if (!row_in) return;
+    const double dcard = px, ddiag = px * sqrt(2.0);
+    constexpr bool RANKED = false;
+    typedef int32_t AccT;
+    const int32_t *acc32 = a.acc;
+    const FhRemote rem{nullptr, nullptr, nullptr};
+#include "dt_fh_solve.inc"
+    const float zz[4] = {c_z.x, c_z.y, c_z.z, c_z.w};
+    const int32_t ff[4] = {c_f.x, c_f.y, c_f.z, c_f.w};
+    const uint32_t cw[8] = {wa.x, wa.y, wa.z, wa.w, wb.x, wb.y, wb.z, wb.w};
+    float fd[4], h[4], g[4], l[4];
+    int32_t ri[4], ar[4];
+#pragma unroll
+    for (int k = 0; k < 4; k++) {
+      const unsigned long long s = wide ? ((unsigned long long)cw[2 * k + 1] << 32) | cw[2 * k] : fh_cache_unpack(cw[k]);
+      const CellOut r = solve(s, zz[k]);
+      fd[k] = r.fd;
+      ri[k] = r.i32;
+      h[k] = r.h;
+      ar[k] = r.ar;
+      dt_gfi_both_cell(r.h, r.ar, ff[k], a.G.expo, a.G.c0, s_tab, g[k], l[k]);
+      asm volatile("" : "+v"(fd[k]), "+v"(ri[k]), "+v"(h[k]), "+v"(ar[k]), "+v"(g[k]), "+v"(l[k]));
+      __builtin_amdgcn_sched_barrier(0);
+    }
+    fh_store4(a.fdist + o, fd[0], fd[1], fd[2], fd[3]);
+    fh_store4(a.idx + o, ri[0], ri[1], ri[2], ri[3]);
+    fh_store4(a.hand + o, h[0], h[1], h[2], h[3]);
+    if (a.a_river) fh_store4(a.a_river + o, ar[0], ar[1], ar[2], ar[3]);
+    fh_store4(a.G.gfi + o, g[0], g[1], g[2], g[3]);
+    fh_store4(a.G.lnhlh + o, l[0], l[1], l[2], l[3]);
+  }
+};
diff --git a/descriptools_amd/csrc/dt_kernels.h b/descriptools_amd/csrc/dt_kernels.h
--- a/descriptools_amd/csrc/dt_kernels.h
+++ b/descriptools_amd/csrc/dt_kernels.h
@@ -67,6 +67,10 @@
                        const int32_t *col_starts, int tx, void *send, int32_t *counts, int32_t *scratch);
 int dt_launch_ds_walk_seed(hipStream_t s, const DtWin &w, const float *dem, int64_t n, const int32_t *ys,
                            const int32_t *xs, void *rec);
+bool dt_tail_fused_shape_ok(int64_t H, int64_t W);
+int dt_launch_tail_ds_fh(hipStream_t s, const DtWin &w, const float *dem, const uint8_t *fdr, const int32_t *acc,
+                         double px, double n_gfi, double b_gfi, void *fh_scratch, float *fdist, int32_t *idx,
+                         float *hand, int32_t *a_river, float *gfi, float *lnhlh, double dz, int raw, float *down);
 int dt_launch_downslope_v1(hipStream_t s, const float *dem, const uint8_t *fdr, int64_t H, int64_t W,
                            double px, double dz, int raw, float *out);
 int dt_launch_hand_i64(hipStream_t s, const float *dem, const int64_t *idx, int64_t n, float *hand);
diff --git a/descriptools_amd/csrc/dt_kernels.hip b/descriptools_amd/csrc/dt_kernels.hip
--- a/descriptools_amd/csrc/dt_kernels.hip
+++ b/descriptools_amd/csrc/dt_kernels.hip
@@ -3,6 +3,7 @@
 #include "dt_common.h"
 #include "dt_kernels.h"
 #include "dt_math.h"
+#include "dt_fh_tail.h"
 
 void dt_math_host_table(DtLogEntry *tab) {
   for (int i = 0; i < DT_LOGTAB_N; i++) {
@@ -623,12 +624,18 @@
 #define MW_RING 0x2000u
 #define MW_STOP 0x8000u
 
-template <int DW_M, bool QUEUE, bool RANKED>
+struct DsNoTail {
+  __device__ __forceinline__ void before(int, int, int) {}
+  __device__ __forceinline__ void after(unsigned char *, int, int, int) {}
+};
+
+template <int DW_M, bool QUEUE, bool RANKED, class TAIL = DsNoTail>
 __device__ __forceinline__ void ds_win_body(const float *__restrict__ dem,
                                                        const uint8_t *__restrict__ fdr, DtWin w,
                                                        double px, double dz, float dzf, int raw,
                                                        float *__restrict__ out, int tiles_x, int ntiles,
-                                                       int *__restrict__ n_unresolved, DsQueue queue, DsWalkOut wo) {
+                                                       int *__restrict__ n_unresolved, DsQueue queue, DsWalkOut wo,
+                                                       TAIL tail = TAIL()) {
   constexpr int DW_WIN = DW_CORE + 2 * DW_M, DW_LD = DW_WIN + 4;
   __shared__ __attribute__((aligned(16))) unsigned char smem[DW_LD * DW_WIN * 6];
   __shared__ uint16_t s_lut[256];
@@ -649,6 +656,7 @@
     }
   }
   const int tyi = tile / tiles_x, txi = tile - tyi * tiles_x;
+  tail.before(tile, tyi, txi);
   const int wy0 = tyi * DW_CORE - DW_M, wx0 = txi * DW_CORE - DW_M;
   const bool vec = (w.ld % 4 == 0) && (((uintptr_t)dem & 15) == 0) && (((uintptr_t)fdr & 3) == 0);
   const int ya = max(-w.halo, -w.gy0), yb = min(w.H + w.halo, w.Hg - w.gy0);
@@ -871,6 +879,7 @@
       slot++;
     }
   }
+  tail.after(smem, tile, tyi, txi);
 }
 
 template <int DW_M>
@@ -880,6 +889,16 @@
                                                        int ntiles, int *__restrict__ n_unresolved) {
   ds_win_body<DW_M, false, false>(dem, fdr, w, px, dz, dzf, raw, out, tiles_x, ntiles, n_unresolved, DsQueue(),
                                   DsWalkOut());
+}
+template <int EARLY>
+__global__ __launch_bounds__(1024, 8) void k_tail_ds_fh(const float *__restrict__ dem, const uint8_t *__restrict__ fdr,
+                                                        DtWin w, double px, double dz, float dzf, int raw,
+                                                        float *__restrict__ out, int tiles_x, int ntiles,
+                                                        FhTailArgs a) {
+  static_assert(FH_TAIL_LDS <= (DW_CORE + 2 * 24 + 4) * (DW_CORE + 2 * 24) * 6, "the last pass's arrays fit the window");
+  static_assert(DW_CORE == TW && DW_CORE == TH, "one downslope tile is one tile of the last pass");
+  ds_win_body<24, false, false>(dem, fdr, w, px, dz, dzf, raw, out, tiles_x, ntiles, nullptr, DsQueue(), DsWalkOut(),
+                                FhTail<EARLY>{a, dem, fdr, w, tiles_x, px});
 }
 __global__ __launch_bounds__(1024, 8) void k_downslope_win_r(const float *__restrict__ dem,
                                                          const uint8_t *__restrict__ fdr, DtWin w, double px,
@@ -1499,6 +1518,29 @@
   }
   return DT_OK;
 }
+bool dt_tail_fused_shape_ok(int64_t H, int64_t W) { return H > 0 && W > 0 && W % DW_CORE == 0; }
+#ifndef DT_TAIL_EARLY
+#define DT_TAIL_EARLY 0
+#endif
+int dt_launch_tail_ds_fh(hipStream_t s, const DtWin &w, const float *dem, const uint8_t *fdr, const int32_t *acc,
+                         double px, double n_gfi, double b_gfi, void *fh_scratch, float *fdist, int32_t *idx,
+                         float *hand, int32_t *a_river, float *gfi, float *lnhlh, double dz, int raw, float *down) {
+  const bool single = w.halo == 0 && w.gy0 == 0 && w.gx0 == 0 && w.Hg == w.H && w.Wg == w.W;
+  DT_REQUIRE(single && dt_tail_fused_shape_ok(w.H, w.W) && w.ld % 4 == 0,
+             "the fused tail takes a single raster with rows of whole 64-cell tiles (dt_tail_fused_ok)");
+  DT_REQUIRE((((uintptr_t)dem | (uintptr_t)fdr | (uintptr_t)acc | (uintptr_t)fdist | (uintptr_t)idx | (uintptr_t)hand |
+               (uintptr_t)a_river | (uintptr_t)gfi | (uintptr_t)lnhlh | (uintptr_t)down) & 15) == 0,
+             "the fused tail takes 16-byte aligned rasters");
+  const int tiles_x = w.W / DW_CORE, tiles_y = (w.H + DW_CORE - 1) / DW_CORE;
+  const int64_t ntiles = (int64_t)tiles_x * tiles_y;
+  float dzf = (float)dz;
+  if ((double)dzf < dz) dzf = nextafterf(dzf, INFINITY);
+  FhTailArgs a;
+  DT_TRY(dt_fh_tail_args(s, w, fh_scratch, acc, n_gfi, b_gfi, px, fdist, idx, hand, a_river, gfi, lnhlh, &a));
+  hipLaunchKernelGGL(k_tail_ds_fh<DT_TAIL_EARLY>, dim3((unsigned)ntiles), dim3(1024), 0, s, dem, fdr, w, px, dz, dzf,
+                     raw, down, tiles_x, (int)ntiles, a);
+  return DT_OK;
+}
 int dt_launch_downslope_v1(hipStream_t s, const float *dem, const uint8_t *fdr, int64_t H, int64_t W,
                            double px, double dz, int raw, float *out) {
   int64_t n = H * W;
diff --git a/descriptools_amd/csrc/dt_tiles.hip b/descriptools_amd/csrc/dt_tiles.hip
--- a/descriptools_amd/csrc/dt_tiles.hip
+++ b/descriptools_amd/csrc/dt_tiles.hip
@@ -1,35 +1,15 @@
 #include "dt_common.h"
 #include "dt_kernels.h"
 #include "dt_math.h"
-
-#define TW 64
-#define TH 64
+#include "dt_fh_tail.h"
+
 #define NT (TW * TH)
-#define PS (2 * TW + 2 * (TH - 2))
 #define CPT (NT / 256)
 
 #define NX_SINK 0xFFFFu
 #define NX_EXIT 0xFFFEu
 #define NX_REXIT 0xFFFDu
 #define X_NONE 0xFFFFu
-
-__device__ __forceinline__ int dt_slot_of(int ly, int lx) {
-  if (ly == 0) return lx;
-  if (ly == TH - 1) return TW + lx;
-  if (lx == 0) return 2 * TW + (ly - 1);
-  if (lx == TW - 1) return 2 * TW + (TH - 2) + (ly - 1);
-  return -1;
-}
-__device__ __forceinline__ void dt_cell_of_slot(int s, int &ly, int &lx) {
-  if (s < TW) { ly = 0; lx = s; }
-  else if (s < 2 * TW) { ly = TH - 1; lx = s - TW; }
-  else if (s < 2 * TW + (TH - 2)) { ly = s - 2 * TW + 1; lx = 0; }
-  else { ly = s - 2 * TW - (TH - 2) + 1; lx = TW - 1; }
-}
-__device__ __forceinline__ uint32_t dt_node_of(int y, int x, int tiles_x) {
-  int ty = y / TH, tx = x / TW;
-  return (uint32_t)((ty * tiles_x + tx) * PS + dt_slot_of(y - ty * TH, x - tx * TW));
-}
 
 __device__ __forceinline__ int dt_tile_of_block(int b, int ntiles) {
   const int full = ntiles & ~15;
@@ -1074,19 +1054,6 @@
   return DT_OK;
 }
 
-#define FHT_DEAD 0xFFFFFFFFu
-#define FHT_REMOTE 0x80000000u
-#define FHT_DONE 0x8000u
-#define FHT_CAP 20000u
-#define K_RIVER 1u
-#define K_DEAD 2u
-#define K_EXIT 3u
-#define K_REXIT 4u
-
-__device__ __forceinline__ unsigned long long fht_pack(uint32_t ptr, uint32_t nd, uint32_t ncf) {
-  return ((unsigned long long)ptr << 32) | ((unsigned long long)nd << 16) | (unsigned long long)ncf;
-}
-
 struct FhTile {
   uint8_t *s_fdr;
   uint8_t *s_halo;
@@ -1211,19 +1178,6 @@
     if (!((uint32_t)T.s_st[c] & FHT_DONE)) T.s_st[c] = fht_pack((uint32_t)c | (K_DEAD << 12), 0, FHT_DONE);
   }
   __syncthreads();
-}
-
-__device__ __forceinline__ uint32_t fh_cache_pack(unsigned long long s) {
-  uint32_t ptr = (uint32_t)(s >> 32);
-  return (ptr & 0x7FFFu) | ((uint32_t)((s >> 16) & 0xFFu) << 15) | ((uint32_t)(s & 0xFFu) << 23);
-}
-__device__ __forceinline__ unsigned long long fh_cache_unpack(uint32_t v) {
-  return fht_pack(v & 0x7FFFu, (v >> 15) & 0xFFu, ((v >> 23) & 0xFFu) | FHT_DONE);
-}
-__device__ __forceinline__ unsigned long long fh_cache_get(const unsigned long long *__restrict__ cache, bool wide,
-                                                            int tile, int c) {
-  if (wide) return cache[(size_t)tile * NT + c];
-  return fh_cache_unpack(reinterpret_cast<const uint32_t *>(cache + (size_t)tile * NT)[c]);
 }
 
 __global__ __launch_bounds__(256) void k_fh_tile1(const uint8_t *__restrict__ fdr,
@@ -1556,60 +1510,6 @@
   nodes[nnodes + i] = o;
 }
 
-struct FhGfi {
-  float *gfi, *lnhlh;
-  double expo, c0;
-  const DtLogEntry *tab;
-};
-struct FhRemote {
-  const long long *gidx;
-  const float *zr;
-  const long long *ar;
-};
-template <typename AccT>
-struct FhPay;
-template <>
-struct FhPay<int32_t> {
-  unsigned long long v[PS];
-  __device__ __forceinline__ void set(int i, float z, int32_t a) {
-    v[i] = ((unsigned long long)(uint32_t)a << 32) | (unsigned long long)__float_as_uint(z);
-  }
-  __device__ __forceinline__ void get(int i, float &z, int32_t &a) const {
-    const unsigned long long p = v[i];
-    z = __uint_as_float((uint32_t)p);
-    a = (int32_t)(uint32_t)(p >> 32);
-  }
-};
-template <>
-struct FhPay<long long> {
-  long long av[PS];
-  float zv[PS];
-  __device__ __forceinline__ void set(int i, float z, long long a) {
-    av[i] = a;
-    zv[i] = z;
-  }
-  __device__ __forceinline__ void get(int i, float &z, long long &a) const {
-    z = zv[i];
-    a = av[i];
-  }
-};
-
-typedef float fh_v4f __attribute__((ext_vector_type(4)));
-typedef int fh_v4i __attribute__((ext_vector_type(4)));
-__device__ __forceinline__ void fh_store4(float *p, float a, float b, float c, float d) {
-  fh_v4f v = {a, b, c, d};
-  __builtin_nontemporal_store(v, reinterpret_cast<fh_v4f *>(p));
-}
-__device__ __forceinline__ void fh_store4(int32_t *p, int32_t a, int32_t b, int32_t c, int32_t d) {
-  fh_v4i v = {a, b, c, d};
-  __builtin_nontemporal_store(v, reinterpret_cast<fh_v4i *>(p));
-}
-typedef long long fh_v2l __attribute__((ext_vector_type(2)));
-__device__ __forceinline__ void fh_store4(long long *p, long long a, long long b, long long c, long long d) {
-  fh_v2l v0 = {a, b}, v1 = {c, d};
-  __builtin_nontemporal_store(v0, reinterpret_cast<fh_v2l *>(p));
-  __builtin_nontemporal_store(v1, reinterpret_cast<fh_v2l *>(p + 2));
-}
 
 template <bool RANKED, int VH, int MINW, typename AccT>
 __global__ __launch_bounds__(256, MINW) void k_fh_tile3(const uint8_t *__restrict__ fdr,
@@ -1679,58 +1579,7 @@
                    (!a_river || ((uintptr_t)a_river & 15) == 0) &&
                    (!G.gfi || ((((uintptr_t)G.gfi | (uintptr_t)G.lnhlh | (uintptr_t)acc32) & 15) == 0));
   const double dcard = px, ddiag = px * sqrt(2.0);
-  struct CellOut {
-    float fd, h;
-    int32_t i32;
-    AccT ar;
-    long long i64;
-  };
-  auto solve = [&](unsigned long long s, float z) -> CellOut {
-    uint32_t ptr = (uint32_t)(s >> 32), nd = (uint32_t)((s >> 16) & 0xFFFFu);
-    uint32_t ncf = (uint32_t)(s & 0xFFFFu), nc = ncf & 0x7FFFu;
-    uint32_t kind = (ptr >> 12) & 7u, f = ptr & 0xFFFu;
-    bool ok = false;
-    uint32_t ridx = 0;
-    float pz = 0.0f;
-    AccT pa = 0;
-    if (ncf & FHT_DONE) {
-      if (kind == K_RIVER) {
-        ok = true;
-        ridx = (uint32_t)((y0 + (int)f / TW) * w.W + x0 + (int)f % TW);
-        long long ro = (long long)(y0 + (int)f / TW) * w.ld + x0 + (int)f % TW;
-        pz = dem ? dem[ro] : DT_NODATA;
-        pa = acc32 ? acc32[ro] : (AccT)-100;
-      } else if (kind == K_EXIT || kind == K_REXIT) {
-        int slot = dt_slot_of((int)f / TW, (int)f % TW);
-        unsigned long long xs = s_x[slot];
-        uint32_t xptr = (uint32_t)(xs >> 32);
-        if (xptr != FHT_DEAD) {
-          nc += (uint32_t)(xs & 0x7FFFu);
-          nd += (uint32_t)((xs >> 16) & 0xFFFFu);
-          ok = nc + nd <= FHT_CAP;
-          ridx = xptr;
-          s_pay.get(slot, pz, pa);
-        }
-      }
-    }
-    const bool remote = RANKED && ok && (ridx & FHT_REMOTE) != 0u;
-    CellOut o;
-    o.fd = ok ? (float)(dcard * (double)nc + ddiag * (double)nd) : DT_NODATA;
-    o.i32 = (ok && !remote) ? (int32_t)ridx : -100;
-    o.i64 = -100;
-    if (RANKED && ok) {
-      o.i64 = remote ? rem.gidx[ridx & ~FHT_REMOTE]
-                     : (long long)(w.gy0 + (int)(ridx / (uint32_t)w.W)) * w.Wg + w.gx0 + (int)(ridx % (uint32_t)w.W);
-      o.i32 = (int32_t)o.i64;
-    }
-    o.h = DT_NODATA;
-    if (z != DT_NODATA && ok) {
-      o.h = z - pz;
-      if (o.h < 0.0f && o.h != DT_NODATA) o.h = 0.0f;
-    }
-    o.ar = ok ? pa : (AccT)-100;
-    return o;
-  };
+#include "dt_fh_solve.inc"
   if (vec) {
     constexpr int VPT = NT / 4 / 256;
 #pragma unroll 1
@@ -1979,6 +1828,23 @@
   return DT_OK;
 }
 
+int dt_fh_tail_args(hipStream_t s, const DtWin &w, void *scratch, const int32_t *acc, double n_gfi, double b_gfi,
+                    double size, float *fdist, int32_t *idx, float *hand, int32_t *a_river, float *gfi, float *lnhlh,
+                    FhTailArgs *a) {
+  const FhScratch f = fh_layout(w, scratch);
+  a->acc = acc;
+  a->nnodes = (uint32_t)f.nnodes;
+  a->nodes = f.nodes;
+  a->cache = f.cache;
+  a->cache_wide = f.cache_wide;
+  a->fdist = fdist;
+  a->idx = idx;
+  a->hand = hand;
+  a->a_river = a_river;
+  a->G = FhGfi{gfi, lnhlh, n_gfi, log(b_gfi) + n_gfi * log(size * size), dt_math_device_table(s)};
+  return DT_OK;
+}
+
 #define RK_MAX 64
 struct RkLayout {
   int ty, tx, nranks;
diff --git a/include/descriptools_hip.h b/include/descriptools_hip.h
--- a/include/descriptools_hip.h
+++ b/include/descriptools_hip.h
@@ -275,6 +275,11 @@
                                  const int64_t *rem_gidx, const float *rem_zr, const int64_t *rem_ar,
                                  float *fdist, int32_t *idx32, int64_t *idx64, float *hand, int32_t *a_river,
                                  float *gfi, float *lnhlh);
+int dt_tail_fused_ok(int64_t H, int64_t W);
+int dt_dev_flowhand_gfi_finish_downslope(dt_ctx *ctx, const dt_window *whole, const float *dem, const uint8_t *fdr,
+                                         const int8_t *river, const int32_t *acc32, double px, double n_gfi, double b,
+                                         float *fdist, int32_t *idx32, float *hand, int32_t *a_river, float *gfi,
+                                         float *lnhlh, double dz, int raw, float *down);
 
 int dt_dev_slope_d8_f64_w(dt_ctx *ctx, const dt_window *win, const double *dem, double px, uint8_t *fdr, float *proxy);
 int dt_dev_slope_twi_f64_w(dt_ctx *ctx, const dt_window *win, const double *dem, const int32_t *acc32, double px,
```

Result: faster. 36440 Mcells/s (median of 6 runs) (+1.2%).
